# Plachtaa/FAcodec

Measured on AMD Instinct MI355X. Metric: 24kHz audio sec encoded+decoded per wall-sec, higher is better.
Workload: dtype f32; 1 GPU; configs[1]: batch=32/GPU x 2 s @ 24 kHz, forward encoder->FVQ(6 codebooks)->decoder, FAcodec configs/config.yml model (137.7 M params), weights formula-generated, weight-norm re-materialised every step; clips_per_gpu=32, samples_per_clip=48000, parallelism=dp1 (independent clips, no collective)

## Files before the change

facodec_amd/_lib.py:

```python
import ctypes as C
import os

_HERE = os.path.dirname(os.path.abspath(__file__))
LIB_PATH = os.environ.get("FAC_LIB_PATH", os.path.join(_HERE, "libfacodec_hip.so"))

PAD_ZERO, PAD_REFLECT = 0, 1
ACT_NONE, ACT_TANH, ACT_MISH, ACT_LOG_MEL = 0, 1, 2, 3
ACT_GATE, ACT_WN_RES_SKIP = 4, 5

_p = C.c_void_p
_i = C.c_int
_i64 = C.c_int64
_f = C.c_float


class ConvDesc(C.Structure):
    _fields_ = [
        ("x", _p), ("w", _p), ("bias", _p), ("alpha_in", _p), ("alpha_out", _p), ("res", _p), ("y", _p), ("y2", _p), ("alpha_y2", _p), ("w_k1", _p), ("bias_k1", _p),
        ("x_bs", _i64), ("x_cs", _i64), ("y_bs", _i64), ("y_cs", _i64),
        ("B", C.c_int32), ("C_in", C.c_int32), ("T_in", C.c_int32), ("C_out", C.c_int32),
        ("C_out_pad", C.c_int32), ("T_out", C.c_int32),
        ("K", C.c_int32), ("stride", C.c_int32), ("dilation", C.c_int32), ("pad_left", C.c_int32),
        ("pad_mode", C.c_int32), ("n_phase", C.c_int32), ("y_tstride", C.c_int32), ("phase_shift", C.c_int32),
        ("act", C.c_int32),
        ("w_batched", C.c_int32), ("w_bs", _i64), ("ws", _p), ("ws_bytes", _i64), ("w_split", _p),
        ("K1", C.c_int32), ("dilation2", C.c_int32), ("row_phases", C.c_int32),
        ("x_p8", _p), ("x_p8_plane_bytes", _i64), ("y2_p8", _p), ("y2_p8_plane_bytes", _i64),
        ("pw_split", C.c_int32), ("split_rows", C.c_int32),
        ("gate_cond", _p), ("gate_cond_bs", _i64),
    ]


class VqDesc(C.Structure):
    _fields_ = [
        ("residual", _p), ("z_in", _p), ("zq_acc", _p), ("zq_out", _p), ("w_in", _p), ("b_in", _p),
        ("codebook", _p), ("w_out", _p), ("w_out_scale", _p), ("b_out", _p), ("mask", _p), ("codes", _p), ("z_e", _p),
        ("loss_part", _p), ("codes_bs", _i64),
        ("B", C.c_int32), ("D", C.c_int32), ("T", C.c_int32), ("Kc", C.c_int32),
    ]



VQ_DECODE_MAX_Q = 16


class VqDecodeDesc(C.Structure):
    _fields_ = [
        ("codes", _p * 3), ("codes_bs", _i64 * 3), ("codes_qs", _i64 * 3), ("n_q", C.c_int32 * 3),
        ("codebook", _p * VQ_DECODE_MAX_Q), ("w_out", _p * VQ_DECODE_MAX_Q), ("w_out_scale", _p * VQ_DECODE_MAX_Q),
        ("b_out", _p * VQ_DECODE_MAX_Q), ("style", _p), ("outs", _p), ("z", _p * 3),
        ("B", C.c_int32), ("D", C.c_int32), ("T", C.c_int32), ("Kc", C.c_int32),
    ]


class ResampleDesc(C.Structure):
    _fields_ = [
        ("hist", _p), ("x", _p), ("lens", _p), ("y", _p), ("hist_out", _p), ("table", _p), ("offs", _p),
        ("hist_bs", _i64), ("x_bs", _i64), ("y_bs", _i64), ("q0", _i64), ("m_lo", _i64),
        ("B", C.c_int32), ("n_hist", C.c_int32), ("T", C.c_int32), ("n_out", C.c_int32),
        ("o", C.c_int32), ("n", C.c_int32), ("taps", C.c_int32),
    ]


SIGNATURES = {
    "fac_version": (_i, []),
    "fac_last_error": (C.c_char_p, []),
    "fac_wn_scale": (_i, [_p, _p, _p, _i, _i, _p]),
    "fac_pack_conv_w": (_i, [_p, _p, _p, _i, _i, _i, _i, _p]),
    "fac_pack_convtr_w_rows": (_i, [_p, _p, _p, _i, _i, _i, _p]),
    "fac_conv_w_split_bytes": (_i64, [_i, _i, _i]),
    "fac_conv_w_split2_bytes": (_i64, [_i, _i, _i, _i]),
    "fac_pack_conv_w_split2": (_i, [_p, _p, _p, _i, _i, _i, _i, _p]),
    "fac_gemm_w_split_bytes": (_i64, [_i, _i, _i, _i]),
    "fac_pack_gemm_w_split": (_i, [_p, _i64, _i64, _i64, _p, _p, _i, _i, _i, _i, _p]),
    "fac_pack_conv_w_split": (_i, [_p, _p, _p, _i, _i, _i, _p]),
    "fac_conv_w_split_rows_bytes": (_i64, [_i, _i, _i, _i]),
    "fac_pack_conv_w_split_rows": (_i, [_p, _p, _p, _i, _i, _i, _i, _p]),
    "fac_flip_transpose_w": (_i, [_p, _p, _p, _i, _i, _i, _p]),
    "fac_prep_begin": (_i, []),
    "fac_prep_set_phase": (_i, [_i]),
    "fac_prep_abort": (_i, []),
    "fac_prep_end": (_i, []),
    "fac_prep_replay": (_i, [_i, _p]),
    "fac_prep_info": (_i, [_i, _p, _p]),
    "fac_prep_free": (_i, [_i]),
    "fac_pack_conv_w_bwd": (_i, [_p, _p, _p, _i, _i, _i, _i, _p]),
    "fac_pad_fold_bwd": (_i, [_p, _p, _i, _i, _i, _i, _i, _i, _p]),
    "fac_conv1d_bwd_weight_ws_bytes": (_i64, [_i, _i, _i, _i, _i]),
    "fac_conv1d_bwd_weight": (_i, [_p, _p, _p, _p, _i64, _i, _i, _i, _i, _i, _i, _i, _i, _i, _i, _i, _i, _p]),
    "fac_conv1d_bwd_weight_split_ws_bytes": (_i64, [_i, _i, _i, _i, _i, _i, _i, _i, _i, _i]),
    "fac_conv1d_bwd_weight_split_form": (_i, [_i, _i, _i, _i, _i, _i, _i, _i, _i, _i, _i, C.POINTER(C.c_int)]),
    "fac_conv1d_bwd_weight_k1_ws_bytes": (_i64, [_i, _i, _i, _i]),
    "fac_conv1d_bwd_weight_k1_ws_bytes_for": (_i64, [_p, _p, _i, _i, _i, _i]),
    "fac_conv1d_bwd_weight_taps_tx": (_i64, [_i, _i, _i, _i, _i]),
    "fac_conv1d_bwd_weight_taps_ws_bytes": (_i64, [_i, _i, _i, _i, _i, _i, _i, _i]),
    "fac_conv1d_bwd_weight_taps_ws_bytes_for": (_i64, [_p, _i, _i, _i, _i, _i, _i, _i, _i]),
    "fac_conv1d_bwd_weight_taps": (_i, [_p, _p, _p, _p, _p, _i64, _i, _i, _i, _i, _i, _i, _i, _i, _i, _p]),
    "fac_conv1d_bwd_weight_k1": (_i, [_p, _p, _p, _p, _p, _i64, _i, _i, _i, _i, _p]),
    "fac_conv1d_bwd_weight_split": (_i, [_p, _p, _p, _p, _i64, _i, _i, _i, _i, _i, _i, _i, _i, _i, _i, _i, _i, _p]),
    "fac_conv1d_bwd_weight_split_db_ok": (_i, [_i, _i, _i, _i, _i, _i, _i, _i, _i, _i]),
    "fac_conv1d_bwd_weight_split_db": (_i, [_p, _p, _p, _p, _p, _i64, _i, _i, _i, _i, _i, _i, _i, _i, _i, _i, _i, _i, _p]),
    "fac_weight_norm_bwd": (_i, [_p, _p, _p, _p, _p, _i, _i, _p]),
    "fac_snake_bwd": (_i, [_p, _p, _p, _p, _p, _p, _i, _i, _i, _p]),
    "fac_pack_lstm_whh_t": (_i, [_p, _p, _i, _p]),
    "fac_lstm_layer_bwd": (_i, [_p, _p, _p, _p, _p, _p, _i, _i, _i, _p]),
    "fac_to_p8": (_i, [_p, _p, _p, _i, _i, _i, _p]),
    "fac_lstm_persist_ok": (_i, [_i, _i]),
    "fac_lstm_persist_stream_ok": (_i, [_p]),
    "fac_pack_lstm_whh16": (_i, [_p, _p, _i, _i, _p]),
    "fac_lstm_layer_fwd_persist": (_i, [_p, _p, _p, _p, _p, _p, _i, _i, _i, _i, _p]),
    "fac_lstm_layer_bwd_persist": (_i, [_p, _p, _p, _p, _p, _p, _i, _i, _i, _i, _p]),
    "fac_lstm_persist_split_ok": (_i, [_i, _i]),
    "fac_lstm_persist_timeouts": (_i, []),
    "fac_lstm_persist_arm": (_i, [_p]),
    "fac_lstm_abort_flag": (_i, [_p, _p]),
    "fac_mask_flags_if": (_i, [_p, _i, _p, _p]),
    "fac_pack_lstm_whh_split": (_i, [_p, _p, _i, _p]),
    "fac_lstm_layer_fwd_persist_split": (_i, [_p, _p, _p, _p, _i, _i, _i, _i, _p]),
    "fac_snake_bwd_fused": (_i, [_p, _p, _p, _p, _p, _p, _p, _p, _i, _i, _i, _p]),
    "fac_bias_grad": (_i, [_p, _p, _p, _i, _i, _i, _p]),
    "fac_snake_bwd_fused_rs": (_i, [_p, _p, _p, _i64, _p, _p, _p, _p, _p, _i, _i, _i, _p]),
    "fac_pad_fold_edges": (_i, [_p, _i, _i, _i, _i, _i, _p]),
    "fac_pack_convtr_w": (_i, [_p, _p, _p, _i, _i, _i, _i, _p]),
    "fac_conv1d_fwd": (_i, [C.POINTER(ConvDesc), _p]),
    "fac_conv1d_variant": (_i, [C.POINTER(ConvDesc), C.c_char_p, _i]),
    "fac_snake_fwd": (_i, [_p, _p, _p, _i, _i, _i, _p]),
    "fac_lstm_to_time_major": (_i, [_p, _p, _i, _i, _i, _p]),
    "fac_lstm_from_time_major": (_i, [_p, _p, _p, _p, _i, _i, _i, _p]),
    "fac_pack_lstm_whh": (_i, [_p, _p, _i, _p]),
    "fac_lstm_layer_fwd": (_i, [_p, _p, _p, _p, _i, _i, _i, _p]),
    "fac_lstm_layer_fwd_from": (_i, [_p, _p, _p, _p, _i, _i, _i, _i64, _p]),
    "fac_lstm_layer_fwd_train": (_i, [_p, _p, _p, _p, _p, _p, _i, _i, _i, _i64, _p]),
    "fac_lstm_gate_bwd": (_i, [_p, _p, _p, _p, _p, _p, _p, _i, _i, _i64, _i, _p]),
    "fac_tanh_bwd": (_i, [_p, _p, _p, _i64, _p]),
    "fac_pair_bwd": (_i, [_p, _p, _p, _i64, _i, C.c_float, C.c_float, _i, _p]),
    "fac_spec_power_bwd": (_i, [_p, _p, _p, _i, _i, _i, _i, _p]),
    "fac_stft_frames_bwd": (_i, [_p, _p, _i, _i, _i, _i, _i, _i, _i, _p]),
    "fac_vq_latent_bwd": (_i, [_p, _p, _p, _i64, _p, _p, _p, _p, _i, _i, _p]),
    "fac_vq_codebook_grad": (_i, [_p, _p, _p, _i64, _p, _p, _i, _i, _i, _i, _p]),
    "fac_layernorm_c_affine_bwd": (_i, [_p, _p, _p, _p, _p, _p, _i, _i, _i, _p]),
    "fac_rows_fma": (_i, [_p, _p, _p, _p, _i, _i64, _f, _p]),
    "fac_grad_norm_clip": (_i, [_p, _i64, _f, _p, _p, _p]),
    "fac_adamw_step": (_i, [_p, _p, _p, _p, _i64, _f, _f, _f, _f, _f, _i64, _p, _p]),
    "fac_logdiff_rms_bwd": (_i, [_p, _p, _p, _i, _i, _i, _f, _f, _i, _p]),
    "fac_gather_copy": (_i, [_p, _p, _p, _i, _p]),
    "fac_adamw_step_masked": (_i, [_p, _p, _p, _p, _i64, _p, _i, _p, _p, _p, _f, _f, _f, _f, _f, _p, _p]),
    "fac_gate_bwd": (_i, [_p, _p, _p, _i, _i, _i, _p]),
    "fac_mish_fwd": (_i, [_p, _p, _i64, _p]),
    "fac_mish_bwd": (_i, [_p, _p, _p, _i64, _p]),
    "fac_glu_bwd": (_i, [_p, _p, _p, _i, _i, _i, _p]),
    "fac_mul_scaled": (_i, [_p, _p, _p, _f, _i64, _p]),
    "fac_embed_sum_bwd": (_i, [_p, _p, _p, _i, _i, _i, _i, _i, _i, _i, _p]),
    "fac_gate_bwd_cond": (_i, [_p, _p, _i64, _p, _p, _p, _i64, _i, _i, _i, _p]),
    "fac_masked_mean_bwd": (_i, [_p, _p, _p, _i, _i, _i, _p]),
    "fac_attention_probs": (_i, [_p, _p, _p, _p, _i, _i, _i, _i, _p]),
    "fac_attention_pv": (_i, [_p, _p, _p, _i, _i, _i, _i, _p]),
    "fac_attention_bwd_pv": (_i, [_p, _p, _p, _p, _p, _i, _i, _i, _i, _p]),
    "fac_attention_bwd_qk": (_i, [_p, _p, _p, _p, _p, _p, _p, _i, _i, _i, _i, _p]),
    "fac_aa_snakebeta_bwd": (_i, [_p, _p, _p, _p, _p, _p, _p, _p, _p, _i, _i, _i, _p]),
    "fac_leaky_relu": (_i, [_p, _p, _p, _i64, _f, _i, _i, _i, _i, _i, _p]),
    "fac_spec_to_cat": (_i, [_p, _p, _i, _i, _i, _i, _i, _i, _i, _p]),
    "fac_period_fold": (_i, [_p, _p, _i, _i, _i, _i, _i, _i, _p]),
    "fac_zero_insert": (_i, [_p, _p, _i64, _i, _i, _p]),
    "fac_row_stack3": (_i, [_p, _p, _i64, _i, _i, _i, _i, _p]),
    "fac_spec_to_rows": (_i, [_p, _p, _i, _i, _i, _i, _i, _i, _p]),
    "fac_pad_reflect": (_i, [_p, _p, _i, _i, _i, _i, _p]),
    "fac_disc_preprocess": (_i, [_p, _p, _p, _p, _i, _i, _p]),
    "fac_cross_entropy": (_i, [_p, _p, _p, _p, _p, _i64, _i, _f, _p]),
    "fac_focal_scalar": (_i, [_p, _p, _f, _p]),
    "fac_crop_rows": (_i, [_p, _p, _p, _i, _i, _i64, _i, _i, _p]),
    "fac_stream_push": (_i, [_p, _p, _i64, _i64, _i, _i, _i, _p]),
    "fac_vq_fwd": (_i, [C.POINTER(VqDesc), _p]),
    "fac_vq_loss_tiles": (_i, [_i]),
    "fac_vq_decode": (_i, [C.POINTER(VqDecodeDesc), _p]),
    "fac_rccl_available": (_i, []),
    "fac_rccl_unique_id": (_i, [_p]),
    "fac_rccl_comm_init": (_i, [C.POINTER(_p), _p, _i, _i]),
    "fac_rccl_comm_destroy": (_i, [_p]),
    "fac_allreduce_arena": (_i, [_p, _p, _i64, _i, _p]),
    "fac_vq_search": (_i, [_p, _p, _p, _i64, _i, _p]),
    "fac_gate_tanh_sigmoid": (_i, [_p, _p, _i64, _p, _i, _i, _i, _p]),
    "fac_embed_sum": (_i, [_p, _p, _p, _i, _i, _i, _i, _i, _i, _i, _i, _p]),
    "fac_glu_residual": (_i, [_p, _p, _p, _i, _i, _i, _p]),
    "fac_add": (_i, [_p, _p, _p, _i64, _p]),
    "fac_sub2": (_i, [_p, _p, _p, _p, _i64, _p]),
    "fac_mul_mask": (_i, [_p, _p, _i, _i, _i, _p]),
    "fac_wn_res_skip": (_i, [_p, _p, _p, _i, _i, _i, _i, _p]),
    "fac_attention": (_i, [_p, _p, _p, _p, _p, _i, _i, _i, _i, _p]),
    "fac_attention_stream": (_i, [_p, _p, _p, _p, _p, _i, _i, _i, _i, _p]),
    "fac_attention_route": (_i, [_i, _i]),
    "fac_attention_stream_tile": (_i, [_i]),
    "fac_masked_mean": (_i, [_p, _p, _p, _i, _i, _i, _p]),
    "fac_layernorm_c_affine": (_i, [_p, _p, _p, _i, _i, _i, _p]),
    "fac_stft_frames": (_i, [_p, _p, _i, _i, _i, _i, _i, _i, _i, _p]),
    "fac_stft_frames_ragged": (_i, [_p, _p, _p, _i, _i, _i, _i, _i, _i, _i, _p]),
    "fac_mask_tail": (_i, [_p, _p, _i, _i, _i, _i, _p]),
    "fac_mask_tail_i64": (_i, [_p, _p, _i, _i, _i, _i, _p]),
    "fac_frame_mask": (_i, [_p, _p, _p, _i, _i, _i, _p]),
    "fac_resample": (_i, [C.POINTER(ResampleDesc), _p]),
    "fac_resample_form": (_i, [C.POINTER(ResampleDesc), _p]),
    "fac_spec_power": (_i, [_p, _p, _i, _i, _i, _i, _p]),
    "fac_reduce_pair": (_i, [_p, _p, _p, _p, _i64, _i, _f, _f, _i, _p]),
    "fac_aa_snakebeta_fwd": (_i, [_p, _p, _p, _p, _p, _i, _i, _i, _p]),
    "fac_logdiff_rms": (_i, [_p, _p, _p, _p, _i, _i, _i, _f, _f, _i, _p]),
    "fac_jdc_affine_lrelu_pool": (_i, [_p, _p, _p, _p, _i, _i, _i, _i, _i, _i, _i, _f, _p]),
    "fac_jdc_layout_in": (_i, [_p, _p, _i, _i, _i, _i, _p]),
    "fac_jdc_to_time_major": (_i, [_p, _p, _i, _i, _i, _i, _i, _i, _i, _p]),
    "fac_jdc_to_nchw": (_i, [_p, _p, _i, _i, _i, _i, _i, _i, _p]),
    "fac_jdc_head": (_i, [_p, _p, _p, _p, _p, _i, _i, _i, _i, _p]),
    "fac_f0_normalize": (_i, [_p, _p, _p, _i, _i, _p]),
    "fac_mel_log_norm": (_i, [_p, _p, _i, _i, _i, _p]),
}

_lib = None


class FacodecHipError(RuntimeError):
    pass


def load():
    global _lib
    if _lib is not None:
# ... 20 lines not shown
```

facodec_amd/build.py:

```python
import os
import subprocess
import sys
from concurrent.futures import ThreadPoolExecutor

HERE = os.path.dirname(os.path.abspath(__file__))
CSRC = os.path.join(HERE, "csrc")
TAG = os.environ.get("FAC_BUILD_TAG", "")
LIB = os.path.join(HERE, "libfacodec_hip%s.so" % ("_" + TAG if TAG else ""))
OBJDIR = "build" + ("_" + TAG if TAG else "")
SOURCES = ["conv1d_api.hip", "conv1d_tile_128x128.hip", "conv1d_tile_96x128.hip", "conv1d_tile_64x128.hip",
           "conv1d_tile_32x256.hip", "conv1d_tile_128x32.hip", "conv1d_tile_128x256.hip", "conv1d_fused_ru.hip", "conv1d_narrow.hip", "conv1d_pw.hip", "conv1d_pw_split.hip", "conv1d_skinny.hip", "conv1d_bsplit.hip", "conv1d_bsplit96.hip", "conv1d_gemm_split.hip", "conv1d_bsplit2.hip", "conv1d_bwd.hip", "conv1d_wgrad_split.hip", "conv1d_wgrad_k1.hip", "train_misc.hip", "optim.hip", "train_quant.hip", "train_pred.hip", "train_disc.hip", "train_redecoder.hip", "pack.hip", "prep_batch.hip", "lstm.hip", "lstm_persist.hip", "vq.hip", "vq_decode.hip", "misc.hip", "attention_stream.hip", "ragged.hip", "resample.hip", "jdc.hip", "rccl_arena.hip"]
FLAGS = ["--offload-arch=gfx950", "-O3", "-std=c++17", "-fPIC", "-ffp-contract=off",
         "-Wno-unused-result"] + os.environ.get("FAC_EXTRA_FLAGS", "").split()


def _hipcc():
    for cand in (os.environ.get("HIPCC"), "/opt/rocm/bin/hipcc", "hipcc"):
        if cand and (os.path.isabs(cand) and os.path.exists(cand) or not os.path.isabs(cand)):
            return cand
    return "hipcc"


def _stale(target, deps):
    if not os.path.exists(target):
        return True
    tt = os.path.getmtime(target)
    return any(os.path.getmtime(d) > tt for d in deps)


def build_lib(force=False, verbose=True):
    hipcc = _hipcc()
    headers = sorted(os.path.join(CSRC, f) for f in os.listdir(CSRC) if f.endswith(".h")) + [os.path.join(HERE, "..", "include", "facodec_hip.h")]
    objs, jobs = [], []
    os.makedirs(os.path.join(CSRC, OBJDIR), exist_ok=True)
    for src in SOURCES:
        s = os.path.join(CSRC, src)
        o = os.path.join(CSRC, OBJDIR, src.replace(".hip", ".o"))
        objs.append(o)
        if force or _stale(o, [s] + headers):
            jobs.append([hipcc, *FLAGS, "-c", s, "-o", o])

    def run(cmd):
        if verbose:
            print(" ".join(cmd), file=sys.stderr)
        subprocess.run(cmd, check=True)

    with ThreadPoolExecutor(max_workers=min(8, max(1, len(jobs)))) as ex:
        list(ex.map(run, jobs))
    if force or jobs or _stale(LIB, objs):
        run([hipcc, "--offload-arch=gfx950", "-shared", "-fPIC", *objs, "-ldl", "-o", LIB])
    return LIB


if __name__ == "__main__":
    build_lib(force="--force" in sys.argv)
    print(LIB)
```

facodec_amd/convplan.py:

```python
from collections import namedtuple

__all__ = ["ConvPlan", "ConvTrPlan", "plan_conv", "plan_convtr", "plan_gemm", "tile_rows", "gemm_split_ok", "gemm_split_strided_ok", "split2_ok",
           "pw_taps_ok", "pw_split_tail_ok", "convtr_split_ok", "convtr_rows_ok", "flat_strided_ok", "flat_convtr_ok", "W_FP32", "W_TAPS",
           "W_GEMM", "W_GEMM_STRIDED", "W_SPLIT2", "W_FP32_PW_TAPS", "PER_CLIP", "FLAT_STRIDED", "FLAT_STRIDE1", "TR_POLYPHASE", "TR_ROWS",
           "TR_ROWS_SPLIT", "TR_ROWS_PW_TAPS", "TR_FLAT"]

W_FP32, W_TAPS, W_GEMM, W_GEMM_STRIDED, W_SPLIT2, W_FP32_PW_TAPS = "fp32", "split_taps", "split_gemm", "split_gemm_strided", "split2", "fp32_pw_taps"
PER_CLIP, FLAT_STRIDED, FLAT_STRIDE1 = "per_clip", "flat_strided", "flat_stride1"
ConvPlan = namedtuple("ConvPlan", "layout form p8")
TR_POLYPHASE, TR_ROWS, TR_ROWS_SPLIT, TR_ROWS_PW_TAPS, TR_FLAT = "polyphase", "rows", "rows_split", "rows_pw_taps", "flat_rows_split"
ConvTrPlan = namedtuple("ConvTrPlan", "layout p8")


def _sw():
    from . import ops
    return ops


def gemm_split_ok(c_out, c_in, k, n_cols, t_out=None):
    sw = _sw()
    if not (sw.BF16_SPLIT and k in (1, 2)):
        return False
    if c_in < sw.GEMM_SPLIT_MIN_CIN or c_out < 64 or n_cols < 1024:
        return False
    return k == 1 or (t_out is not None and t_out >= 256)


def gemm_split_strided_ok(c_out, c_in, k, stride, batch, t_out):
    return (_sw().BF16_SPLIT and 1 < stride <= 16 and stride < k <= 2 * stride and c_in >= 32
            and c_out >= 64 and t_out >= 256 and batch * t_out >= 1024)


def split2_ok(c_out, k, k1, stride, n_cols):
    kv = k1 if 0 < k1 < k else k
    return (_sw().BF16_SPLIT and 8 <= c_out <= 32 and ((kv == 9 and stride in (1, 2)) or (kv == 3 and stride == 1))
            and n_cols >= 4096)


def pw_split_tail_ok(c_in, c_out, cols):
    sw = _sw()
    return sw.BF16_SPLIT and sw.PW_SPLIT and c_in == c_out and c_in in (256, 384) and cols >= 65536


def pw_taps_ok(c_in, c_out, k, stride, transposed, batch, t_out):
    sw = _sw()
    if not (sw.BF16_SPLIT and sw.PW_SPLIT and sw.PW_TAPS and stride == 2):
        return False
    taps, rows = (2, 2 * c_out) if transposed else (4, c_out)
    if k != 4 or (c_in * taps) % 64 or c_in * taps > 384 or rows % 64:
        return False
    return batch * ((t_out + 31) // 32) >= 2 * (256 // (rows // 64)) * 12


def convtr_rows_ok(t_in, stride, causal=True):
    sw = _sw()
    return sw.CONVTR_ROWS and causal and 2 <= stride <= 16 and t_in >= sw.CONVTR_ROWS_MIN_T


def convtr_split_ok(c_in, c_out, stride, batch, t_in, causal=True, alpha_in=None):
    return (_sw().BF16_SPLIT and causal and alpha_in is None and 2 <= stride <= 16 and c_in >= 64
            and t_in >= 256 and batch * t_in >= 1024 and c_out * stride >= 64)


def flat_strided_ok(c_out, c_in, k, s, batch, n_out):
    return (_sw().FLAT_TRAIN and k == 2 * s and s > 1 and n_out < 256 and not gemm_split_strided_ok(c_out, c_in, k, s, batch, n_out)
            and gemm_split_strided_ok(c_out, c_in, k, s, 1, batch * (n_out + 1) - 1))


def flat_convtr_ok(c_in, c_out, s, batch, t_cols):
    return (_sw().FLAT_TRAIN and t_cols < 256 and not convtr_split_ok(c_in, c_out, s, batch, t_cols)
            and convtr_split_ok(c_in, c_out, s, 1, batch * t_cols))


def tile_rows(c_out, c_in, k, grad=False):
    sw = _sw()
    return 96 if (sw.BF16_SPLIT and not grad and k == 7 and c_out in sw.BS_ROWS96 and c_in % 8 == 0) else 64


def plan_conv(c_out, c_in, k, stride, dilation, batch, t_in, t_out, *, k1=0, alpha_in=False, plain=True, res=False,
              causal_reflect=False, grad=True, c_out_mult16=True, split_k=(1, 3, 5, 7), floor_k=(3, 5), tail="pw_split",
              pw_taps=True, split2=False, flat_infer=False, flat_stride1=False, flat_train=None):
    sw = _sw()
    cols = batch * t_out
    p8 = 2.0 * c_out * k / (4.0 * stride)
    if split2 and split2_ok(c_out, k, k1, stride, cols):
        return ConvPlan(W_SPLIT2, PER_CLIP, None)
    if stride > 1:
        strided = not alpha_in and dilation == 1 and not k1
        flat_t = (flat_train is not None and strided and plain and t_in % stride == 0
                  and (flat_train == "zero" or (causal_reflect and t_in > stride))
                  and flat_strided_ok(c_out, c_in, k, stride, batch, t_out))
        if flat_t and flat_train == "reflect":
            return ConvPlan(W_GEMM_STRIDED, FLAT_STRIDED, p8)
        if pw_taps and stride == 2 and strided and plain and pw_taps_ok(c_in, c_out, k, 2, False, batch, t_out):
            return ConvPlan(W_FP32_PW_TAPS, PER_CLIP, None)
        if strided and gemm_split_strided_ok(c_out, c_in, k, stride, batch, t_out):
            return ConvPlan(W_GEMM_STRIDED, PER_CLIP, p8)
        if flat_t:
            return ConvPlan(W_GEMM_STRIDED, FLAT_STRIDED, p8)
        if (flat_infer and strided and not res and causal_reflect and k == 2 * stride and t_in % stride == 0 and t_in > stride
                and not grad and gemm_split_strided_ok(c_out, c_in, k, stride, 1, batch * (t_in // stride + 1) - 1)):
            return ConvPlan(W_GEMM_STRIDED, FLAT_STRIDED, p8)
    elif not alpha_in and not k1 and k in split_k:
        if k == 1 and gemm_split_ok(c_out, c_in, 1, cols):
            if not (pw_split_tail_ok(c_in, c_out, cols) if tail == "pw_split"
                    else tail is not None and c_in == c_out and c_in in (256, 384) and cols >= 65536):
                return ConvPlan(W_GEMM, PER_CLIP, None)
        if (sw.BF16_SPLIT and k in (3, 5, 7) and c_in % 16 == 0 and c_out > 2 and (c_out % 16 == 0 or not c_out_mult16)
                and cols > 640 and (k not in floor_k or (c_in >= 64 and c_out > 32))):
            if (flat_infer and flat_stride1 and k == 7 and not res and causal_reflect and not grad and batch >= 4
                    and (k - 1) * dilation < t_in <= 224 and c_in * c_out >= 1 << 20):
                return ConvPlan(W_TAPS, FLAT_STRIDE1, None)
            return ConvPlan(W_TAPS, PER_CLIP, None)
    return ConvPlan(W_FP32, PER_CLIP, None)


def plan_gemm(c_out, c_in, n_cols):
    ok = gemm_split_ok(c_out, c_in, 1, n_cols)
    return ConvPlan(W_GEMM if ok else W_FP32, PER_CLIP, 2.0 * c_out / 4.0 if ok else None)


def plan_convtr(c_in, c_out, stride, batch, t_in, *, causal=True, alpha_in=False, grad=True, flat_infer=False, flat_train_cols=None):
    a = True if alpha_in else None
    p8 = 2.0 * c_out * 2 * stride / 4.0
    if causal and flat_train_cols is not None and flat_convtr_ok(c_in, c_out, stride, batch, flat_train_cols):
        return ConvTrPlan(TR_FLAT, p8)
    if causal and not alpha_in and pw_taps_ok(c_in, c_out, 2 * stride, stride, True, batch, t_in):
        return ConvTrPlan(TR_ROWS_PW_TAPS, None)
    if convtr_split_ok(c_in, c_out, stride, batch, t_in, causal, a):
        return ConvTrPlan(TR_ROWS_SPLIT, p8)
    if flat_infer and not grad and t_in < 256 and convtr_split_ok(c_in, c_out, stride, 1, batch * (t_in + 1), causal, a):
        return ConvTrPlan(TR_FLAT, p8)
    return ConvTrPlan(TR_ROWS if convtr_rows_ok(t_in, stride, causal) else TR_POLYPHASE, None)
```

facodec_amd/csrc/common.h:

```cpp
#pragma once
#include <hip/hip_runtime.h>
#include <stdint.h>
#include <stdio.h>
#include <stdarg.h>
#include "../../include/facodec_hip.h"

namespace fac {

void set_error(const char* fmt, ...);

inline int check_launch(const char* what) {
  hipError_t e = hipGetLastError();
  if (e != hipSuccess) {
    set_error("%s: launch failed: %s", what, hipGetErrorString(e));
    return FAC_ERR_LAUNCH;
  }
  return FAC_OK;
}

#define FAC_REQUIRE(cond, ...)          \
  do {                                  \
    if (!(cond)) {                      \
      ::fac::set_error(__VA_ARGS__);    \
      return FAC_ERR_ARG;               \
    }                                   \
  } while (0)

__host__ __device__ constexpr int cin_pad_dev(int c) { return ((c + 47) / 48) * 48; }

__device__ __attribute__((noinline)) float sin_sq_slow(float y) {
  const float s = sinf(y);
  return __fmul_rn(s, s);
}

__device__ __forceinline__ float sin_sq(float y) {
  if (__builtin_expect(fabsf(y) > 4096.0f, 0)) return sin_sq_slow(y);
  const float k = rintf(y * 0.63661977236758134308f);
  float r = fmaf(k, -1.5703125f, y);
  r = fmaf(k, -4.837512969970703125e-4f, r);
  r = fmaf(k, -7.54978995489188216e-8f, r);
  const float z = r * r;
  float ps = fmaf(z, -1.9515295891e-4f, 8.3321608736e-3f);
  ps = fmaf(ps, z, -1.6666654611e-1f);
  const float sn = fmaf(ps * z, r, r);
  float pc = fmaf(z, 2.443315711809948e-5f, -1.388731625493765e-3f);
  pc = fmaf(pc, z, 4.166664568298827e-2f);
  const float cs = fmaf(pc * z, z, fmaf(z, -0.5f, 1.0f));
  const float v = (((int)k) & 1) ? cs : sn;
  return __fmul_rn(v, v);
}

__device__ __forceinline__ float snake_inv(float alpha) { return __fdiv_rn(1.0f, __fadd_rn(alpha, 1e-9f)); }
__device__ __forceinline__ float snake_apply(float x, float alpha, float inv) {
  return __fadd_rn(x, __fmul_rn(inv, sin_sq(__fmul_rn(alpha, x))));
}

__device__ __attribute__((noinline)) float apply_act_slow(float v, int act) {
  if (act == FAC_ACT_TANH) return tanhf(v);
  if (act == FAC_ACT_MISH) {
    const float sp = v > 20.f ? v : log1pf(expf(v));
    return v * tanhf(sp);
  }
  if (act == FAC_ACT_LOG_MEL) return (logf(1e-5f + v) + 4.0f) / 4.0f;
  return v;
}

__device__ __forceinline__ float sigmoid_f(float x) { return __fdiv_rn(1.0f, 1.0f + expf(-x)); }

__device__ __forceinline__ int reflect_index(int t, int T, int Text) {
  int j;
  if (t < 0) j = -t;
  else if (t < Text) j = t;
  else j = 2 * (Text - 1) - t;
  return (j >= 0 && j < T) ? j : -1;
}


typedef __bf16 bf16x8 __attribute__((ext_vector_type(8)));
typedef __bf16 bf16x4 __attribute__((ext_vector_type(4)));
typedef float f32x16 __attribute__((ext_vector_type(16)));
typedef float f32x4 __attribute__((ext_vector_type(4)));
typedef float f32x2 __attribute__((ext_vector_type(2)));
typedef unsigned u32x4 __attribute__((ext_vector_type(4)));

__device__ __forceinline__ void split3(float x, __bf16& h, __bf16& m, __bf16& l) {
  h = (__bf16)x;
  const float r1 = x - (float)h;
  m = (__bf16)r1;
  l = (__bf16)(r1 - (float)m);
}

__device__ __forceinline__ void wg_barrier() {
  asm volatile("" ::: "memory");
  __builtin_amdgcn_s_barrier();
  asm volatile("" ::: "memory");
}

template <class V>
__host__ __device__ constexpr int xcd_contiguous_id(V v, int n) {
  const int q8 = n >> 3, r8 = n & 7;
  const int xcd = v & 7, within = v >> 3;
  return (xcd < r8 ? xcd * (q8 + 1) : r8 * (q8 + 1) + (xcd - r8) * q8) + within;
}
constexpr bool xcd_contiguous_is_permutation(int n) {
  bool seen[64] = {};
  for (int v = 0; v < n; ++v) {
    const int id = xcd_contiguous_id(v, n);
    if (id < 0 || id >= n || seen[id]) return false;
    seen[id] = true;
  }
  return true;
}
static_assert(xcd_contiguous_is_permutation(1) && xcd_contiguous_is_permutation(7) && xcd_contiguous_is_permutation(8) &&
                  xcd_contiguous_is_permutation(9) && xcd_contiguous_is_permutation(13) && xcd_contiguous_is_permutation(64),
              "xcd_contiguous_id must map [0, n) onto [0, n)");

struct XcdGrid {
  int per_xcd;
  unsigned grid;
};
inline XcdGrid xcd_padded_grid(long long total) {
  const int per_xcd = (int)((total + 7) / 8);
  return {per_xcd, (unsigned)(8 * per_xcd)};
}


constexpr size_t FAC_LDS_MAX = 160 * 1024;

template <auto Kern>
inline void allow_dynamic_lds(size_t bytes = FAC_LDS_MAX) {
  static bool done = false;
  if (!done) {
    (void)hipFuncSetAttribute(reinterpret_cast<const void*>(Kern), hipFuncAttributeMaxDynamicSharedMemorySize, (int)bytes);
    done = true;
  }
}

constexpr int FAC_MAX_DEV = 16;
inline int device_cus() {
  static int cus[FAC_MAX_DEV] = {0};
  int dev = 0, v = 0;
  if (hipGetDevice(&dev) != hipSuccess || dev < 0 || dev >= FAC_MAX_DEV) return 0;
  if (cus[dev] == 0 && hipDeviceGetAttribute(&v, hipDeviceAttributeMultiprocessorCount, dev) == hipSuccess) cus[dev] = v;
  return cus[dev];
}

}

#define FAC_PRIO_STAGE 3
#define FAC_PRIO_MFMA 0
```

facodec_amd/csrc/conv1d_api.hip:

```cpp
#include "conv1d_mfma.h"
#include <stdlib.h>

namespace fac {

enum ConvKernel : int {
  CK_128x32 = 0,
  CK_32x256 = 1,
  CK_64x128 = 2,
  CK_96x128 = 3,
  CK_128x128 = 4,
  CK_128x256 = 5,
  CK_96x256 = 6,
  CK_FUSED_RU = 7,
  CK_128x160 = 8,
  CK_NARROW = 9,
  CK_SKINNY = 10,
  CK_BSPLIT = 11,
  CK_CIN1 = 12,
  CK_THIN = 13,
  CK_PW = 14,
  CK_GSPLIT = 15,
  CK_BSPLIT2 = 16,
  CK_PWS = 17,
  CK_PWT = 18,
  CK_BSPLIT96 = 19,
};

static ConvKernel select_variant(const fac_conv_desc* d) {
  const int co = d->C_out;
  if (d->row_phases > 1) return CK_128x256;
  if (d->T_out <= 32) return CK_128x32;
  if (co <= 32) return CK_32x256;
  if (co <= 64) return CK_64x128;
  const bool wide = d->K == 1 && d->n_phase == 1 && d->T_out >= 512;
  if (d->T_out > 128 && d->T_out <= 160 && co > 64) return CK_128x160;
  if (co % 128 != 0 && co % 96 == 0) return wide ? CK_96x256 : CK_96x128;
  return wide ? CK_128x256 : CK_128x128;
}

static bool narrow_ok(const fac_conv_desc* d) {
  return d->C_out <= 2 && d->stride == 1 && d->n_phase == 1 && d->phase_shift == 0 && d->y_tstride == 1 && !d->res && !d->y2 &&
         !d->w_batched && d->y && (long long)d->B <= 65535 && (long long)d->B * ((d->T_out + 1023) / 1024) >= 128;
}

static bool pw_enabled() {
  static const bool on = !(getenv("FAC_PW") && getenv("FAC_PW")[0] == '0');
  return on;
}

static int conv_plan(const fac_conv_desc* d, ConvArgs& a, ConvKernel& k) {
  FAC_REQUIRE(d && (d->x || d->x_p8) && (d->w || d->w_split) && (d->y || d->y2 || d->y2_p8), "conv1d: null pointer");
  FAC_REQUIRE(!d->y2 || d->alpha_y2 || d->act == FAC_ACT_WN_RES_SKIP, "conv1d: y2 needs alpha_y2");
  FAC_REQUIRE(d->B > 0 && d->C_in > 0 && d->C_out > 0 && d->T_in > 0 && d->T_out > 0,
              "conv1d: bad shape B=%d C_in=%d C_out=%d T_in=%d T_out=%d", d->B, d->C_in, d->C_out,
              d->T_in, d->T_out);
  FAC_REQUIRE(d->K >= 1 && d->stride >= 1 && d->dilation >= 1 && d->pad_left >= 0,
              "conv1d: bad K/stride/dilation/pad");
  FAC_REQUIRE(d->C_out_pad % 32 == 0 && (d->C_out_pad >= d->C_out || d->row_phases > 1), "conv1d: C_out_pad must be a multiple of 32");
  FAC_REQUIRE(d->n_phase >= 1 && d->y_tstride >= 1, "conv1d: bad phase config");
  FAC_REQUIRE((long long)d->B * d->n_phase <= 65535, "conv1d: B*n_phase too large for grid.z");
  a.x = d->x; a.w = d->w; a.bias = d->bias; a.alpha_in = d->alpha_in; a.alpha_out = d->alpha_out;
  a.res = d->res; a.y = d->y; a.y2 = d->y2; a.alpha2 = d->alpha_y2;
  a.w1 = d->w_k1; a.bias1 = d->bias_k1;
  a.x_p8 = reinterpret_cast<const unsigned char*>(d->x_p8); a.x_p8_ps = d->x_p8_plane_bytes;
  a.y2_p8 = reinterpret_cast<unsigned char*>(d->y2_p8); a.y2_p8_ps = d->y2_p8_plane_bytes;
  FAC_REQUIRE(!d->y2_p8 || d->alpha_y2, "conv1d: y2_p8 needs alpha_y2");
  if (d->w_k1) {
    FAC_REQUIRE(d->C_in == d->C_out && d->C_out_pad == d->C_out && d->n_phase == 1 && d->stride == 1 &&
                    d->alpha_out && d->act == FAC_ACT_NONE && !d->w_batched,
                "conv1d: fused ResidualUnit needs C_in == C_out (multiple of 32), stride 1, a Snake alpha_out");
  }
  a.x_bs = d->x_bs; a.x_cs = d->x_cs; a.y_bs = d->y_bs; a.y_cs = d->y_cs; a.w_bs = d->w_bs;
  a.B = d->B; a.C_in = d->C_in; a.T_in = d->T_in; a.C_out = d->C_out; a.C_out_pad = d->C_out_pad;
  a.T_out = d->T_out; a.K = d->K; a.stride = d->stride; a.dil = d->dilation;
  a.pad_left = d->pad_left; a.pad_mode = d->pad_mode; a.n_phase = d->n_phase;
  a.y_tstride = d->y_tstride; a.act = d->act; a.w_batched = d->w_batched;
  a.phase_shift = d->phase_shift;
  a.rp = d->row_phases > 1 ? d->row_phases : 1;
  FAC_REQUIRE(!d->gate_cond || (d->act == FAC_ACT_GATE && d->gate_cond_bs >= 0),
              "conv1d: gate_cond is the conditioning row of the FAC_ACT_GATE epilogue (act=%d gate_cond_bs=%lld)", d->act,
              (long long)d->gate_cond_bs);
  a.gate_cond = d->gate_cond; a.gate_cond_bs = d->gate_cond_bs;
  if (a.rp > 1) {
    FAC_REQUIRE(d->n_phase == 1 && d->y_tstride == 1 && d->phase_shift == 0 && d->stride == 1 && a.rp <= 128 && !d->w_k1 &&
                    !d->w_batched && d->C_out_pad == fac_convtr_rows(d->C_out, a.rp) && !(d->K1 > 0 && d->K1 < d->K),
                "conv1d: row_phases needs a plain stride-1 launch on weights from fac_pack_convtr_w_rows");
  }
  a.K1 = d->K1 > 0 ? d->K1 : d->K; a.dil2 = d->dilation2;
  FAC_REQUIRE(a.K1 <= d->K && d->K % a.K1 == 0 && (a.K1 == d->K || d->dilation2 > 0), "conv1d: bad two-level taps (K=%d K1=%d)", d->K, d->K1);
  FAC_REQUIRE(!conv_two_level(a) || (!d->w_k1 && d->n_phase == 1 && d->pad_mode == FAC_PAD_ZERO && !d->w_batched),
              "conv1d: two-level taps need a plain, zero-padded conv");
  conv_set_virtual(a);
  FAC_REQUIRE(d->phase_shift >= 0 && d->phase_shift < d->n_phase + (d->n_phase == 1), "conv1d: bad phase_shift");
  {
    long long last = (long long)(d->T_out - 1) * d->stride + (long long)conv_max_tap_offset(a) - d->pad_left;
    int pad_right = last >= d->T_in ? (int)(last - d->T_in + 1) : 0;
    int max_pad = d->pad_left > pad_right ? d->pad_left : pad_right;
    a.T_ext = d->T_in > max_pad ? d->T_in : max_pad + 1;
  }
  if (d->x_p8 || d->y2_p8) {
    const bool gs = d->w_split && (d->K <= 2 || (d->stride > 1 && d->K <= 2 * d->stride)) && conv_gsplit_ok(a) &&
                    !conv_skinny_ok(a, d->ws, d->ws_bytes) && d->C_in % 8 == 0 && d->x_p8_plane_bytes < (1ll << 32);
    const bool ok = !d->y2_p8 && (gs || (d->w_split && !conv_two_level(a) && (d->split_rows == 96 ? conv_bsplit96_p8_ok(a) : conv_bsplit_p8_ok(a)) &&
                                       !conv_cin1_ok(a)));
    FAC_REQUIRE(ok, "conv1d: P8 operands given but the launch does not run on a kernel that takes them (K=%d stride=%d C_in=%d columns=%lld)",
                d->K, d->stride, d->C_in, (long long)d->B * d->T_out);
  }
  if (d->act == FAC_ACT_GATE || d->act == FAC_ACT_WN_RES_SKIP) {
    FAC_REQUIRE(d->w && !d->w_k1 && !d->x_p8 && !conv_two_level(a) && conv_skinny_ok(a, d->ws, d->ws_bytes),
                "conv1d: FAC_ACT_GATE / FAC_ACT_WN_RES_SKIP exist only for few-column launches (B * T_out <= 640) with a workspace");
    k = CK_SKINNY;
    return FAC_OK;
  }
  if (d->w_k1) { k = CK_FUSED_RU; return FAC_OK; }
  a.gflat = 0;
  a.grt = 0;
  if (d->w_split && (a.KV == 9 || a.KV == 3) && d->C_out <= 32 && conv_bsplit2_ok(a)) {
    a.w = reinterpret_cast<const float*>(d->w_split);
    k = CK_BSPLIT2;
    return FAC_OK;
  }
  FAC_REQUIRE(!conv_two_level(a) || d->w, "conv1d: two-level taps outside the split kernel's shapes need fp32 weights");
  const bool pw_on = pw_enabled();
  if (pw_on && d->pw_split && d->w && conv_pwt_ok(a)) { k = CK_PWT; return FAC_OK; }
  if (d->w_split && (d->K <= 2 || (d->stride > 1 && d->K <= 2 * d->stride)) && conv_gsplit_ok(a) &&
      !conv_skinny_ok(a, d->ws, d->ws_bytes)) {
    a.w = reinterpret_cast<const float*>(d->w_split);
    k = CK_GSPLIT;
    return FAC_OK;
  }
  if (a.rp > 1) {
    FAC_REQUIRE(d->w != nullptr && d->w != (const float*)d->w_split, "conv1d: row_phases launch outside the split kernel's shapes needs fp32 weights");
    k = CK_128x256;
    return FAC_OK;
  }
  const bool two_level = conv_two_level(a);
  FAC_REQUIRE(d->split_rows == 0 || d->split_rows == 64 || d->split_rows == 96, "conv1d: split_rows must be 0, 64 or 96");
  if (d->split_rows == 96) {
    FAC_REQUIRE(d->w_split && !two_level && conv_bsplit96_ok(a) && !conv_cin1_ok(a),
                "conv1d: split_rows = 96 needs a stride-1 k = 7 launch with C_out %% 96 == 0, C_in %% 8 == 0 and more than 640 columns "
                "(K=%d stride=%d C_in=%d C_out=%d columns=%lld)", d->K, d->stride, d->C_in, d->C_out, (long long)d->B * d->T_out);
    a.w = reinterpret_cast<const float*>(d->w_split);
    k = CK_BSPLIT96;
    return FAC_OK;
  }
  if (d->w_split && !two_level && conv_bsplit_ok(a) && !conv_cin1_ok(a)) {
    a.w = reinterpret_cast<const float*>(d->w_split);
    k = CK_BSPLIT;
    return FAC_OK;
  }
  FAC_REQUIRE(d->w != nullptr && (const void*)d->w != d->w_split,
              "conv1d: shape does not qualify for a split-bf16 kernel (K=%d stride=%d C_in=%d C_out=%d columns=%lld) and no fp32 "
              "weights were given", d->K, d->stride, d->C_in, d->C_out, (long long)d->B * d->T_out);
  if (!two_level && conv_skinny_ok(a, d->ws, d->ws_bytes)) k = CK_SKINNY;
  else if (narrow_ok(d) && (!two_level || (a.KV - 1) * a.dil <= 64)) k = CK_NARROW;
  else if (conv_thin_ok(a, d->ws, d->ws_bytes)) k = CK_THIN;
  else if (conv_cin1_ok(a)) k = CK_CIN1;
  else if (pw_on && d->pw_split && conv_pw_ok(a) && conv_pws_ok(a)) k = CK_PWS;
  else if (pw_on && conv_pw_ok(a)) k = CK_PW;
  else k = select_variant(d);
  return FAC_OK;
}

}

extern "C" int fac_conv1d_fwd(const fac_conv_desc* d, fac_stream_t stream) {
  using namespace fac;
  ConvArgs a;
  ConvKernel k;
  if (const int rc = conv_plan(d, a, k)) return rc;
  hipStream_t s = (hipStream_t)stream;
  switch (k) {
    case CK_128x32: return conv_dispatch_128x32(a, s);
    case CK_32x256: return conv_dispatch_32x256(a, s);
    case CK_64x128: return conv_dispatch_64x128(a, s);
    case CK_96x128: return conv_dispatch_96x128(a, s);
    case CK_128x128: return conv_dispatch_128x128(a, s);
    case CK_128x256: return conv_dispatch_128x256(a, s);
    case CK_96x256: return conv_dispatch_96x256(a, s);
    case CK_FUSED_RU: return conv_dispatch_fused_ru(a, s);
    case CK_128x160: return conv_dispatch_128x160(a, s);
    case CK_NARROW: return conv_dispatch_narrow(a, s);
    case CK_SKINNY: return conv_dispatch_skinny(a, d->ws, d->ws_bytes, s);
    case CK_BSPLIT: return conv_dispatch_bsplit(a, s);
    case CK_CIN1: return conv_dispatch_cin1(a, s);
    case CK_THIN: return conv_dispatch_thin(a, d->ws, s);
    case CK_PW: return conv_dispatch_pw(a, s);
    case CK_GSPLIT: return conv_dispatch_gsplit(a, s);
    case CK_BSPLIT2: return conv_dispatch_bsplit2(a, s);
    case CK_PWS: return conv_dispatch_pws(a, s);
    case CK_PWT: return conv_dispatch_pwt(a, s);
    case CK_BSPLIT96: return conv_dispatch_bsplit96(a, s);
  }
  return FAC_ERR_ARG;
}

extern "C" int fac_conv1d_variant(const fac_conv_desc* d, char* name, int name_len) {
  using namespace fac;
  ConvArgs a;
  ConvKernel k;
  if (const int rc = conv_plan(d, a, k)) return rc;
  if (!name || name_len <= 0) return k;
  switch (k) {
    case CK_128x32: snprintf(name, name_len, "conv1d_mfma_kernel<1,1,4,1,K> 128x32"); break;
    case CK_32x256: snprintf(name, name_len, "conv1d_mfma_kernel<1,2,1,4,K> 32x256"); break;
    case CK_64x128: snprintf(name, name_len, "conv1d_mfma_kernel<2,1,1,4,K> 64x128"); break;
    case CK_96x128: snprintf(name, name_len, "conv1d_mfma_kernel<3,1,1,4,K> 96x128"); break;
    case CK_128x128: snprintf(name, name_len, "conv1d_mfma_kernel<2,2,2,2,K> 128x128"); break;
    case CK_128x256:
      snprintf(name, name_len, a.rp > 1 ? "conv1d_mfma_kernel<2,2,2,4,2> 128x256 (convtr, all phases per tile)" : "conv1d_mfma_kernel<2,2,2,4,K> 128x256");
      break;
    case CK_96x256: snprintf(name, name_len, "conv1d_mfma_kernel<3,1,1,8,K> 96x256"); break;
    case CK_FUSED_RU: snprintf(name, name_len, "conv1d_mfma_kernel<C/32,1,1,4,7,fused RU> Cx128"); break;
    case CK_128x160: snprintf(name, name_len, "conv1d_mfma_kernel<1,5,4,1,K> 128x160"); break;
    case CK_NARROW:
      snprintf(name, name_len, conv_two_level(a) ? "conv1d_narrow_kernel (VALU, C_out<=2, two-level taps)" : "conv1d_narrow_kernel (VALU, C_out<=2)");
      break;
    case CK_SKINNY:
      snprintf(name, name_len, conv_skinny_single_launch(a) ? "conv1d_gemv_kernel (single launch, <=4 columns)"
                                                            : "conv1d_skinny_kernel (split reduction, <=640 columns)");
      break;
    case CK_BSPLIT: snprintf(name, name_len, "conv1d_bsplit_kernel<%d> 64x256 (bf16x3 split, fp32-grade)", a.K); break;
    case CK_CIN1: snprintf(name, name_len, "conv1d_cin1_kernel (VALU, C_in=1, store stream)"); break;
    case CK_THIN: snprintf(name, name_len, "conv1d_thin_kernel (VALU, C_out<=8, split channels)"); break;
    case CK_PW: snprintf(name, name_len, "conv1d_pw_kernel (k=1 streaming, W in LDS)"); break;
    case CK_GSPLIT:
      snprintf(name, name_len, "conv1d_gemm_split_kernel<%d> 128x128 (bf16x3 split GEMM, fp32-grade)", a.stride > 1 ? 2 : a.K);
      break;
    case CK_BSPLIT2: snprintf(name, name_len, "conv1d_bsplit2_kernel<%d,%d> 32x512 (bf16x3 split, fp32-grade)", a.KV, a.stride); break;
    case CK_PWS: snprintf(name, name_len, "conv1d_pws_kernel (k=1 streaming, W planes in LDS, bf16x3 split, fp32-grade)"); break;
    case CK_PWT: snprintf(name, name_len, "conv1d_pwt_kernel<%d taps> (streaming, W planes in LDS, bf16x3 split, fp32-grade)", a.K); break;
    case CK_BSPLIT96: snprintf(name, name_len, "conv1d_bsplit_kernel<%d> 96x256 (bf16x3 split, fp32-grade)", a.K); break;
  }
  return k;
}
```

facodec_amd/csrc/conv1d_bsplit.hip:

```cpp
#include "conv1d_bsplit_kernel.h"

namespace fac {

__device__ __forceinline__ void pack_conv_split_body(const float* __restrict__ v, const float* __restrict__ scale,
                                                     bf16x8* __restrict__ out, int C_out, int C_in, int K, int G, int H, int n_st,
                                                     int CO, long long n, int vb, int vg) {
  for (long long idx = (long long)vb * 256 + threadIdx.x; idx < n; idx += (long long)vg * 256) {
    const int co = (int)(idx % CO);
    long long r = idx / CO;
    const int hs = (int)(r % H);
    r /= H;
    const int s = (int)(r % n_st);
    const int ct = (int)(r / n_st);
    const int g = hs % G, k = hs / G;
    const int cog = ct * CO + co;
    const float sc = (scale != nullptr && cog < C_out) ? scale[cog] : 1.0f;
    bf16x8 h, m, l;
#pragma unroll
    for (int i = 0; i < 8; ++i) {
      const int ci = (s * G + g) * 8 + i;
      float w = 0.f;
      if (cog < C_out && ci < C_in && k < K) {
        w = v[((long long)cog * C_in + ci) * K + k];
        if (scale != nullptr) w = __fmul_rn(w, sc);
      }
      __bf16 a, b2, c;
      split3(w, a, b2, c);
      h[i] = a; m[i] = b2; l[i] = c;
    }
    const long long base = ((long long)ct * n_st + s) * 3;
    out[((base + 0) * H + hs) * CO + co] = h;
    out[((base + 1) * H + hs) * CO + co] = m;
    out[((base + 2) * H + hs) * CO + co] = l;
  }
}

__global__ __launch_bounds__(256) void pack_conv_split_kernel(const float* __restrict__ v, const float* __restrict__ scale,
                                                              bf16x8* __restrict__ out, int C_out, int C_in, int K, int G, int H,
                                                              int n_st, int CO, long long n) {
  pack_conv_split_body(v, scale, out, C_out, C_in, K, G, H, n_st, CO, n, blockIdx.x, gridDim.x);
}

__global__ __launch_bounds__(256) void bsplit_batch_kernel(const PrepJob* __restrict__ jobs, const int* __restrict__ first, int njobs) {
  const int j = prep_find_job(first, njobs, blockIdx.x);
  const PrepJob& J = jobs[j];
  pack_conv_split_body(static_cast<const float*>(J.a), static_cast<const float*>(J.b), static_cast<bf16x8*>(J.out), J.i[0], J.i[1],
                       J.i[2], J.i[3], J.i[4], J.i[5], J.i[6], J.n, blockIdx.x - first[j], J.nblocks);
}

int prep_launch_bsplit(const PrepJob* jobs, const int* first, int njobs, int total, hipStream_t s) {
  hipLaunchKernelGGL(bsplit_batch_kernel, dim3(total), dim3(256), 0, s, jobs, first, njobs);
  return check_launch("bsplit_batch");
}

bool conv_bsplit_ok(const ConvArgs& a) {
  if (!((a.K == 7 || a.K == 5 || a.K == 3) && a.stride == 1 && a.n_phase == 1 && a.phase_shift == 0 && a.y_tstride == 1 && !a.alpha_in &&
        !a.w1 && !a.w_batched && (long long)a.B * a.T_out > 640))
    return false;
  const int G = bs_group(a.C_in), tt = G == 2 ? 256 : 512;
  const int kp = G == 2 ? a.K - 1 : ((a.K + 1) & ~1) - 1;
  return a.C_in % (8 * G) == 0 && G * ((tt + kp * a.dil + 63) / 64) <= BS_NSW * BS_XU &&
         a.x_cs * (long long)a.C_in < (1ll << 31);
}

bool conv_bsplit_p8_ok(const ConvArgs& a) {
  return conv_bsplit_ok(a) && bs_group(a.C_in) == 2 && (long long)a.T_in * 16 < (1ll << 32);
}

int conv_dispatch_bsplit(ConvArgs& a, hipStream_t s) {
  if (a.K == 5)
    return bs_group(a.C_in) == 2 ? bsplit_launch<5, 2, 4, BS_NSW_WIDE>(a, s) : bsplit_launch<5, 1, 8, BS_NSW>(a, s);
  if (a.K == 3)
    return bs_group(a.C_in) == 2 ? bsplit_launch<3, 2, 4, BS_NSW_WIDE>(a, s) : bsplit_launch<3, 1, 8, BS_NSW>(a, s);
  return bs_group(a.C_in) == 2 ? bsplit_launch<7, 2, 4, BS_NSW_WIDE>(a, s) : bsplit_launch<7, 1, 8, BS_NSW>(a, s);
}

}

extern "C" int fac_debug_bsplit_occupancy(int lds_bytes) {
  int n = -1;
  auto kern = fac::conv1d_bsplit_kernel<7, 2, 4, fac::BS_NSW_WIDE>;
  (void)hipFuncSetAttribute(reinterpret_cast<const void*>(kern), hipFuncAttributeMaxDynamicSharedMemorySize, (int)fac::FAC_LDS_MAX);
  if (hipOccupancyMaxActiveBlocksPerMultiprocessor(&n, kern, (4 + fac::BS_NSW) * 64, (size_t)lds_bytes) != hipSuccess) return -1;
  return n;
}

static bool split_rows_ok(int K, int rows) { return rows == fac::BS_CO || (rows == fac::BS96_CO && K == 7); }

extern "C" int64_t fac_conv_w_split_rows_bytes(int C_out, int C_in, int K, int rows) {
  using namespace fac;
  if (!split_rows_ok(K, rows)) return -1;
  const int G = rows == BS96_CO ? 1 : bs_group(C_in);
  const int64_t n_ct = (C_out + rows - 1) / rows, n_st = (C_in + 8 * G - 1) / (8 * G);
  return n_ct * n_st * 3 * bs_slots(K, G) * rows * 16;
}

extern "C" int64_t fac_conv_w_split_bytes(int C_out, int C_in, int K) { return fac_conv_w_split_rows_bytes(C_out, C_in, K, fac::BS_CO); }

extern "C" int fac_pack_conv_w_split_rows(const float* v, const float* scale, void* out, int C_out, int C_in, int K, int rows,
                                          fac_stream_t stream) {
  using namespace fac;
  FAC_REQUIRE(v && out && C_out > 0 && C_in > 0 && K > 0, "pack_conv_w_split: bad arguments");
  FAC_REQUIRE(split_rows_ok(K, rows), "pack_conv_w_split: no %d-row tile for K=%d", rows, K);
  const int G = rows == BS96_CO ? 1 : bs_group(C_in);
  const int n_ct = (C_out + rows - 1) / rows, n_st = (C_in + 8 * G - 1) / (8 * G), H = bs_slots(K, G);
  const long long n = (long long)n_ct * n_st * H * rows;
  const int blocks = (int)((n + 255) / 256 < 65535 ? (n + 255) / 256 : 65535);
  if (prep_recording()) {
    PrepJob j{}; j.a = v; j.b = scale; j.out = out; j.kind = PK_CONV_SPLIT; j.nblocks = blocks; j.n = n;
    j.i[0] = C_out; j.i[1] = C_in; j.i[2] = K; j.i[3] = G; j.i[4] = H; j.i[5] = n_st; j.i[6] = rows;
    return prep_record(PU_BSPLIT, j);
  }
  hipLaunchKernelGGL(pack_conv_split_kernel, dim3(blocks), dim3(256), 0, (hipStream_t)stream, v, scale,
                     reinterpret_cast<bf16x8*>(out), C_out, C_in, K, G, H, n_st, rows, n);
  return check_launch("pack_conv_w_split");
}

extern "C" int fac_pack_conv_w_split(const float* v, const float* scale, void* out, int C_out, int C_in, int K,
                                     fac_stream_t stream) {
  return fac_pack_conv_w_split_rows(v, scale, out, C_out, C_in, K, fac::BS_CO, stream);
}
```

facodec_amd/csrc/conv1d_bsplit_kernel.h:

```cpp
#pragma once
#include "conv1d_mfma.h"
#include <type_traits>
#include "inflight_regs.h"
#include "prep_batch.h"

namespace fac {

constexpr int BS_CO = 64;
constexpr int BS96_CO = 96;
constexpr int BS_NSW = 4;
constexpr int BS_NSW_WIDE = 4;
constexpr int BS_XU = 3;
constexpr int BS_WIDE_MIN = 64;
__host__ __device__ constexpr int bs_group(int C_in) { return C_in >= BS_WIDE_MIN ? 2 : 1; }

__host__ __device__ constexpr int bs_slots(int K, int G) { return (G * K + 1) & ~1; }

template <int KT, int G, int NMW, int NSW, int MB = 2>
__global__ __launch_bounds__((NMW + NSW) * 64, (NMW + NSW) / 4) void conv1d_bsplit_kernel(ConvArgs a) {
  constexpr int NB = 2;
  constexpr int CO = 32 * MB;
  constexpr bool WIDE = NMW == 4;
  constexpr int BS_TT = 64 * NMW;
  constexpr int H = bs_slots(KT, G);
  constexpr int W_STAGE = 3 * H * CO * 16;
  extern __shared__ __attribute__((aligned(16))) unsigned char sm[];
  const int tid = threadIdx.x;
  const int lane = tid & 63;
  const int wave = __builtin_amdgcn_readfirstlane(tid >> 6);
  const int XW = a.XW;
  const int X_STAGE = 48 * G * XW;
  const int STG = W_STAGE + X_STAGE;
  unsigned char* Wbuf = sm;
  unsigned char* Xbuf = sm + W_STAGE;
  const int n_chunks = (a.C_in + 8 * G - 1) / (8 * G);
  const int dil = a.dil;

  const int n_tiles = a.n_tiles;
  typedef const __attribute__((address_space(4))) ConvArgs* KArgP;
  const KArgP kargs = (KArgP)__builtin_amdgcn_kernarg_segment_ptr();
  auto fresh_args = [&]() {
    KArgP q = kargs;
    asm volatile("" : "+s"(q));
    return q;
  };
  auto decode = [&](KArgP ka, int v, int& t0_, int& co0_, int& b_) {
    const int id = xcd_contiguous_id(v, n_tiles);
    const int nt = ka->n_t_tiles;
    const int tt = id % nt;
    const int rest = id / nt;
    const int nb = ka->B;
    b_ = rest % nb;
    co0_ = (rest / nb) * CO;
    t0_ = tt * BS_TT;
  };
  const bool overlap = a.persist != 0;
  unsigned char* epi_base = sm + (overlap ? STG : 0);
  auto walk = [&](auto role) {
  constexpr int ROLE = decltype(role)::value;
  constexpr bool STAGING = ROLE != 0;
  bool first = true;
  unsigned cboff[BS_XU] = {}, nboff[BS_XU] = {};
  unsigned long long cmask[BS_XU] = {}, nmask[BS_XU] = {};
  const float *cxg = nullptr, *nxg = nullptr;
  const unsigned char *cws = nullptr, *nws = nullptr;
  for (int vb = blockIdx.x; vb < n_tiles; vb += gridDim.x) {
  int t0, co0, b;
  decode(fresh_args(), vb, t0, co0, b);
  const bool has_nt = overlap && vb + (int)gridDim.x < n_tiles;

  if constexpr (STAGING) {
    const int lw = wave - NMW;
    __builtin_amdgcn_s_setprio(FAC_PRIO_STAGE);
    const float* xg = a.x + (long long)b * a.x_bs;
    const int xcs = (int)a.x_cs;
    const unsigned char* wsrc = reinterpret_cast<const unsigned char*>(a.w) + (long long)(co0 / CO) * n_chunks * W_STAGE;
    const int n_blk = (XW + 63) >> 6;
    int u_g[BS_XU], u_c[BS_XU], u_idx[BS_XU];
#pragma unroll
    for (int j = 0; j < BS_XU; ++j) {
      const int u = lw + NSW * j;
      u_g[j] = u % G;
      const int c = (u / G) * 64 + lane;
      u_c[j] = (u < G * n_blk && c < XW) ? c : -1;
      const int tin = t0 - a.pad_left + c;
      int idx;
      if (a.pad_mode == FAC_PAD_REFLECT) idx = reflect_index(tin, a.T_in, a.T_ext);
      else idx = (tin >= 0 && tin < a.T_in) ? tin : -1;
      u_idx[j] = u_c[j] >= 0 ? idx : -1;
    }
    constexpr int NBLK = W_STAGE / 1024;
    constexpr int ND = (NBLK + NSW - 1) / NSW;
    constexpr int NX = BS_XU * 8;
    static_assert(W_STAGE % 1024 == 0 && ND + NX <= 63 && NX == 24, "vmcnt is a 6-bit counter; FAC_XREGS24_* list 24 registers per set");
    auto stage_w = [&](int chunk, int buf) {
      constexpr int N16 = W_STAGE / 16;
      const unsigned char* src = wsrc + (long long)chunk * W_STAGE;
      unsigned char* dst = Wbuf + buf * STG;
      for (int i = lw; i * 64 < N16; i += NSW) {
        const int q = i * 64 + lane;
        if (q < N16)
          __builtin_amdgcn_global_load_lds((glb_void_t*)(src + (long long)q * 16), (lds_void_t*)(dst + i * 1024), 16, 0, 0);
      }
    };
    auto write_x = [&](int buf, const float (&xr)[BS_XU][8]) {
      unsigned char* xd = Xbuf + buf * STG;
#pragma unroll
      for (int j = 0; j < BS_XU; ++j) {
        if (u_c[j] < 0) continue;
        bf16x8 h, m, l;
#pragma unroll
        for (int i = 0; i < 8; ++i) {
          __bf16 p0, p1, p2;
          split3(xr[j][i], p0, p1, p2);
          h[i] = p0; m[i] = p1; l[i] = p2;
        }
        *reinterpret_cast<bf16x8*>(xd + ((0 * G + u_g[j]) * XW + u_c[j]) * 16) = h;
        *reinterpret_cast<bf16x8*>(xd + ((1 * G + u_g[j]) * XW + u_c[j]) * 16) = m;
        *reinterpret_cast<bf16x8*>(xd + ((2 * G + u_g[j]) * XW + u_c[j]) * 16) = l;
      }
    };
    if constexpr (ROLE == 2) {
      typedef float wv4 __attribute__((ext_vector_type(4)));
      const unsigned char* xp = a.x_p8 + (long long)b * (a.C_in / 8) * a.T_in * 16;
      const long long grp_bytes = (long long)a.T_in * 16;
      unsigned u_poff[BS_XU];
      bool any_pad = false;
#pragma unroll
      for (int j = 0; j < BS_XU; ++j) {
        u_poff[j] = (unsigned)(u_idx[j] >= 0 ? u_idx[j] : 0) * 16u;
        any_pad = any_pad || __builtin_amdgcn_ballot_w64(u_c[j] >= 0 && u_idx[j] < 0) != 0;
      }
      for (int c = -1; c < n_chunks; ++c) {
        if (c + 1 < n_chunks) {
          const int buf = (c + 1) & 1;
          wv4 wv[ND], xv[BS_XU][3];
          const unsigned char* src = wsrc + (long long)(c + 1) * W_STAGE;
#pragma unroll
          for (int j = 0; j < ND; ++j) {
            const int bi = min(lw + NSW * j, NBLK - 1);
            wv[j] = *reinterpret_cast<const wv4*>(src + bi * 1024 + lane * 16);
          }
#pragma unroll
          for (int j = 0; j < BS_XU; ++j) {
            const unsigned char* grp = xp + (long long)((c + 1) * G + u_g[j]) * grp_bytes;
#pragma unroll
            for (int pl = 0; pl < 3; ++pl) xv[j][pl] = *reinterpret_cast<const wv4*>(grp + pl * a.x_p8_ps + u_poff[j]);
          }
          unsigned char* xd = Xbuf + buf * STG;
#pragma unroll
          for (int j = 0; j < BS_XU; ++j) {
            if (u_c[j] < 0) continue;
#pragma unroll
            for (int pl = 0; pl < 3; ++pl) {
              wv4 v = xv[j][pl];
              if (any_pad && u_idx[j] < 0) v = wv4{0.f, 0.f, 0.f, 0.f};
              *reinterpret_cast<wv4*>(xd + ((pl * G + u_g[j]) * XW + u_c[j]) * 16) = v;
            }
          }
          unsigned char* dst = Wbuf + buf * STG;
#pragma unroll
          for (int j = 0; j < ND; ++j) {
            const int bi = min(lw + NSW * j, NBLK - 1);
            *reinterpret_cast<wv4*>(dst + bi * 1024 + lane * 16) = wv[j];
          }
        }
        __syncthreads();
      }
    } else if constexpr (WIDE) {
#define BS_LD(n, R)                                                                                                          \
  asm volatile("global_load_dword v" #R ", %0, %1" : : "v"(u_boff[(n) / 8]), "s"(grp[(n) / 8] + (long long)((n) % 8) * xcs) : "memory", "v" #R);
#define BS_RD(n, R) asm volatile("v_cndmask_b32_e64 %0, 0, v" #R ", %1" : "=v"(xr[(n) / 8][(n) % 8]) : "s"(u_mask[(n) / 8]) : "memory");
      auto tile_params = [&](int t0_, int b_, int co0_, unsigned (&boff)[BS_XU], unsigned long long (&mask)[BS_XU], const float*& xgp,
                             const unsigned char*& wsp) {
        const KArgP ka = fresh_args();
        const int pad_left = ka->pad_left, pad_mode = ka->pad_mode, T_in = ka->T_in, T_ext = ka->T_ext;
#pragma unroll
        for (int j = 0; j < BS_XU; ++j) {
          const int tin = t0_ - pad_left + u_c[j];
          int idx;
          if (pad_mode == FAC_PAD_REFLECT) idx = reflect_index(tin, T_in, T_ext);
          else idx = (tin >= 0 && tin < T_in) ? tin : -1;
          if (u_c[j] < 0) idx = -1;
          boff[j] = (unsigned)(idx >= 0 ? idx : 0) * 4u;
          mask[j] = __builtin_amdgcn_ballot_w64(idx >= 0);
        }
        xgp = ka->x + (long long)b_ * ka->x_bs;
        wsp = reinterpret_cast<const unsigned char*>(ka->w) + (long long)(co0_ / CO) * n_chunks * W_STAGE;
      };
      if (first) tile_params(t0, b, co0, cboff, cmask, cxg, cws);
      if (has_nt) {
        int nt0, nco0, nb;
        decode(fresh_args(), vb + (int)gridDim.x, nt0, nco0, nb);
        tile_params(nt0, nb, nco0, nboff, nmask, nxg, nws);
      }
      auto load_a = [&](const float* xgp, const unsigned (&u_boff)[BS_XU], int chunk) {
        const float* grp[BS_XU];
#pragma unroll
        for (int j = 0; j < BS_XU; ++j) grp[j] = xgp + (long long)((chunk * G + u_g[j]) * 8) * xcs;
        FAC_XREGS24_A(BS_LD)
      };
      auto load_b = [&](const float* xgp, const unsigned (&u_boff)[BS_XU], int chunk) {
        const float* grp[BS_XU];
#pragma unroll
        for (int j = 0; j < BS_XU; ++j) grp[j] = xgp + (long long)((chunk * G + u_g[j]) * 8) * xcs;
        FAC_XREGS24_B(BS_LD)
      };
      auto take_a = [&](float (&xr)[BS_XU][8], const unsigned long long (&u_mask)[BS_XU]) { FAC_XREGS24_A(BS_RD) };
      auto take_b = [&](float (&xr)[BS_XU][8], const unsigned long long (&u_mask)[BS_XU]) { FAC_XREGS24_B(BS_RD) };
      typedef float wv4 __attribute__((ext_vector_type(4)));
// ... 25 lines not shown
            for (int j = 0; j < BS_XU; ++j) u_boff[j] = nx2 ? nboff[j] : cboff[j];
            const float* xgp = nx2 ? nxg : cxg;
            const int chunk = nx2 ? c + 2 - n_chunks : c + 2;
            if (i == 0) load_a(xgp, u_boff, chunk); else load_b(xgp, u_boff, chunk);
          }
          if (has_next) {
            write_x(1 - i, xr);
            if (has_next2) asm volatile("s_waitcnt vmcnt(%0)" : : "n"(NX) : "memory");
            else asm volatile("s_waitcnt vmcnt(0)" ::: "memory");
            unsigned char* dst = Wbuf + (1 - i) * STG + wblk0 * 1024 + lane16;
#pragma unroll
            for (int j = 0; j < ND; ++j) {
              asm volatile("" : "+v"(wv[j]) : : "memory");
              *reinterpret_cast<wv4*>(dst + j * 1024) = wv[j];
            }
          }
          if (c >= -1) {
            asm volatile("s_waitcnt lgkmcnt(0)" ::: "memory");
            __builtin_amdgcn_s_barrier();
            asm volatile("" ::: "memory");
          }
        }
      }
      if (has_nt) {
#pragma unroll
        for (int j = 0; j < BS_XU; ++j) {
          cboff[j] = nboff[j];
          cmask[j] = nmask[j];
        }
        cxg = nxg;
        cws = nws;
      }
#undef BS_LD
#undef BS_RD
    } else {
      int u_off[BS_XU];
#pragma unroll
      for (int j = 0; j < BS_XU; ++j) u_off[j] = u_idx[j] >= 0 ? u_idx[j] : 0;
      auto load_x = [&](int chunk, float (&xr)[BS_XU][8]) {
#pragma unroll
        for (int j = 0; j < BS_XU; ++j) {
          const float* grp = xg + (long long)((chunk * G + u_g[j]) * 8) * xcs;
#pragma unroll
          for (int i = 0; i < 8; ++i) {
            const float v = (grp + (long long)i * xcs)[u_off[j]];
            xr[j][i] = u_idx[j] >= 0 ? v : 0.f;
          }
        }
      };
      float xa[BS_XU][8], xb[BS_XU][8];
      load_x(0, xa);
      stage_w(0, 0);
      if (n_chunks > 1) load_x(1, xb);
      write_x(0, xa);
      __syncthreads();
      for (int chunk = 0; chunk < n_chunks; chunk += 2) {
        if (chunk + 1 < n_chunks) {
          stage_w(chunk + 1, 1);
          if (chunk + 2 < n_chunks) load_x(chunk + 2, xa);
          write_x(1, xb);
        }
        __syncthreads();
        if (chunk + 1 >= n_chunks) break;
        if (chunk + 2 < n_chunks) {
          stage_w(chunk + 2, 0);
          if (chunk + 3 < n_chunks) load_x(chunk + 3, xb);
          write_x(0, xa);
        }
        __syncthreads();
      }
    }
    __builtin_amdgcn_s_setprio(0);
  } else {
  __builtin_amdgcn_s_setprio(FAC_PRIO_MFMA);
  const int l31 = lane & 31;
  const int kq = lane >> 5;
  const int n0 = wave * 64;
  f32x16 acc[MB][NB];
#pragma unroll
  for (int m = 0; m < MB; ++m)
#pragma unroll
    for (int n = 0; n < NB; ++n)
#pragma unroll
      for (int r = 0; r < 16; ++r) acc[m][n][r] = 0.f;

  const int x_lane = (G == 2 ? kq * XW : kq * dil) * 16;
  const int x_step = (G == 2 ? dil : 2 * dil) * 16;

  if (first) __syncthreads();
  if constexpr (NMW == 4) {
    constexpr int S = H / 2;
    auto pipeline = [&](auto MBc) {
    constexpr int MBv = decltype(MBc)::value;
    bf16x8 A[2][MBv][3], Bf[2][NB][3];
    auto ld = [&](int buf, int st, bf16x8 (&Ad)[MBv][3], bf16x8 (&Bd)[NB][3]) {
      const unsigned char* Wb = Wbuf + buf * STG + (kq * CO + l31) * 16;
      const unsigned char* Xb = Xbuf + buf * STG + (n0 + l31) * 16 + x_lane + st * x_step;
      constexpr int PO[3] = {1, 0, 2};
#pragma unroll
      for (int pi = 0; pi < 3; ++pi) {
#pragma unroll
        for (int n = 0; n < NB; ++n) Bd[n][PO[pi]] = *reinterpret_cast<const bf16x8*>(Xb + (PO[pi] * G * XW + n * 32) * 16);
#pragma unroll
        for (int m = 0; m < MBv; ++m) Ad[m][PO[pi]] = *reinterpret_cast<const bf16x8*>(Wb + ((PO[pi] * H + 2 * st) * CO + m * 32) * 16);
      }
    };
    auto mma = [&](const bf16x8 (&Ac)[MBv][3], const bf16x8 (&Bc)[NB][3]) {
      constexpr int TA[6] = {1, 2, 0, 1, 0, 0}, TB[6] = {1, 0, 2, 0, 1, 0};
#pragma unroll
      for (int q = 0; q < 6; ++q)
#pragma unroll
        for (int m = 0; m < MBv; ++m)
#pragma unroll
          for (int n = 0; n < NB; ++n) acc[m][n] = __builtin_amdgcn_mfma_f32_32x32x16_bf16(Ac[m][TA[q]], Bc[n][TB[q]], acc[m][n], 0, 0, 0);
    };
    auto interleave = [&]() {
#pragma unroll
      for (int i = 0; i < 3 * (MBv + NB); ++i) {
        __builtin_amdgcn_sched_group_barrier(0x008, (6 * MBv * NB) / (3 * (MBv + NB)) > 0 ? (6 * MBv * NB) / (3 * (MBv + NB)) : 1, 0);
        __builtin_amdgcn_sched_group_barrier(0x100, 1, 0);
      }
    };
    ld(0, 0, A[0], Bf[0]);
    for (int base = 0; base < n_chunks; base += 2) {
#pragma unroll
      for (int cc = 0; cc < 2; ++cc) {
        const int chunk = base + cc;
        if (chunk >= n_chunks) break;
        const int buf = cc;
#pragma unroll
        for (int st = 0; st < S; ++st) {
          const int cur = (cc * S + st) & 1;
          if (st + 1 < S) {
            if (cur == 0) ld(buf, st + 1, A[1], Bf[1]); else ld(buf, st + 1, A[0], Bf[0]);
            if (cur == 0) mma(A[0], Bf[0]); else mma(A[1], Bf[1]);
            interleave();
            __builtin_amdgcn_sched_barrier(0);
          } else {
            asm volatile("s_waitcnt lgkmcnt(0)" ::: "memory");
            __builtin_amdgcn_s_barrier();
            asm volatile("" ::: "memory");
            __builtin_amdgcn_sched_barrier(0);
            if (chunk + 1 < n_chunks) {
              if (cur == 0) ld(buf ^ 1, 0, A[1], Bf[1]); else ld(buf ^ 1, 0, A[0], Bf[0]);
            }
            if (cur == 0) mma(A[0], Bf[0]); else mma(A[1], Bf[1]);
            if (chunk + 1 < n_chunks) interleave();
            __builtin_amdgcn_sched_barrier(0);
          }
        }
      }
    }
    };
    if (MB == 2 && co0 + 32 >= a.C_out) pipeline(std::integral_constant<int, 1>{});
    else pipeline(std::integral_constant<int, MB>{});
  } else {
  for (int chunk = 0; chunk < n_chunks; ++chunk) {
    const int buf = chunk & 1;
    const unsigned char* Wb = Wbuf + buf * STG + (kq * CO + l31) * 16;
    const unsigned char* Xb = Xbuf + buf * STG + (n0 + l31) * 16 + x_lane;
    bf16x8 A[2][MB][3], Bf[1][NB][3];
    auto ldA = [&](int st, bf16x8 (&Ad)[MB][3]) {
#pragma unroll
      for (int p = 0; p < 3; ++p)
#pragma unroll
        for (int m = 0; m < MB; ++m)
          Ad[m][p] = *reinterpret_cast<const bf16x8*>(Wb + ((p * H + 2 * st) * CO + m * 32) * 16);
    };
    auto ldB = [&](int st, bf16x8 (&Bd)[NB][3]) {
      const int xo = st * x_step;
      constexpr int PO[3] = {1, 0, 2};
#pragma unroll
      for (int pi = 0; pi < 3; ++pi)
#pragma unroll
        for (int n = 0; n < NB; ++n)
          Bd[n][PO[pi]] = *reinterpret_cast<const bf16x8*>(Xb + xo + (PO[pi] * G * XW + n * 32) * 16);
    };
#pragma unroll
    for (int st = 0; st < H / 2; ++st) {
      ldB(st, Bf[0]);
      ldA(st, A[0]);
      __builtin_amdgcn_sched_barrier(0);
      constexpr int TA[6] = {1, 2, 0, 1, 0, 0}, TB[6] = {1, 0, 2, 0, 1, 0};
#pragma unroll
      for (int q = 0; q < 6; ++q)
#pragma unroll
        for (int m = 0; m < MB; ++m)
#pragma unroll
          for (int n = 0; n < NB; ++n)
            acc[m][n] = __builtin_amdgcn_mfma_f32_32x32x16_bf16(A[0][m][TA[q]], Bf[0][n][TB[q]], acc[m][n], 0, 0, 0);
      __builtin_amdgcn_sched_barrier(0);
    }
    __syncthreads();
  }
  }
  __builtin_amdgcn_s_setprio(0);
  {
    float* tile = reinterpret_cast<float*>(epi_base);
    constexpr int EP = BS_TT + 4;
    if constexpr (MB == 3) {
      int lane_off = 4 * kq * EP + n0 + l31;
      asm volatile("" : "+v"(lane_off));
      tile += lane_off;
#pragma unroll
      for (int m = 0; m < MB; ++m)
#pragma unroll
        for (int n = 0; n < NB; ++n)
#pragma unroll
          for (int r = 0; r < 16; ++r) tile[(m * 32 + (r & 3) + 8 * (r >> 2)) * EP + n * 32] = acc[m][n][r];
    } else
#pragma unroll
    for (int m = 0; m < MB; ++m)
#pragma unroll
      for (int n = 0; n < NB; ++n)
#pragma unroll
        for (int r = 0; r < 16; ++r)
          tile[(m * 32 + (r & 3) + 8 * (r >> 2) + 4 * kq) * EP + n0 + n * 32 + l31] = acc[m][n][r];
  }
  }
  __syncthreads();

  {
    const KArgP e = fresh_args();
    const float* tile = reinterpret_cast<const float*>(epi_base);
    constexpr int EP = BS_TT + 4;
    constexpr int NTH = (NMW + NSW) * 64;
    constexpr int QPR = BS_TT / 4;
    float* yg = e->y ? e->y + (long long)b * e->y_bs : nullptr;
    float* y2g = e->y2 ? e->y2 + (long long)b * e->y_bs : nullptr;
    const float* rg = e->res ? e->res + (long long)b * e->y_bs : nullptr;
    const bool vec_ok = (e->y_cs & 3) == 0 && (e->y_bs & 3) == 0 && (!yg || (reinterpret_cast<unsigned long long>(e->y) & 15) == 0) &&
                        (!y2g || (reinterpret_cast<unsigned long long>(e->y2) & 15) == 0) &&
                        (!rg || (reinterpret_cast<unsigned long long>(e->res) & 15) == 0);
    for (int q = tid; q < CO * QPR; q += NTH) {
      const int row = q / QPR, tq = q - row * QPR;
      const int co = co0 + row, t = t0 + 4 * tq;
      if (co >= e->C_out || t >= e->T_out) continue;
      const float4 av = *reinterpret_cast<const float4*>(tile + row * EP + 4 * tq);
      float v[4] = {av.x, av.y, av.z, av.w};
      const float bs = e->bias ? e->bias[co] : 0.f;
      const float al = e->alpha_out ? e->alpha_out[co] : 0.f;
      const float inv = e->alpha_out ? snake_inv(al) : 0.f;
      const long long o = (long long)co * e->y_cs + t;
      const bool full = vec_ok && t + 3 < e->T_out;
      float rv[4] = {0.f, 0.f, 0.f, 0.f};
      if (rg) {
        if (full) {
          const float4 r4 = *reinterpret_cast<const float4*>(rg + o);
          rv[0] = r4.x; rv[1] = r4.y; rv[2] = r4.z; rv[3] = r4.w;
        } else {
#pragma unroll
          for (int i = 0; i < 4; ++i) rv[i] = t + i < e->T_out ? rg[o + i] : 0.f;
        }
      }
#pragma unroll
      for (int i = 0; i < 4; ++i) {
        float x = v[i] + bs;
        if (e->alpha_out) x = snake_apply(x, al, inv);
        if (e->act != FAC_ACT_NONE) x = apply_act_slow(x, e->act);
        v[i] = x + rv[i];
      }
      float w[4];
      if (y2g) {
        const float a2 = e->alpha2[co], i2 = snake_inv(a2);
#pragma unroll
        for (int i = 0; i < 4; ++i) w[i] = snake_apply(v[i], a2, i2);
      }
      if (full) {
        if (yg) *reinterpret_cast<float4*>(yg + o) = make_float4(v[0], v[1], v[2], v[3]);
        if (y2g) *reinterpret_cast<float4*>(y2g + o) = make_float4(w[0], w[1], w[2], w[3]);
      } else {
#pragma unroll
        for (int i = 0; i < 4; ++i) {
          if (t + i >= e->T_out) continue;
          if (yg) yg[o + i] = v[i];
          if (y2g) y2g[o + i] = w[i];
        }
      }
    }
  }
  first = !overlap;
  if (vb + (int)gridDim.x < n_tiles) __syncthreads();
  }
  };
  if (wave >= NMW) {
    if constexpr (WIDE) {
      if (a.x_p8 != nullptr) walk(std::integral_constant<int, 2>{});
      else walk(std::integral_constant<int, 1>{});
    } else {
      walk(std::integral_constant<int, 1>{});
    }
  } else {
    walk(std::integral_constant<int, 0>{});
  }
}

template <int KT, int G, int NMW, int NSW, int MB = 2>
static int bsplit_launch(ConvArgs& a, hipStream_t s) {
  constexpr int H = bs_slots(KT, G), TT = 64 * NMW, CO = 32 * MB;
  a.XW = TT + (H / G - 1) * a.dil;
  const size_t stg = (size_t)3 * H * CO * 16 + (size_t)48 * G * a.XW;
  const size_t epi = (size_t)CO * (TT + 4) * sizeof(float);
  a.n_t_tiles = (a.T_out + TT - 1) / TT;
  const long long n_wg = (long long)a.n_t_tiles * ((a.C_out + CO - 1) / CO) * a.B;
  if (n_wg > 0x7fffffffll) {
    set_error("conv1d: too many workgroups (%lld)", n_wg);
    return FAC_ERR_ARG;
  }
  const int n_chunks = (a.C_in + 8 * G - 1) / (8 * G);
  int cus = device_cus() & ~7;
  a.persist = (NMW == 4 && a.x_p8 == nullptr && n_chunks % 2 == 0 && cus >= 8 && n_wg > cus &&
               stg + (stg > epi ? stg : epi) <= FAC_LDS_MAX) ? 1 : 0;
  size_t lds = a.persist ? stg + (stg > epi ? stg : epi) : (2 * stg > epi ? 2 * stg : epi);
  if (lds > FAC_LDS_MAX) {
    set_error("conv1d(bf16 split): tile needs %zu B of LDS (dil=%d)", lds, a.dil);
    return FAC_ERR_ARG;
  }
  constexpr auto kern = conv1d_bsplit_kernel<KT, G, NMW, NSW, MB>;
  allow_dynamic_lds<kern>();
  a.n_tiles = (int)n_wg;
  hipLaunchKernelGGL(kern, dim3((unsigned)(a.persist ? cus : n_wg)), dim3((NMW + NSW) * 64), lds, s, a);
  return check_launch("conv1d_bsplit");
}

}
```

facodec_amd/csrc/conv1d_mfma.h:

```cpp
#pragma once
#include "common.h"

namespace fac {

typedef __attribute__((address_space(3))) void lds_void_t;
typedef __attribute__((address_space(1))) const void glb_void_t;

constexpr int CONV_XMAX = 6;

struct ConvArgs {
  const float* x;
  const float* w;
  const float* bias;
  const float* alpha_in;
  const float* alpha_out;
  const float* res;
  float* y;
  float* y2;
  const float* alpha2;
  const float* w1;
  const float* bias1;
  long long x_bs, x_cs, y_bs, y_cs, w_bs;
  int B, C_in, T_in, T_ext, C_out, C_out_pad, T_out;
  int K, stride, dil, pad_left, pad_mode;
  int n_phase, y_tstride, act, w_batched;
  int phase_shift;
  int K1, dil2;
  int K2v, KV, CV;
  int cic;
  int XW;
  int XB;
  int XQ, XR;
  int n_t_tiles;
  int n_tiles, persist;
  int x_off;
  int gflat;
  int grt;
  const unsigned char* x_p8;
  long long x_p8_ps;
  unsigned char* y2_p8;
  long long y2_p8_ps;
  int rp;
  const float* gate_cond;
  long long gate_cond_bs;
};

__host__ __device__ inline int conv_max_tap_offset(const ConvArgs& a) {
  const int K1 = (a.K1 > 0 && a.K1 < a.K) ? a.K1 : a.K;
  return (a.K / K1 - 1) * a.dil2 + (K1 - 1) * a.dil;
}
__host__ __device__ inline bool conv_two_level(const ConvArgs& a) { return a.K1 > 0 && a.K1 < a.K; }
inline void conv_set_virtual(ConvArgs& a) {
  a.KV = conv_two_level(a) ? a.K1 : a.K;
  a.K2v = a.K / a.KV;
  a.CV = a.C_in * a.K2v;
}

template <int KT>
struct ConvUnroll {
  static constexpr int UC = (KT == 1) ? 4 : ((KT == 2 || KT == 3) ? 2 : 1);
  static constexpr int CIC = KT == 1 ? 24 : (KT == 2 || KT == 3) ? 16 : (KT >= 4 && KT <= 7) ? 8 : (KT > 7 ? 4 : 0);
};

template <int KT, int T_TILE>
constexpr int conv_cic() {
  return ((KT == 2 || KT == 3) && T_TILE >= 256) ? 8 : ConvUnroll<KT>::CIC;
}

constexpr int CONV_WPE = 4;
template <int MB, int NB, int WM, int WN, int KT, bool FUSE = false>
__global__ __launch_bounds__((WM * WN + 4) * 64, (WM * WN == 4 ? CONV_WPE : 3)) void conv1d_mfma_kernel(ConvArgs a) {
  constexpr int NMW = WM * WN;
  constexpr int CO_TILE = 32 * MB * WM;
  constexpr int T_TILE = 32 * NB * WN;
  constexpr int CO4 = CO_TILE / 4;
  constexpr bool ALLW = (WM * WN == 8) && !FUSE;
  extern __shared__ __attribute__((aligned(16))) float smem[];

  const int tid = threadIdx.x;
  const int lane = tid & 63;
  const int wave = __builtin_amdgcn_readfirstlane(tid >> 6);

  int t0, co0, b, phase;
  {
    const int id = xcd_contiguous_id<unsigned>(blockIdx.x, gridDim.x);
    const int nt = a.n_t_tiles, nbp = a.B * a.n_phase;
    const int tt = id % nt;
    const int rest = id / nt;
    const int bp = rest % nbp;
    const int ct = rest / nbp;
    t0 = tt * T_TILE;
    co0 = ct * CO_TILE;
    b = bp / a.n_phase;
    phase = bp - b * a.n_phase;
  }
  int y_off = phase - a.phase_shift, tap_shift = 0;
  if (y_off < 0) {
    y_off += a.n_phase;
    tap_shift = 1;
  }

  const int K = KT > 0 ? KT : a.KV;
  const int cic = KT > 0 ? conv_cic<KT, T_TILE>() : a.cic;
  const int XW = a.XW, XB = a.XB;
  const int w_stage = cic * K * CO_TILE;
  const int x_stage = cic * XW;
  float* Wbuf = smem;
  float* Xbuf = smem + 2 * w_stage;
  const int n_chunks = (a.CV + cic - 1) / cic;

  if (wave >= NMW) {
    const int lw = wave - NMW;
    __builtin_amdgcn_s_setprio(3);
    const float* xg = a.x + (long long)b * a.x_bs;
    const int w_rows_total = cin_pad_dev(a.C_in) * a.K;
    const float* wg = a.w + (long long)phase * w_rows_total * a.C_out_pad +
                      (a.w_batched ? (long long)b * a.w_bs : 0ll);
    const int tin0 = t0 * a.stride - a.pad_left - a.x_off;
    const bool vec_ok = ((a.x_cs | a.x_bs) & 3) == 0 && ((reinterpret_cast<unsigned long long>(a.x) & 15) == 0);
    const int r_first = lw / XB, cb_first = lw - r_first * XB;
    const int K2v = a.K2v, dil2 = a.dil2;
    const bool x_dma = a.alpha_in == nullptr && vec_ok && tin0 >= 0 && tin0 + (K2v - 1) * dil2 + XW <= a.T_in &&
                       (K2v == 1 || (dil2 & 3) == 0);

    auto stage = [&](int chunk, int buf) {
      {
        const int n4 = cic * K * CO4;
        const int row_base = chunk * cic * K;
        float* dst0 = Wbuf + buf * w_stage;
        for (int i = lw; i * 64 < n4; i += 4) {
          const int q = i * 64 + lane;
          if (q < n4) {
            const int row = q / CO4;
            const int c4 = q - row * CO4;
            int grow = row_base + row;
            grow = grow < w_rows_total ? grow : w_rows_total - 1;
            int co = co0 + 4 * c4;
            co = co < a.C_out_pad ? co : a.C_out_pad - 4;
            const float* src = wg + (long long)grow * a.C_out_pad + co;
            __builtin_amdgcn_global_load_lds((glb_void_t*)src, (lds_void_t*)(dst0 + i * 256), 16, 0, 0);
          }
        }
      }
      const int ci0 = chunk * cic;
      const int XW4 = XW >> 2;
      if (x_dma) {
        float* dst = Xbuf + buf * x_stage;
        for (int it = lw; it < cic * XB; it += 4) {
          const int r = it / XB;
          const int c4 = (it - r * XB) * 64 + lane;
          if (c4 < XW4) {
            int v = ci0 + r;
            v = v < a.CV ? v : a.CV - 1;
            const int ci = v / K2v, k2 = v - ci * K2v;
            const float* src = xg + (long long)ci * a.x_cs + tin0 + k2 * dil2 + 4 * c4;
            __builtin_amdgcn_global_load_lds((glb_void_t*)src, (lds_void_t*)(dst + r * XW + (it - r * XB) * 256), 16, 0, 0);
          }
        }
        return;
      }
      float4 xr[CONV_XMAX];
      float xal[CONV_XMAX];
      {
        int r = r_first, cb = cb_first;
#pragma unroll
        for (int j = 0; j < CONV_XMAX; ++j) {
          float4 v = make_float4(0.f, 0.f, 0.f, 0.f);
          float al = 0.f;
          const int c4 = cb * 64 + lane;
          const int vch = ci0 + r;
          const int ci = vch / K2v, k2 = vch - ci * K2v;
          if (r < cic && c4 < XW4 && vch < a.CV) {
            const int tin = tin0 + 4 * c4 + k2 * dil2;
            const float* xrow = xg + (long long)ci * a.x_cs;
            if (vec_ok && (tin & 3) == 0 && tin >= 0 && tin + 3 < a.T_in) {
              v = *reinterpret_cast<const float4*>(xrow + tin);
            } else {
              float e[4];
#pragma unroll
              for (int u = 0; u < 4; ++u) {
                int idx;
                if (a.pad_mode == FAC_PAD_REFLECT) idx = reflect_index(tin + u, a.T_in, a.T_ext);
                else idx = (tin + u >= 0 && tin + u < a.T_in) ? tin + u : -1;
                e[u] = idx >= 0 ? xrow[idx] : 0.f;
              }
              v = make_float4(e[0], e[1], e[2], e[3]);
            }
            if (a.alpha_in != nullptr) al = a.alpha_in[ci];
          }
          xr[j] = v;
          xal[j] = al;
          r += a.XQ;
          cb += a.XR;
          if (cb >= XB) { cb -= XB; ++r; }
        }
      }
// ... 273 lines not shown
        if (y2g) {
          const float a2 = a.alpha2[co], i2 = snake_inv(a2);
#pragma unroll
          for (int i = 0; i < 4; ++i) w[i] = snake_apply(v[i], a2, i2);
        }
        if (full) {
          if (yg) *reinterpret_cast<float4*>(yg + o) = make_float4(v[0], v[1], v[2], v[3]);
          if (y2g) *reinterpret_cast<float4*>(y2g + o) = make_float4(w[0], w[1], w[2], w[3]);
        } else {
#pragma unroll
          for (int i = 0; i < 4; ++i) {
            if (u + i >= T_tot) continue;
            if (yg) yg[o + i] = v[i];
            if (y2g) y2g[o + i] = w[i];
          }
        }
      }
    } else
    for (int q = tid; q < CO_TILE * QPR; q += NTH) {
      const int row = q / QPR, tq = q - row * QPR;
      const int co = co0 + row, t = t0 + 4 * tq;
      if (co >= a.C_out || t >= a.T_out) continue;
      const float4 av = *reinterpret_cast<const float4*>(smem + row * EP + 4 * tq);
      float v[4] = {av.x, av.y, av.z, av.w};
      const float bs = a.bias ? a.bias[co] : 0.f;
      const float al = a.alpha_out ? a.alpha_out[co] : 0.f;
      const float inv = a.alpha_out ? snake_inv(al) : 0.f;
      const long long o = (long long)co * a.y_cs + (long long)t * a.y_tstride + y_off;
      const bool full = vec_ok && t + 3 < a.T_out;
      float rv[4] = {0.f, 0.f, 0.f, 0.f};
      if (rg) {
        if (full) {
          const float4 r4 = *reinterpret_cast<const float4*>(rg + o);
          rv[0] = r4.x; rv[1] = r4.y; rv[2] = r4.z; rv[3] = r4.w;
        } else {
#pragma unroll
          for (int i = 0; i < 4; ++i) rv[i] = t + i < a.T_out ? rg[o + (long long)i * a.y_tstride] : 0.f;
        }
      }
#pragma unroll
      for (int i = 0; i < 4; ++i) {
        float x = v[i] + bs;
        if (a.alpha_out) x = snake_apply(x, al, inv);
        if (a.act != FAC_ACT_NONE) x = apply_act_slow(x, a.act);
        v[i] = x + rv[i];
      }
      float w[4] = {0.f, 0.f, 0.f, 0.f};
      if (y2g) {
        const float a2 = a.alpha2[co], i2 = snake_inv(a2);
#pragma unroll
        for (int i = 0; i < 4; ++i) w[i] = snake_apply(v[i], a2, i2);
      }
      if (full) {
        if (yg) *reinterpret_cast<float4*>(yg + o) = make_float4(v[0], v[1], v[2], v[3]);
        if (y2g) *reinterpret_cast<float4*>(y2g + o) = make_float4(w[0], w[1], w[2], w[3]);
      } else {
#pragma unroll
        for (int i = 0; i < 4; ++i) {
          if (t + i >= a.T_out) continue;
          if (yg) yg[o + (long long)i * a.y_tstride] = v[i];
          if (y2g) y2g[o + (long long)i * a.y_tstride] = w[i];
        }
      }
    }
  }
}

template <int MB, int NB, int WM, int WN, int KT, bool FUSE = false>
int launch_cfg(ConvArgs& a, hipStream_t s) {
  constexpr int CO_TILE = 32 * MB * WM;
  constexpr int T_TILE = 32 * NB * WN;
  constexpr int UC = ConvUnroll<KT>::UC;
  constexpr int STEP = 2 * UC;
  a.x_off = ((-a.pad_left) % 4 + 4) % 4;
  a.XW = (((T_TILE - 1) * a.stride + (a.KV - 1) * a.dil + 1 + a.x_off + (a.phase_shift > 0 ? 1 : 0)) + 3) & ~3;
  a.XB = (a.XW / 4 + 63) / 64;
  a.XQ = 4 / a.XB;
  a.XR = 4 % a.XB;
  const int per_ci = a.KV * CO_TILE + a.XW;
  int cic;
  if constexpr (KT > 0) {
    cic = conv_cic<KT, T_TILE>();
    if (cic * a.XB > 4 * CONV_XMAX || (size_t)2 * cic * per_ci * sizeof(float) > (WM * WN == 4 ? 80 : 160) * 1024)
      return launch_cfg<MB, NB, WM, WN, 0, FUSE>(a, s);
  } else {
    int lim = 9216 / per_ci;
    const int lim_regs = (4 * CONV_XMAX) / a.XB;
    if (lim > lim_regs) lim = lim_regs;
    if (lim > 32) lim = 32;
    lim = (lim / STEP) * STEP;
    if (lim < STEP) lim = STEP;
    const int cin_r = ((a.CV + STEP - 1) / STEP) * STEP;
    cic = lim < cin_r ? lim : cin_r;
    for (int c = cic; c >= STEP && c * 2 > cic; c -= STEP)
      if (cin_r % c == 0) { cic = c; break; }
    if (cic * a.XB > 4 * CONV_XMAX) {
      set_error("conv1d: receptive field too wide to stage (K=%d stride=%d dil=%d)", a.K, a.stride, a.dil);
      return FAC_ERR_ARG;
    }
  }
  a.cic = cic;
  size_t lds = (size_t)2 * cic * per_ci * sizeof(float);
  if constexpr ((WM * WN == 8) && !FUSE) {
    const size_t epi = (size_t)CO_TILE * (T_TILE + 4) * sizeof(float);
    if (lds < epi) lds = epi;
  }
  if (lds > FAC_LDS_MAX) {
    set_error("conv1d: tile needs %zu B of LDS (K=%d stride=%d dil=%d)", lds, a.K, a.stride, a.dil);
    return FAC_ERR_ARG;
  }
  constexpr auto kern = conv1d_mfma_kernel<MB, NB, WM, WN, KT, FUSE>;
  allow_dynamic_lds<kern>();
  a.n_t_tiles = (a.T_out + T_TILE - 1) / T_TILE;
  if (a.rp > 1 && !((WM * WN == 8) && !FUSE && CO_TILE == 128)) {
    set_error("conv1d: row_phases needs the 128-row all-waves-epilogue tile");
    return FAC_ERR_ARG;
  }
  const int n_co_tiles = a.rp > 1 ? a.C_out_pad / CO_TILE : (a.C_out + CO_TILE - 1) / CO_TILE;
  const long long n_wg = (long long)a.n_t_tiles * n_co_tiles * a.B * a.n_phase;
  if (n_wg > 0x7fffffffll) {
    set_error("conv1d: too many workgroups (%lld)", n_wg);
    return FAC_ERR_ARG;
  }
  hipLaunchKernelGGL(kern, dim3((unsigned)n_wg), dim3((WM * WN + 4) * 64), lds, s, a);
  return check_launch("conv1d_mfma");
}

int conv_dispatch_128x128(ConvArgs& a, hipStream_t s);
int conv_dispatch_96x128(ConvArgs& a, hipStream_t s);
int conv_dispatch_64x128(ConvArgs& a, hipStream_t s);
int conv_dispatch_32x256(ConvArgs& a, hipStream_t s);
int conv_dispatch_128x32(ConvArgs& a, hipStream_t s);
int conv_dispatch_128x256(ConvArgs& a, hipStream_t s);
int conv_dispatch_96x256(ConvArgs& a, hipStream_t s);
int conv_dispatch_fused_ru(ConvArgs& a, hipStream_t s);
int conv_dispatch_128x160(ConvArgs& a, hipStream_t s);
int conv_dispatch_narrow(ConvArgs& a, hipStream_t s);
bool conv_cin1_ok(const ConvArgs& a);
bool conv_pw_ok(const ConvArgs& a);
int conv_dispatch_pw(ConvArgs& a, hipStream_t s);
bool conv_thin_ok(const ConvArgs& a, const void* ws, long long ws_bytes);
int conv_dispatch_thin(ConvArgs& a, void* ws, hipStream_t s);
int conv_dispatch_cin1(ConvArgs& a, hipStream_t s);
bool conv_bsplit2_ok(const ConvArgs& a);
int conv_dispatch_bsplit2(ConvArgs& a, hipStream_t s);
bool conv_gsplit_ok(const ConvArgs& a);
int conv_dispatch_gsplit(ConvArgs& a, hipStream_t s);
bool conv_bsplit_ok(const ConvArgs& a);
bool conv_bsplit_p8_ok(const ConvArgs& a);
int conv_dispatch_bsplit(ConvArgs& a, hipStream_t s);
bool conv_bsplit96_ok(const ConvArgs& a);
bool conv_bsplit96_p8_ok(const ConvArgs& a);
int conv_dispatch_bsplit96(ConvArgs& a, hipStream_t s);
bool conv_pws_ok(const ConvArgs& a);
int conv_dispatch_pws(ConvArgs& a, hipStream_t s);
bool conv_pwt_ok(const ConvArgs& a);
int conv_dispatch_pwt(ConvArgs& a, hipStream_t s);
bool conv_skinny_ok(const ConvArgs& a, const void* ws, long long ws_bytes);
bool conv_skinny_single_launch(const ConvArgs& a);
int conv_dispatch_skinny(ConvArgs& a, void* ws, long long ws_bytes, hipStream_t s);

}
```

facodec_amd/csrc/prep_batch.h:

```cpp
#pragma once
#include "common.h"

namespace fac {

struct PrepJob {
  const void* a;
  const void* b;
  void* out;
  long long n;
  long long l[3];
  int kind;
  int nblocks;
  int i[8];
};

enum PrepUnit { PU_PACK = 0, PU_BSPLIT, PU_GSPLIT, PU_BSPLIT2, PU_BWD, PU_COUNT };

enum PrepKind {
  PK_WN_SCALE = 0, PK_CONV, PK_CONVTR, PK_CONVTR_ROWS, PK_FLIP_T,
  PK_CONV_SPLIT,
  PK_GEMM_SPLIT,
  PK_CONV_SPLIT2,
  PK_CONV_BWD
};

bool prep_recording();
int prep_record(int unit, const PrepJob& j);

int prep_launch_pack(const PrepJob* jobs, const int* first, int njobs, int total, hipStream_t s);
int prep_launch_bsplit(const PrepJob* jobs, const int* first, int njobs, int total, hipStream_t s);
int prep_launch_gsplit(const PrepJob* jobs, const int* first, int njobs, int total, hipStream_t s);
int prep_launch_bsplit2(const PrepJob* jobs, const int* first, int njobs, int total, hipStream_t s);
int prep_launch_bwd(const PrepJob* jobs, const int* first, int njobs, int total, hipStream_t s);

inline int prep_blocks(long long n) { return (int)((n + 255) / 256 < 65535 ? (n + 255) / 256 : 65535); }

__device__ __forceinline__ int prep_find_job(const int* __restrict__ first, int njobs, int b) {
  int lo = 0, hi = njobs - 1;
  while (lo < hi) {
    const int mid = (lo + hi + 1) >> 1;
    if (first[mid] <= b) lo = mid; else hi = mid - 1;
  }
  return lo;
}

}
```

facodec_amd/dac_model.py:

```python
from torch import nn

from . import autograd as A
from . import ops
from .wprep import cached_forward
from .layers import SConv1d, SConvTranspose1d, SLSTM, Snake1d

FUSED_RU_CHANNELS = (64,)


class ResidualUnit(nn.Module):

    def __init__(self, dim=16, dilation=1, causal=False):
        super().__init__()
        self.block = nn.Sequential(
            Snake1d(dim),
            SConv1d(dim, dim, kernel_size=7, dilation=dilation, causal=causal, norm="weight_norm"),
            Snake1d(dim),
            SConv1d(dim, dim, kernel_size=1, causal=causal, norm="weight_norm"),
        )

    @property
    def alpha_in(self):
        return self.block[0].flat()

    def run(self, x, x_act, alpha_next=None, want_raw=True):
        b = self.block
        k7, k1 = b[1], b[3]
        streaming = ops.BF16_SPLIT and x.shape[0] * ((x.shape[-1] + 31) // 32) >= 8192
        if k7.w.c_out in FUSED_RU_CHANNELS and x_act.shape[-1] == x.shape[-1] and not streaming:
            return_pair = ops.conv1d(x_act, k7.w.packed(), k7.w.c_out, 7, bias=k7.w.bias, dilation=k7.dilation,
                                     alpha_out=b[2].flat(), res=x, w_k1=k1.w.packed(), bias_k1=k1.w.bias,
                                     alpha_y2=alpha_next, want_y=want_raw or alpha_next is None, causal=k7.causal)
            return return_pair if alpha_next is not None else (return_pair, None)
        h = b[1].run(x_act, alpha_out=b[2].flat())
        if h.shape[-1] != x.shape[-1]:
            pad = (x.shape[-1] - h.shape[-1]) // 2
            x = x[..., pad:-pad].contiguous()
        if alpha_next is None:
            return b[3].run(h, res=x), None
        return b[3].run(h, res=x, alpha_y2=alpha_next, want_y=want_raw)

    def forward(self, x):
        if self.training:
            b = self.block
            y = A.conv(b[3], A.snake(b[2], A.conv(b[1], A.snake(b[0], x))))
            return A.add(x, y)
        return self.run(x, ops.snake(x, self.alpha_in))[0]


def _run_units(units, x, x_act, alpha_after):
    for j, ru in enumerate(units):
        last = j == len(units) - 1
        nxt = alpha_after if last else units[j + 1].alpha_in
        x, x_act = ru.run(x, x_act, alpha_next=nxt, want_raw=not last)
    return x_act


class EncoderBlock(nn.Module):

    def __init__(self, dim=16, stride=1, causal=False):
        super().__init__()
        self.block = nn.Sequential(
            ResidualUnit(dim // 2, dilation=1, causal=causal),
            ResidualUnit(dim // 2, dilation=3, causal=causal),
            ResidualUnit(dim // 2, dilation=9, causal=causal),
            Snake1d(dim // 2),
            SConv1d(dim // 2, dim, kernel_size=2 * stride, stride=stride, causal=causal, norm="weight_norm"),
        )

    @property
    def alpha_in(self):
        return self.block[0].alpha_in

    def run(self, x, x_act, alpha_next=None):
        b = self.block
        z_act = _run_units([b[0], b[1], b[2]], x, x_act, b[3].flat())
        return b[4].run(z_act, alpha_y2=alpha_next) if alpha_next is not None else (b[4].run(z_act), None)

    def forward(self, x):
        return self.run(x, ops.snake(x, self.alpha_in))[0]


class Encoder(nn.Module):

    def __init__(self, d_model=64, strides=(2, 4, 8, 8), d_latent=64, causal=False, lstm=2):
        super().__init__()
        layers = [SConv1d(1, d_model, kernel_size=7, causal=causal, norm="weight_norm")]
        for s in strides:
            d_model *= 2
            layers.append(EncoderBlock(d_model, stride=s, causal=causal))
        self.use_lstm = lstm
        if lstm:
            layers.append(SLSTM(d_model, lstm))
        layers += [Snake1d(d_model), SConv1d(d_model, d_latent, kernel_size=3, causal=causal, norm="weight_norm")]
        self.block = nn.Sequential(*layers)
        self.enc_dim = d_model
        self.boundary_hook = None

    def _forward_train(self, x):
        mods = list(self.block)
        x = A.conv(mods[0], x)
        for m in mods[1:-2]:
            if self.boundary_hook is not None:
                self.boundary_hook(m, x)
            if isinstance(m, EncoderBlock):
                b = m.block
                x, xa = A.snake_dual(x, b[0].block[0].alpha)
                for j in range(3):
                    nxt = b[j + 1].block[0].alpha if j < 2 else b[3].alpha
                    x, xa = A.res_unit(b[j], x, xa, nxt)
                x = A.conv(b[4], xa)
            else:
                x = A.slstm(m, x)
        return A.conv(mods[-1], A.snake(mods[-2], x))

    @cached_forward
    def forward(self, x):
        if self.training:
            return self._forward_train(x)
        mods = list(self.block)
        blocks = [m for m in mods if isinstance(m, EncoderBlock)]
        final_alpha = mods[-2].flat()
        x, x_act = mods[0].run(x, alpha_y2=blocks[0].alpha_in)
        for i, blk in enumerate(blocks):
            if i + 1 < len(blocks):
                nxt = blocks[i + 1].alpha_in
            else:
                nxt = None if self.use_lstm else final_alpha
            x, x_act = blk.run(x, x_act, alpha_next=nxt)
        if self.use_lstm:
            x_act = mods[-3](x, alpha_out=final_alpha)
        return mods[-1].run(x_act)


class DecoderBlock(nn.Module):

    def __init__(self, input_dim=16, output_dim=8, stride=1, causal=False):
        super().__init__()
        self.block = nn.Sequential(
            Snake1d(input_dim),
            SConvTranspose1d(input_dim, output_dim, kernel_size=2 * stride, stride=stride, causal=causal,
                             norm="weight_norm"),
            ResidualUnit(output_dim, dilation=1, causal=causal),
            ResidualUnit(output_dim, dilation=3, causal=causal),
            ResidualUnit(output_dim, dilation=9, causal=causal),
        )

    @property
    def alpha_in(self):
        return self.block[0].flat()

    def run(self, x_act, alpha_after):
        b = self.block
        y, y_act = b[1].run(x_act, alpha_y2=b[2].alpha_in)
        return _run_units([b[2], b[3], b[4]], y, y_act, alpha_after)

    def forward(self, x):
        raise NotImplementedError("DecoderBlock is executed through Decoder.forward's fused plan")


class Decoder(nn.Module):

    def __init__(self, input_channel, channels, rates, d_out=1, causal=False, lstm=2):
        super().__init__()
        layers = [SConv1d(input_channel, channels, kernel_size=7, causal=causal, norm="weight_norm")]
        self.use_lstm = lstm
        if lstm:
            layers.append(SLSTM(channels, num_layers=lstm))
        out_dim = channels
        for i, s in enumerate(rates):
            in_dim, out_dim = channels // 2 ** i, channels // 2 ** (i + 1)
            layers.append(DecoderBlock(in_dim, out_dim, s, causal=causal))
        layers += [Snake1d(out_dim), SConv1d(out_dim, d_out, kernel_size=7, causal=causal, norm="weight_norm"),
                   nn.Tanh()]
        self.model = nn.Sequential(*layers)
        self.boundary_hook = None

    def _forward_train(self, x):
        mods = list(self.model)
        blocks = [m for m in mods if isinstance(m, DecoderBlock)]
        x = A.conv(mods[0], x)
# ... 36 lines not shown
```

facodec_amd/layers.py:

```python
import math

import torch
from torch import nn

from . import ops


def _uniform_(t, bound):
    with torch.no_grad():
        return t.uniform_(-bound, bound)


class ConvWeights(nn.Module):

    def __init__(self, c_in, c_out, k, weight_norm=True, transposed=False, stride=1, bias=True):
        super().__init__()
        self.c_in, self.c_out, self.k = c_in, c_out, k
        self.transposed, self.stride, self.weight_norm = transposed, stride, weight_norm
        shape = (c_in, c_out, k) if transposed else (c_out, c_in, k)
        fan_in = (c_out if transposed else c_in) * k
        w = _uniform_(torch.empty(shape), 1.0 / math.sqrt(fan_in))
        if weight_norm:
            self.weight_g = nn.Parameter(w.reshape(shape[0], -1).norm(dim=1).reshape(shape[0], 1, 1))
            self.weight_v = nn.Parameter(w)
        else:
            self.weight = nn.Parameter(w)
        self.bias = nn.Parameter(_uniform_(torch.empty(c_out), 1.0 / math.sqrt(fan_in))) if bias else None
        self._packed = None
        self._split = None
        self._rows = None
        self._rows_split = None
        self.freeze_packed = False

    def _vg(self):
        return (self.weight_v.detach(), self.weight_g.detach()) if self.weight_norm else (self.weight.detach(), None)

    def _cached(self, slot, pack, *a, **kw):
        cur = getattr(self, slot)
        if cur is None or not self.freeze_packed:
            cur = pack(*self._vg(), *a, out=cur[0] if isinstance(cur, tuple) else cur, **kw)
            setattr(self, slot, cur)
        return cur

    def packed(self):
        if self.transposed:
            return self._cached("_packed", ops.pack_convtr_weight, self.stride)
        return self._cached("_packed", ops.pack_conv_weight)

    def packed_rows(self):
        return self._cached("_rows", ops.pack_convtr_weight_rows, self.stride)

    def packed_rows_split(self):
        return self._cached("_rows_split", ops.pack_convtr_weight_rows_split, self.stride)

    def packed_split_strided(self, stride):
        return self._cached("_split", ops.pack_gemm_weight_split, in_stride=stride)

    def packed_split(self, rows=64):
        return self._cached("_split", ops.pack_conv_weight_split, rows=rows)

    def _apply(self, fn, *a, **kw):
        self._packed = None
        self._split = None
        self._rows = None
        self._rows_split = None
        return super()._apply(fn, *a, **kw)


class _Norm(nn.Module):

    def __init__(self, name, weights):
        super().__init__()
        setattr(self, name, weights)


FLAT_SHORT_CLIPS = True
FLAT_STRIDE1 = True


class SConv1d(nn.Module):

    def __init__(self, in_channels, out_channels, kernel_size, stride=1, dilation=1, causal=False,
                 norm="none", pad_mode="reflect", bias=True):
        super().__init__()
        self.conv = _Norm("conv", ConvWeights(in_channels, out_channels, kernel_size, norm == "weight_norm", bias=bias))
        self.kernel_size, self.stride, self.dilation = kernel_size, stride, dilation
        self.causal = causal
        self.pad_mode = ops.PAD_REFLECT if pad_mode == "reflect" else ops.PAD_ZERO

    @property
    def w(self):
        return self.conv.conv

    def plan(self, B, T, alpha_in=False, plain=True, res=False):
        return ops.plan_conv(self.w.c_out, self.w.c_in, self.kernel_size, self.stride, self.dilation, B, T, -(-T // self.stride),
                             alpha_in=alpha_in, plain=plain, res=res, causal_reflect=self.causal and self.pad_mode == ops.PAD_REFLECT,
                             grad=torch.is_grad_enabled(), c_out_mult16=False, tail="always", flat_infer=FLAT_SHORT_CLIPS,
                             flat_stride1=FLAT_STRIDE1)

    def run(self, x, alpha_in=None, alpha_out=None, res=None, act=ops.ACT_NONE, alpha_y2=None, want_y=True):
        w, k, s_ = self.w, self.kernel_size, self.stride
        B, _, T = x.shape
        plan = self.plan(B, T, alpha_in is not None, alpha_out is None and res is None and act == ops.ACT_NONE, res is not None)
        split = (w.packed_split_strided(s_) if plan.layout == ops.W_GEMM_STRIDED
                 else w.packed_split(ops.tile_rows(w.c_out, w.c_in, k)) if plan.layout == ops.W_TAPS
                 else w.packed_split() if plan.layout == ops.W_GEMM else None)
        if plan.form != ops.PER_CLIP:
            P = (k - 1) * self.dilation + 1 - s_
            return ops.conv1d_flat(torch.nn.functional.pad(x, (P, 0), mode="reflect"), split, w.c_out, k, s_, T // s_,
                                   dilation=self.dilation, bias=w.bias, p8=plan.p8, alpha_out=alpha_out, act=act, alpha_y2=alpha_y2,
                                   want_y=want_y)
        x = ops.p8_prepass(x, plan.p8)
        return ops.conv1d(x, w.packed() if split is None else None, w.c_out, k, bias=w.bias,
                          stride=s_, dilation=self.dilation, pad_mode=self.pad_mode, alpha_in=alpha_in,
                          alpha_out=alpha_out, res=res, act=act, causal=self.causal, alpha_y2=alpha_y2, want_y=want_y,
                          w_split=split)

    def forward(self, x):
        return self.run(x)


class SConvTranspose1d(nn.Module):

    def __init__(self, in_channels, out_channels, kernel_size, stride=1, causal=False, norm="none"):
        super().__init__()
        self.convtr = _Norm("convtr", ConvWeights(in_channels, out_channels, kernel_size, norm == "weight_norm",
                                                  transposed=True, stride=stride))
        self.stride = stride
        self.causal = causal

    @property
    def w(self):
        return self.convtr.convtr

    def plan(self, B, T, alpha_in=False):
        return ops.plan_convtr(self.w.c_in, self.w.c_out, self.stride, B, T, causal=self.causal, alpha_in=alpha_in,
                               grad=torch.is_grad_enabled(), flat_infer=FLAT_SHORT_CLIPS)

    def run(self, x, alpha_in=None, alpha_y2=None):
        w = self.w
        B, c_in, T = x.shape
        plan = self.plan(B, T, alpha_in is not None)
        if plan.layout == ops.TR_FLAT:
            xz = torch.cat([torch.zeros(B, c_in, 1, device=x.device, dtype=x.dtype), x], -1)
            return ops.conv_transpose1d_flat(xz, w.packed_rows_split(), w.c_out, self.stride, trim=self.stride, bias=w.bias,
                                             alpha_y2=alpha_y2, p8=plan.p8)
        wp = (w.packed_rows_split() if plan.layout == ops.TR_ROWS_SPLIT
              else w.packed() if plan.layout == ops.TR_POLYPHASE else w.packed_rows())
        return ops.conv_transpose1d(ops.p8_prepass(x, plan.p8), wp, w.c_out, self.stride, bias=w.bias, alpha_in=alpha_in,
                                    alpha_y2=alpha_y2, causal=self.causal)

    def forward(self, x):
        return self.run(x)


class Snake1d(nn.Module):

    def __init__(self, channels):
        super().__init__()
        self.alpha = nn.Parameter(torch.ones(1, channels, 1))

    def flat(self):
        return self.alpha.detach().reshape(-1)

    def forward(self, x):
        return ops.snake(x, self.flat())


class _LSTMParams(nn.Module):

    def __init__(self, hidden, num_layers):
        super().__init__()
        b = 1.0 / math.sqrt(hidden)
        for l in range(num_layers):
            for n, shp in (("weight_ih", (4 * hidden, hidden)), ("weight_hh", (4 * hidden, hidden)),
                           ("bias_ih", (4 * hidden,)), ("bias_hh", (4 * hidden,))):
                setattr(self, f"{n}_l{l}", nn.Parameter(_uniform_(torch.empty(shp), b)))


class SLSTM(nn.Module):

    def __init__(self, dimension, num_layers=2, skip=True):
        super().__init__()
        self.lstm = _LSTMParams(dimension, num_layers)
        self.dimension, self.num_layers, self.skip = dimension, num_layers, skip

    def forward(self, x, alpha_out=None):
        B, H, T = x.shape
        inp = ops.lstm_to_time_major(x)
        for l in range(self.num_layers):
            p = self.lstm
            w_raw = getattr(p, f"weight_ih_l{l}").detach()
            bias = ops.add(getattr(p, f"bias_ih_l{l}").detach(), getattr(p, f"bias_hh_l{l}").detach())
            w_hh = getattr(p, f"weight_hh_l{l}").detach()
            persist = ops.lstm_persist_ok(H, B)
            T_, BP = inp.shape[1], inp.shape[2]
            with ops.flop_scale(B / BP):
                pre = ops.lstm_input_proj(inp, w_raw, bias)
                if ops.lstm_persist_split_ok(H, B, T_):
                    inp = ops.lstm_layer_persist_split(pre, w_hh, H, B)
                elif persist:
                    inp = ops.lstm_layer_persist(pre, w_hh, H, B)
                else:
                    inp = ops.lstm_layer(pre, ops.pack_lstm_whh(w_hh), H)
        return ops.lstm_from_time_major(inp, x if self.skip else None, B, alpha_out)
```

facodec_amd/ops.py:

```python
import ctypes as C
import math
import os
from collections import namedtuple

import torch

from . import _lib
from .wprep import prepared
from .convplan import *
from ._lib import ConvDesc, VqDesc, VqDecodeDesc, ResampleDesc, PAD_REFLECT, PAD_ZERO, ACT_NONE, ACT_TANH, ACT_MISH, ACT_LOG_MEL, ACT_GATE, ACT_WN_RES_SKIP


def pad32(n):
    return (n + 31) & ~31


def cin_pad(c):
    return ((c + 47) // 48) * 48


_RAW_STREAM = getattr(torch._C, "_cuda_getCurrentRawStream", None)
_GET_DEVICE = getattr(torch._C, "_cuda_getDevice", None)


# ... 21 lines not shown

def _ptr(t):
    return C.c_void_p(t.data_ptr()) if t is not None else C.c_void_p(0)


def _dev(t, what="tensor"):
    if t is None:
        return None
    if not t.is_cuda:
        raise _lib.FacodecHipError(f"{what} must live on the GPU (got {t.device}); there is no CPU path")
    if t.dtype != torch.float32:
        raise _lib.FacodecHipError(f"{what} must be float32 (got {t.dtype})")
    return t if t.is_contiguous() else t.contiguous()


@prepared
def wn_scale(v, g, out=None):
    v = _dev(v, "weight_v")
    g = _dev(g, "weight_g")
    n = v.shape[0]
    scale = out if out is not None else torch.empty(n, device=v.device, dtype=torch.float32)
    _lib.check(_lib.load().fac_wn_scale(_ptr(v), _ptr(g), _ptr(scale), n, v.numel() // n, _stream()), "fac_wn_scale")
    return scale


@prepared
def pack_conv_weight(v, g=None, out=None, scale=None):
    v = _dev(v, "weight")
    if v.dim() == 2:
        v = v.unsqueeze(-1)
    c_out, c_in, k = v.shape
    cp = pad32(c_out)
    if scale is None and g is not None:
        scale = wn_scale(v, g)
    if out is None:
        out = torch.empty(cin_pad(c_in), k, cp, device=v.device, dtype=torch.float32)
    _lib.check(_lib.load().fac_pack_conv_w(_ptr(v), _ptr(scale), _ptr(out), c_out, c_in, k, cp, _stream()),
               "fac_pack_conv_w")
    return out


@prepared
def pack_convtr_weight(v, g, stride, out=None):
    v = _dev(v, "weight")
    c_in, c_out, k = v.shape
    if k != 2 * stride:
        raise _lib.FacodecHipError(f"polyphase ConvTranspose1d needs kernel_size == 2*stride (got {k}, {stride})")
    cp = pad32(c_out)
    scale = wn_scale(v, g) if g is not None else None
    if out is None:
        out = torch.empty(stride, cin_pad(c_in), 2, cp, device=v.device, dtype=torch.float32)
    _lib.check(_lib.load().fac_pack_convtr_w(_ptr(v), _ptr(scale), _ptr(out), c_in, c_out, stride, cp, _stream()),
               "fac_pack_convtr_w")
    return out


CONVTR_ROWS = False
CONVTR_ROWS_MIN_T = 512


def convtr_rows_pad(c_out, stride):
    cpt = 128 // stride
    return -(-c_out // cpt) * 128


@prepared
def pack_convtr_weight_rows(v, g, stride, out=None):
    v = _dev(v, "weight")
    c_in, c_out, k = v.shape
    if k != 2 * stride:
        raise _lib.FacodecHipError(f"ConvTranspose1d needs kernel_size == 2*stride (got {k}, {stride})")
    scale = wn_scale(v, g) if g is not None else None
    if out is None:
        out = torch.empty(cin_pad(c_in), 2, convtr_rows_pad(c_out, stride), device=v.device, dtype=torch.float32)
    _lib.check(_lib.load().fac_pack_convtr_w_rows(_ptr(v), _ptr(scale), _ptr(out), c_in, c_out, stride, _stream()),
               "fac_pack_convtr_w_rows")
    return out


class ConvLaunchProfile:

    def __init__(self):
        self.records = []

    def summary(self):
        out = {}
        for name, flops, e0, e1 in self.records:
            r = out.setdefault(name, dict(launches=0, flops=0.0, ms=0.0))
            r["launches"] += 1
            r["flops"] += flops
            r["ms"] += e0.elapsed_time(e1)
        return out


_PROFILE = None


class FlopCounter:

    def __init__(self):
        self.flops = dict(conv=0.0, wgrad=0.0, lstm=0.0, dft=0.0)
        self.launches = dict(conv=0, wgrad=0, lstm=0, dft=0)

    def add(self, key, f):
        self.flops[key] += f * _FLOP_SCALE
        self.launches[key] += 1

    @property
    def total(self):
        return sum(v for k, v in self.flops.items() if k != "dft")


_FLOPS = None
_FLOP_SCALE = 1.0


def set_flop_counter(c):
    global _FLOPS
    _FLOPS = c


_FLOP_KEY = "conv"


class flop_key:

    def __init__(self, key):
        self.key = key

    def __enter__(self):
        global _FLOP_KEY
        self.prev, _FLOP_KEY = _FLOP_KEY, self.key

    def __exit__(self, *a):
        global _FLOP_KEY
        _FLOP_KEY = self.prev


class flop_scale:

    def __init__(self, s):
        self.s = s

    def __enter__(self):
        global _FLOP_SCALE
        self.prev, _FLOP_SCALE = _FLOP_SCALE, self.s

    def __exit__(self, *a):
        global _FLOP_SCALE
        _FLOP_SCALE = self.prev

BF16_SPLIT = True
BS_ROWS96 = (96,)


def set_conv_profile(p):
    global _PROFILE
    _PROFILE = p


_CONV_WS = {}
CONV_WS_BYTES = 32 << 20


_STREAM_SLOTS = {}


def register_stream_slot(stream):
    key = stream.cuda_stream
    if key not in _STREAM_SLOTS:
        _STREAM_SLOTS[key] = len(_STREAM_SLOTS) + 1
    return _STREAM_SLOTS[key]


_SIDE_STREAMS = {}


def side_streams(device, n):
    key = (device, n)
    if key not in _SIDE_STREAMS:
        _SIDE_STREAMS[key] = [torch.cuda.Stream(device=device) for _ in range(n)]
        for st in _SIDE_STREAMS[key]:
            register_stream_slot(st)
    return _SIDE_STREAMS[key]


def join_side_streams(device):
    if device.type != "cuda":
        return
    cur = torch.cuda.current_stream(device)
    for (dev, _), streams in _SIDE_STREAMS.items():
        if dev.type == "cuda" and (dev.index is None or device.index is None or dev.index == device.index):
            for st in streams:
                if st != cur:
                    cur.wait_stream(st)


def run_chains(chains, device, n_streams, inputs=()):
    n = min(n_streams, len(chains))
    if n <= 1 or device.type != "cuda":
        return [c() for c in chains]
    main = torch.cuda.current_stream(device)
    streams = side_streams(device, n)
    for st in streams:
        st.wait_stream(main)
        _record_stream(inputs, st)
    outs = []
    for j, c in enumerate(chains):
        with torch.cuda.stream(streams[j % n]):
            outs.append(c())
    for st in streams:
        main.wait_stream(st)
    _record_stream(outs, main)
    return outs


def _record_stream(obj, stream):
    if torch.is_tensor(obj):
        if obj.is_cuda:
            obj.record_stream(stream)
    elif isinstance(obj, (list, tuple)):
        for o in obj:
            _record_stream(o, stream)
    elif isinstance(obj, dict):
        for o in obj.values():
            _record_stream(o, stream)


_CUDA_DEVICES = {}


def _cuda_device(index):
    d = _CUDA_DEVICES.get(index)
    if d is None:
        d = _CUDA_DEVICES[index] = torch.device("cuda", index)
    return d


def _conv_workspace(device):
    slot = _STREAM_SLOTS.get(_raw_stream(device.index), 0) if _STREAM_SLOTS else 0
    key = (device, slot)
    ws = _CONV_WS.get(key)
    if ws is None:
        ws = _CONV_WS[key] = torch.zeros(CONV_WS_BYTES // 4, device=device, dtype=torch.float32)
    return ws


def conv_variant(d):
    buf = C.create_string_buffer(96)
    return _lib.load().fac_conv1d_variant(C.byref(d), buf, 96), buf.value.decode()


def _launch_conv(d, what):
    lib = _lib.load()
    ws = _conv_workspace(_cuda_device(_GET_DEVICE() if _GET_DEVICE is not None else torch.cuda.current_device()))
    d.ws, d.ws_bytes = ws.data_ptr(), CONV_WS_BYTES
    if _FLOPS is not None or _PROFILE is not None:
        flops = 2.0 * d.B * d.n_phase * max(1, d.row_phases) * d.C_out * d.T_out * d.C_in * d.K
        if d.w_k1:
            flops += 2.0 * d.B * d.C_out * d.T_out * d.C_out
    if _FLOPS is not None:
        _FLOPS.add(_FLOP_KEY, flops)
    if _PROFILE is None:
        _lib.check(lib.fac_conv1d_fwd(C.byref(d), _stream()), what)
        return
    name = conv_variant(d)[1][:63]
    e0, e1 = torch.cuda.Event(enable_timing=True), torch.cuda.Event(enable_timing=True)
    e0.record()
    _lib.check(lib.fac_conv1d_fwd(C.byref(d), _stream()), what)
    e1.record()
    _PROFILE.records.append((name, flops, e0, e1))


GEMM_SPLIT_MIN_CIN = 256


@prepared
def pack_gemm_weight_split(v, g=None, out=None, in_stride=1, scale=None):
    v = _dev(v, "weight")
    if v.dim() == 2:
        v = v.unsqueeze(-1)
    c_out, c_in, k = v.shape
    lib = _lib.load()
    if scale is None and g is not None:
        scale = wn_scale(v, g)
    nbytes = lib.fac_gemm_w_split_bytes(c_out, c_in, k, in_stride)
    if out is None:
        out = torch.empty(nbytes, device=v.device, dtype=torch.uint8)
    _lib.check(lib.fac_pack_gemm_w_split(_ptr(v), c_in * k, k, 1, _ptr(scale), out.data_ptr(), c_out, c_in, k, in_stride, _stream()),
               "fac_pack_gemm_w_split")
    return out


def pack_gemm_weight_split_t(w, out=None):
    w = _dev(w, "weight")
    if w.dim() == 2:
        w = w.unsqueeze(-1)
    c_out, c_in, k = w.shape
    assert k == 1
    lib = _lib.load()
    nbytes = lib.fac_gemm_w_split_bytes(c_in, c_out, 1, 1)
    if out is None:
        out = torch.empty(nbytes, device=w.device, dtype=torch.uint8)
    _lib.check(lib.fac_pack_gemm_w_split(_ptr(w), 1, c_in, 1, None, out.data_ptr(), c_in, c_out, 1, 1, _stream()),
               "fac_pack_gemm_w_split(transposed)")
    return out


@prepared
def pack_conv_weight_split2(v, g=None, k1=0, out=None, scale=None):
    v = _dev(v, "weight")
    c_out, c_in, k = v.shape
    lib = _lib.load()
    if scale is None and g is not None:
        scale = wn_scale(v, g)
    nbytes = lib.fac_conv_w_split2_bytes(c_out, c_in, k, k1)
    if out is None:
        out = torch.empty(nbytes, device=v.device, dtype=torch.uint8)
    _lib.check(lib.fac_pack_conv_w_split2(_ptr(v), _ptr(scale), out.data_ptr(), c_out, c_in, k, k1, _stream()),
               "fac_pack_conv_w_split2")
    return out


@prepared
def pack_convtr_weight_rows_split(v, g, stride, out=None):
    rows = pack_convtr_weight_rows(v, g, stride)
    cip, _, R = rows.shape
    c_in = v.shape[0]
    lib = _lib.load()
    nbytes = lib.fac_gemm_w_split_bytes(R, c_in, 2, 1)
    if out is None:
        out = torch.empty(nbytes, device=v.device, dtype=torch.uint8)
    _lib.check(lib.fac_pack_gemm_w_split(_ptr(rows), 1, 2 * R, R, None, out.data_ptr(), R, c_in, 2, 1, _stream()),
               "fac_pack_gemm_w_split(convtr rows)")
    return out, R


@prepared
def pack_conv_weight_split(v, g=None, out=None, scale=None, rows=None):
    v = _dev(v, "weight")
    c_out, c_in, k = v.shape
    if k <= 2:
        return pack_gemm_weight_split(v, g, out=out, scale=scale)
    lib = _lib.load()
    if scale is None and g is not None:
        scale = wn_scale(v, g)
    if rows is None:
        rows = tile_rows(c_out, c_in, k)
    nbytes = lib.fac_conv_w_split_rows_bytes(c_out, c_in, k, rows)
    if nbytes < 0:
        raise _lib.FacodecHipError("pack_conv_weight_split: no %d-row tile for k = %d" % (rows, k))
    if out is None or out.numel() != nbytes:
        out = torch.empty(nbytes, device=v.device, dtype=torch.uint8)
    _lib.check(lib.fac_pack_conv_w_split_rows(_ptr(v), _ptr(scale), out.data_ptr(), c_out, c_in, k, rows, _stream()),
               "fac_pack_conv_w_split_rows")
    out.split_rows = rows
    return out


def conv_out_len(t_in, k, stride, dilation):
    k_eff = (k - 1) * dilation + 1
    padding_total = k_eff - stride
    n_frames = (t_in - k_eff + padding_total) / stride + 1
    ideal = (math.ceil(n_frames) - 1) * stride + (k_eff - padding_total)
    extra = ideal - t_in
    t_out = (t_in + padding_total + extra - k_eff) // stride + 1
    return t_out, padding_total, extra


class P8:

    def __init__(self, planes, shape):
        self.planes, self.shape = planes, tuple(shape)

    @staticmethod
    def empty(B, C, T, device):
        return P8(torch.empty(3, B * (C // 8) * T + 1, 8, device=device, dtype=torch.bfloat16), (B, C, T))

    @property
    def plane_bytes(self):
        return self.planes.stride(0) * 2

    def to_float(self):
        B, C, T = self.shape
        v = self.planes[:, :-1].float().sum(0).reshape(B, C // 8, T, 8)
        return v.permute(0, 1, 3, 2).reshape(B, C, T).contiguous()


def to_p8(x, alpha=None):
    x = _dev(x, "x")
    B, C, T = x.shape
    out = P8.empty(B, C, T, x.device)
    _lib.check(_lib.load().fac_to_p8(_ptr(x), _ptr(alpha), _ptr(out.planes), B, C, T, _stream()), "fac_to_p8")
    return out


P8_PREPASS_MIN_FLOP_PER_BYTE = 450.0


def p8_prepass(x, flop_per_in_byte):
    if (flop_per_in_byte is None or P8_PREPASS_MIN_FLOP_PER_BYTE <= 0 or flop_per_in_byte < P8_PREPASS_MIN_FLOP_PER_BYTE or not BF16_SPLIT or isinstance(x, P8)
            or torch.is_grad_enabled() or not x.is_cuda or x.shape[1] % 8 != 0 or x.shape[0] * (x.shape[1] // 8) * x.shape[2] * 16 >= (1 << 32)):
        return x
    return to_p8(x)


def conv_y_channels(c_out, act):
    return c_out // 2 if act in (ACT_GATE, ACT_WN_RES_SKIP) else c_out


def conv_desc(B, c_in, t_in, c_out, k, stride=1, dilation=1, pad_left=None, pad_mode=PAD_REFLECT, t_out=None, act=ACT_NONE, causal=True,
              k1=0, dilation2=0, c_out_pad=None, split_rows=0):
    if pad_left is None:
        t_o, padding_total, _ = conv_out_len(t_in, k, stride, dilation)
        pad_left = padding_total if causal else padding_total - padding_total // 2
        if t_out is None:
            t_out = t_o
    if t_out is None:
        raise ValueError("t_out required with explicit pad_left")
    d = ConvDesc()
    d.x_bs, d.x_cs = c_in * t_in, t_in
    d.y_bs, d.y_cs = conv_y_channels(c_out, act) * t_out, t_out
    d.B, d.C_in, d.T_in, d.C_out, d.C_out_pad, d.T_out = B, c_in, t_in, c_out, (pad32(c_out) if c_out_pad is None else c_out_pad), t_out
    d.K, d.stride, d.dilation, d.pad_left, d.pad_mode = k, stride, dilation, pad_left, pad_mode
    d.n_phase, d.y_tstride, d.act, d.w_batched, d.w_bs = 1, 1, act, 0, 0
    d.K1, d.dilation2, d.split_rows = k1, dilation2, split_rows
    d.pw_split = 1 if (BF16_SPLIT and PW_SPLIT and (k == 1 or (PW_TAPS and k == 4 and stride == 2))) else 0
    return d


def conv1d(x, w_packed, c_out, k, bias=None, stride=1, dilation=1, pad_left=None, pad_mode=PAD_REFLECT,
           t_out=None, alpha_in=None, alpha_out=None, res=None, act=ACT_NONE, out=None, causal=True,
           alpha_y2=None, want_y=True, w_k1=None, bias_k1=None, w_split=None, k1=0, dilation2=0, skip_acc=None, gate_cond=None):
    x_p8 = x if isinstance(x, P8) else None
    if x_p8 is not None:
        B, c_in, t_in = x_p8.shape
    else:
        if not (x.is_cuda and x.dtype == torch.float32 and x.dim() == 3 and x.stride(2) == 1):
            x = _dev(x, "x")
        B, c_in, t_in = x.shape
    dev_ = x_p8.planes.device if x_p8 is not None else x.device
    d = conv_desc(B, c_in, t_in, c_out, k, stride, dilation, pad_left, pad_mode, t_out, act, causal, k1, dilation2,
                  w_packed.shape[-1] if w_packed is not None else None,
                  getattr(w_split, "split_rows", 0))
    t_out, c_y = d.T_out, conv_y_channels(c_out, act)
    if out is None and want_y:
        out = torch.empty(B, c_y, t_out, device=dev_, dtype=torch.float32)
    y2 = torch.empty(B, c_out, t_out, device=dev_, dtype=torch.float32) if alpha_y2 is not None else None
    if act == ACT_WN_RES_SKIP:
        assert skip_acc is not None and skip_acc.is_contiguous() and skip_acc.shape == out.shape and alpha_y2 is None
        y2 = skip_acc
    res = _dev(res, "res")
    d.bias = bias.data_ptr() if bias is not None else None
    if x_p8 is not None:
        d.x, d.x_p8, d.x_p8_plane_bytes = None, x_p8.planes.data_ptr(), x_p8.plane_bytes
    else:
        d.x = x.data_ptr()
        d.x_bs, d.x_cs = x.stride(0), x.stride(1)
    d.w = w_packed.data_ptr() if w_packed is not None else w_split.data_ptr()
    d.alpha_in = alpha_in.data_ptr() if alpha_in is not None else None
    d.alpha_out = alpha_out.data_ptr() if alpha_out is not None else None
    d.res = res.data_ptr() if res is not None else None
    d.y = out.data_ptr() if out is not None else None
    d.y2 = y2.data_ptr() if y2 is not None else None
    d.alpha_y2 = alpha_y2.data_ptr() if alpha_y2 is not None else None
    d.w_k1 = w_k1.data_ptr() if w_k1 is not None else None
    d.bias_k1 = bias_k1.data_ptr() if bias_k1 is not None else None
    d.w_split = w_split.data_ptr() if w_split is not None else None
    if out is not None and (out.stride(0), out.stride(1)) != (d.y_bs, d.y_cs) and out.shape[0] * out.shape[1] > 1:
        assert out.stride(2) == 1 and y2 is None and res is None and out.shape == (B, c_y, t_out)
        d.y_bs, d.y_cs = out.stride(0), out.stride(1)
    if gate_cond is not None:
        if not (gate_cond.is_cuda and gate_cond.dtype == torch.float32 and gate_cond.dim() == 2 and gate_cond.shape == (B, c_out)
                and (gate_cond.stride(1) == 1 or c_out == 1)):
            raise ValueError(f"gate_cond must be a float32 GPU tensor (B={B}, c_out={c_out}) with contiguous rows, "
                             f"got {tuple(gate_cond.shape)} {gate_cond.dtype} {gate_cond.device}")
        d.gate_cond, d.gate_cond_bs = gate_cond.data_ptr(), gate_cond.stride(0)
    _launch_conv(d, "fac_conv1d_fwd")
    return (out, y2) if alpha_y2 is not None else out


STREAM_FOLD = True
SKINNY_MAX_COLS = 640


def convtr_desc(B, c_in, t_in, c_out, stride, c_out_pad, causal=True, has_history=False, rows=False, split=False):
    t_cols = t_in - 1 if has_history else t_in
    t_total = t_cols * stride
    d = ConvDesc()
    d.x_bs, d.x_cs = c_in * t_in, t_in
    d.y_bs, d.y_cs = c_out * t_total, t_total
    d.B, d.C_in, d.T_in, d.C_out, d.C_out_pad, d.T_out = B, c_in, t_in, c_out, c_out_pad, t_cols
    d.K, d.stride, d.dilation, d.pad_left, d.pad_mode = 2, 1, 1, (0 if has_history else 1), PAD_ZERO
    d.n_phase, d.y_tstride, d.act, d.w_batched, d.w_bs = stride, stride, ACT_NONE, 0, 0
    d.phase_shift = 0 if causal else stride - stride // 2
    if rows or split:
        if not causal or has_history:
            raise _lib.FacodecHipError("the all-phases ConvTranspose1d launch is causal and offline only")
        d.n_phase, d.y_tstride, d.phase_shift, d.row_phases = 1, 1, 0, stride
        d.pw_split = 1 if (BF16_SPLIT and PW_SPLIT and PW_TAPS and not split and stride == 2) else 0
    return d


def conv_transpose1d(x, w_packed, c_out, stride, bias=None, alpha_in=None, out=None, alpha_y2=None, causal=True,
                     has_history=False):
    x_p8 = x if isinstance(x, P8) else None
    if x_p8 is not None:
        assert not has_history
        B, c_in, t_in = x_p8.shape
    else:
        if not (has_history and x.is_cuda and x.dtype == torch.float32 and x.stride(2) == 1):
            x = _dev(x, "x")
        B, c_in, t_in = x.shape
    dev_ = x_p8.planes.device if x_p8 is not None else x.device
    if has_history:
        assert causal
    split_rows = isinstance(w_packed, tuple)
    d = convtr_desc(B, c_in, t_in, c_out, stride, w_packed[1] if split_rows else w_packed.shape[-1], causal, has_history,
                    not split_rows and w_packed.dim() == 3, split_rows)
    if out is None:
        out = torch.empty(B, c_out, d.T_out * stride, device=dev_, dtype=torch.float32)
    d.bias = bias.data_ptr() if bias is not None else None
    if x_p8 is not None:
        d.x, d.x_p8, d.x_p8_plane_bytes = None, x_p8.planes.data_ptr(), x_p8.plane_bytes
    else:
        d.x = x.data_ptr()
        d.x_bs, d.x_cs = x.stride(0), x.stride(1)
    if split_rows:
        d.w, d.w_split = None, w_packed[0].data_ptr()
    else:
        d.w = w_packed.data_ptr()
    d.alpha_in = alpha_in.data_ptr() if alpha_in is not None else None
    d.alpha_out, d.res, d.y = None, None, out.data_ptr()
    y2 = torch.empty_like(out) if alpha_y2 is not None else None
    d.y2 = y2.data_ptr() if y2 is not None else None
    d.alpha_y2 = alpha_y2.data_ptr() if alpha_y2 is not None else None
    _launch_conv(d, "fac_conv1d_fwd(convtr)")
    return (out, y2) if alpha_y2 is not None else out


FLAT_TRAIN = True
PW_SPLIT = os.environ.get("FAC_PW_SPLIT", "1") != "0"
PW_TAPS = True


def pack_conv_for(layout, v, g, stride=1, k1=0, scale=None):
    if layout in (W_FP32, W_FP32_PW_TAPS):
        return pack_conv_weight(v, g, scale=scale), None
    if layout == W_GEMM_STRIDED:
        return None, pack_gemm_weight_split(v, g, in_stride=stride, scale=scale)
    if layout == W_SPLIT2:
        return None, pack_conv_weight_split2(v, g, k1, scale=scale)
    return None, pack_conv_weight_split(v, g, scale=scale, rows=64)


def pack_convtr_for(layout, v, g, stride):
    if layout in (TR_ROWS_SPLIT, TR_FLAT):
        return pack_convtr_weight_rows_split(v, g, stride)
    return pack_convtr_weight(v, g, stride) if layout == TR_POLYPHASE else pack_convtr_weight_rows(v, g, stride)


def convtr_weight_for(v, g, stride, t_in, causal=True, batch=1, alpha_in=None):
    return pack_convtr_for(plan_convtr(v.shape[0], v.shape[1], stride, batch, t_in, causal=causal, alpha_in=alpha_in is not None).layout,
                           v, g, stride)


def flat_conv_cols(B, L, s, n):
    pitch = L // s
    return pitch, B * L, B * pitch - (pitch - n)


def flat_convtr_cols(B, T1):
    return B * T1


def conv1d_flat(xp, w_split, c_out, k, s, n, dilation=1, bias=None, p8=None, alpha_out=None, act=ACT_NONE, alpha_y2=None, want_y=True):
    B, c_in, L = xp.shape
    pitch, t_in, t_out = flat_conv_cols(B, L, s, n)
    xf = p8_prepass(xp.permute(1, 0, 2).reshape(1, c_in, t_in), p8)
    got = conv1d(xf, None, c_out, k, bias=bias, stride=s, dilation=dilation, pad_left=0, pad_mode=PAD_ZERO, t_out=t_out,
                 alpha_out=alpha_out, act=act, alpha_y2=alpha_y2, want_y=want_y, w_split=w_split)

    def back(y):
        if y is None:
            return None
        full = torch.empty(c_out, B * pitch, device=y.device, dtype=y.dtype)
        full[:, :t_out] = y[0]
        return full.reshape(c_out, B, pitch)[:, :, :n].permute(1, 0, 2).contiguous()

    return (back(got[0]), back(got[1])) if alpha_y2 is not None else back(got)


def conv_transpose1d_flat(xz, w_rows_split, c_out, s, trim=0, bias=None, alpha_y2=None, p8=None):
    B, c_in, T1 = xz.shape
    xf = p8_prepass(xz.permute(1, 0, 2).reshape(1, c_in, flat_convtr_cols(B, T1)), p8)
    got = conv_transpose1d(xf, w_rows_split, c_out, s, bias=bias, alpha_y2=alpha_y2, causal=True)
    back = lambda y: y.reshape(c_out, B, T1 * s)[:, :, trim:].permute(1, 0, 2).contiguous()
    return (back(got[0]), back(got[1])) if alpha_y2 is not None else back(got)


def snake(x, alpha, out=None):
    x = _dev(x, "x")
    B, c, t = x.shape
    if out is None:
        out = torch.empty_like(x)
    _lib.check(_lib.load().fac_snake_fwd(_ptr(x), _ptr(alpha), _ptr(out), B, c, t, _stream()), "fac_snake_fwd")
    return out


def lstm_to_time_major(x):
    x = _dev(x, "x")
    B, H, T = x.shape
    xT = torch.empty(H, T, pad32(B), device=x.device, dtype=torch.float32)
    _lib.check(_lib.load().fac_lstm_to_time_major(_ptr(x), _ptr(xT), B, H, T, _stream()), "fac_lstm_to_time_major")
    return xT


def lstm_from_time_major(yT, skip, B, alpha=None):
    H, T, BP = yT.shape
    out = torch.empty(B, H, T, device=yT.device, dtype=torch.float32)
    _lib.check(_lib.load().fac_lstm_from_time_major(_ptr(yT), _ptr(skip), _ptr(alpha), _ptr(out), B, H, T, _stream()),
# ... 944 lines not shown
```

include/facodec_hip.h:

```cpp
#ifndef FACODEC_HIP_H
#define FACODEC_HIP_H

#include <stdint.h>

#ifdef __cplusplus
extern "C" {
#endif

typedef void* fac_stream_t;

#define FAC_OK 0
#define FAC_ERR_ARG (-1)
#define FAC_ERR_LAUNCH (-2)

#define FAC_PAD_ZERO 0
#define FAC_PAD_REFLECT 1

#define FAC_ACT_NONE 0
#define FAC_ACT_TANH 1
#define FAC_ACT_MISH 2
#define FAC_ACT_LOG_MEL 3
#define FAC_ACT_GATE 4
#define FAC_ACT_WN_RES_SKIP 5

int fac_version(void);
const char* fac_last_error(void);


int fac_wn_scale(const float* v, const float* g, float* scale, int n_slices, int slice_len,
                 fac_stream_t stream);

int fac_pack_conv_w(const float* v, const float* scale, float* packed, int C_out, int C_in,
                    int K, int C_out_pad, fac_stream_t stream);

int fac_pack_convtr_w(const float* v, const float* scale, float* packed, int C_in, int C_out,
                      int stride, int C_out_pad, fac_stream_t stream);

static inline int fac_convtr_rows(int C_out, int stride) {
  const int cpt = 128 / stride;
  return ((C_out + cpt - 1) / cpt) * 128;
}
int fac_pack_convtr_w_rows(const float* v, const float* scale, float* packed, int C_in, int C_out, int stride,
                           fac_stream_t stream);

#define FAC_CONV_WS_BYTES (32ll << 20)

typedef struct fac_conv_desc {
  const float* x;
  const float* w;
  const float* bias;
  const float* alpha_in;
  const float* alpha_out;
  const float* res;
  float* y;
  float* y2;
  const float* alpha_y2;
  const float* w_k1;
  const float* bias_k1;
  int64_t x_bs, x_cs;
  int64_t y_bs, y_cs;
  int32_t B, C_in, T_in, C_out, C_out_pad;
  int32_t T_out;
  int32_t K, stride, dilation, pad_left, pad_mode;
  int32_t n_phase;
  int32_t y_tstride;
  int32_t phase_shift;
  int32_t act;
  int32_t w_batched;
  int64_t w_bs;
  void* ws;
  int64_t ws_bytes;
  const void* w_split;
  int32_t K1, dilation2;
  int32_t row_phases;
  const void* x_p8;
  int64_t x_p8_plane_bytes;
  void* y2_p8;
  int64_t y2_p8_plane_bytes;
  int32_t pw_split;
  int32_t split_rows;
  const float* gate_cond;
  int64_t gate_cond_bs;
} fac_conv_desc;

int fac_conv1d_fwd(const fac_conv_desc* d, fac_stream_t stream);
int fac_to_p8(const float* x, const float* alpha, void* out, int B, int C, int T, fac_stream_t stream);
int64_t fac_conv_w_split_bytes(int C_out, int C_in, int K);
int64_t fac_conv_w_split_rows_bytes(int C_out, int C_in, int K, int rows);
int fac_pack_conv_w_split_rows(const float* v, const float* scale, void* out, int C_out, int C_in, int K, int rows, fac_stream_t stream);
int fac_pack_conv_w_split(const float* v, const float* scale, void* out, int C_out, int C_in, int K,
                          fac_stream_t stream);
int64_t fac_conv_w_split2_bytes(int C_out, int C_in, int K, int K1);
int fac_pack_conv_w_split2(const float* v, const float* scale, void* out, int C_out, int C_in, int K, int K1, fac_stream_t stream);
int64_t fac_gemm_w_split_bytes(int R, int C_in, int K, int in_stride);
int fac_pack_gemm_w_split(const float* v, int64_t row_stride, int64_t ci_stride, int64_t k_stride, const float* row_scale, void* out,
                          int R, int C_in, int K, int in_stride, fac_stream_t stream);
int fac_conv1d_variant(const fac_conv_desc* d, char* name, int name_len);

int fac_snake_fwd(const float* x, const float* alpha, float* y, int B, int C, int T,
                  fac_stream_t stream);


int fac_lstm_to_time_major(const float* x, float* xT, int B, int H, int T, fac_stream_t stream);
int fac_lstm_from_time_major(const float* yT, const float* skip, const float* alpha, float* out, int B, int H, int T,
                             fac_stream_t stream);
int fac_pack_lstm_whh(const float* w_hh, float* packed, int H, fac_stream_t stream);
int fac_lstm_layer_fwd(const float* pre, const float* whh_packed, float* yT, float* c, int T,
                       int H, int BP, fac_stream_t stream);
int fac_lstm_layer_fwd_from(const float* pre, const float* whh_packed, float* yT, float* c, int T,
                            int H, int BP, int64_t step0, fac_stream_t stream);
int fac_lstm_layer_fwd_train(const float* pre, const float* whh_packed, float* yT, float* c, float* gates_save,
                             float* c_save, int T, int H, int BP, int64_t step0, fac_stream_t stream);
int fac_lstm_gate_bwd(const float* dy_t, const float* rec, const float* gates_t, const float* c_t, const float* c_prev,
                      float* dc, float* dgates_t, int H, int BP, int64_t rs, int first, fac_stream_t stream);
int fac_pack_lstm_whh_t(const float* w_hh, float* packed, int H, fac_stream_t stream);
int fac_lstm_layer_bwd(const float* dyT, const float* whh_t_packed, const float* gates, const float* cs, float* dgates, float* scratch,
                       int T, int H, int BP, fac_stream_t stream);

int fac_lstm_persist_ok(int H, int B);
int fac_lstm_persist_stream_ok(fac_stream_t stream);
int fac_pack_lstm_whh16(const float* w_hh, float* packed, int H, int transposed, fac_stream_t stream);
int fac_lstm_layer_fwd_persist(const float* pre, const float* whh16, float* hfrag, float* yT, float* gates_save, float* c_save,
                               int T, int H, int B, int BP, fac_stream_t stream);
int fac_lstm_layer_bwd_persist(const float* dyT, const float* whh16t, const float* gates, const float* cs, float* dgates,
                               float* scratch, int T, int H, int B, int BP, fac_stream_t stream);
int fac_lstm_persist_split_ok(int H, int B);
int fac_lstm_persist_timeouts(void);
int fac_lstm_persist_arm(fac_stream_t stream);
int fac_lstm_abort_flag(float* dst, fac_stream_t stream);
int fac_mask_flags_if(float* flags, int n, const float* poison, fac_stream_t stream);
int fac_pack_lstm_whh_split(const float* w_hh, void* packed, int H, fac_stream_t stream);
int fac_lstm_layer_fwd_persist_split(const float* pre, const void* wsplit, void* hsplit, float* yT, int T, int H, int B, int BP,
                                     fac_stream_t stream);
int fac_tanh_bwd(const float* y, const float* dy, float* dx, int64_t n, fac_stream_t stream);
int fac_pair_bwd(const float* a, const float* b, float* da, int64_t n, int mode, float eps, float scale, int accumulate,
                 fac_stream_t stream);
int fac_spec_power_bwd(const float* spec, const float* dout, float* dspec, int B, int F, int n_frames, int power,
                       fac_stream_t stream);
int fac_stft_frames_bwd(const float* dframes, float* dwave, int B, int T, int n_win, int n_frames, int hop, int pad,
                        int n_off, fac_stream_t stream);
int fac_vq_latent_bwd(const float* z_e, const float* codebook, const int64_t* codes, int64_t codes_bs, const float* d_zst,
                      const float* wc, float* d_ze, float* z_st, int B, int T, fac_stream_t stream);
int fac_vq_codebook_grad(const float* z_e, const float* codebook, const int64_t* codes, int64_t codes_bs, const float* wb,
                         float* dcb, int B, int T, int Kc, int accumulate, fac_stream_t stream);
int fac_layernorm_c_affine_bwd(const float* x, const float* style, const float* dout, float* dx, float* dstyle, float* stats,
                               int B, int C, int T, fac_stream_t stream);
int fac_rows_fma(const float* a, const float* w, const float* c, float* out, int B, int64_t per, float sign,
                 fac_stream_t stream);
int fac_grad_norm_clip(const float* g, int64_t n, float max_norm, float* scratch, float* norm_out, fac_stream_t stream);
int fac_adamw_step(float* p, const float* g, float* m, float* v, int64_t n, float lr, float beta1, float beta2, float eps,
                   float weight_decay, int64_t step, const float* clip, fac_stream_t stream);
int fac_adamw_step_masked(float* p, const float* g, float* m, float* v, int64_t n, const int64_t* offsets, int n_params,
                          const float* flags, int32_t* steps, float* bc, float lr, float beta1, float beta2, float eps,
                          float weight_decay, const float* clip, fac_stream_t stream);
int fac_gather_copy(const void* const* src, void* const* dst, const int64_t* n, int count, fac_stream_t stream);
int fac_gate_bwd(const float* a, const float* d, float* da, int B, int C, int T, fac_stream_t stream);
int fac_mish_fwd(const float* x, float* y, int64_t n, fac_stream_t stream);
int fac_mish_bwd(const float* x, const float* d, float* dx, int64_t n, fac_stream_t stream);
int fac_glu_bwd(const float* a, const float* d, float* da, int B, int C, int T, fac_stream_t stream);
int fac_mul_scaled(const float* a, const float* b, float* out, float scale, int64_t n, fac_stream_t stream);
int fac_embed_sum_bwd(const float* dx, const int64_t* codes, float* dtables, int B, int n_tab, int n_codes, int code_row0, int V,
                      int E, int T, fac_stream_t stream);
int fac_gate_bwd_cond(const float* a, const float* g, int64_t g_bs, const float* d, float* da, float* dcond, int64_t dcond_bs,
                      int B, int C, int T, fac_stream_t stream);
int fac_masked_mean_bwd(const float* dout, const float* mask, float* dx, int B, int C, int T, fac_stream_t stream);
int fac_attention_probs(const float* q, const float* k, const float* mask, float* P, int B, int H, int dk, int T,
                        fac_stream_t stream);
int fac_attention_pv(const float* P, const float* v, float* o, int B, int H, int dk, int T, fac_stream_t stream);
int fac_attention_bwd_pv(const float* P_used, const float* v, const float* dO, float* dv, float* dP, int B, int H, int dk,
                         int T, fac_stream_t stream);
int fac_attention_bwd_qk(const float* P, float* dP, const float* q, const float* k, const float* mask, float* dq, float* dk_,
                         int B, int H, int dk, int T, fac_stream_t stream);
int fac_aa_snakebeta_bwd(const float* x, const float* alpha_log, const float* beta_log, const float* filter12, const float* dy,
                         float* dx, float* dalpha, float* dbeta, float* scratch, int B, int C, int T, fac_stream_t stream);
int fac_leaky_relu(const float* x, const float* dy, float* out, int64_t n, float slope, int T, int pitch, int valid,
                   int rows_per_group, int valid_rows, fac_stream_t stream);
int fac_period_fold(const float* x, float* out, int B, int T, int period, int L, int pitch, int backward, fac_stream_t stream);
int fac_zero_insert(const float* dy, float* up, int64_t rows, int T, int stride, fac_stream_t stream);
int fac_row_stack3(const float* x, float* out, int64_t rows, int T, int C, int F, int backward, fac_stream_t stream);
int fac_spec_to_cat(const float* src, float* dst, int B, int Ft, int T, int f0, int Fb, int pitch, int backward, fac_stream_t stream);
int fac_spec_to_rows(const float* src, float* dst, int B, int Ft, int T, int f0, int Fb, int backward, fac_stream_t stream);
int fac_pad_reflect(const float* x, float* out, int B, int T, int pad_l, int pad_r, fac_stream_t stream);
int fac_disc_preprocess(const float* x, const float* dz, float* out, float* stats, int B, int T, fac_stream_t stream);
int fac_cross_entropy(const float* logits, const int64_t* labels, float* loss, float* dlogits, float* scratch, int64_t N,
                      int C, float grad_scale, fac_stream_t stream);
int fac_focal_scalar(const float* ce, float* out2, float gamma, fac_stream_t stream);
int fac_crop_rows(const float* src, float* dst, const int64_t* start, int B, int C, int64_t T_src, int T_dst, int scale,
                  fac_stream_t stream);
int fac_stream_push(float* buf, const float* src, int64_t rows, int64_t cap, int hist, int n_prev, int n_new,
                    fac_stream_t stream);

int fac_flip_transpose_w(const float* v, const float* scale, float* out, int C_out, int C_in, int K, fac_stream_t stream);

int fac_prep_begin(void);
int fac_prep_set_phase(int phase);
int fac_prep_abort(void);
int fac_prep_end(void);
int fac_prep_replay(int plan, fac_stream_t stream);
int fac_prep_info(int plan, int* n_jobs, int* n_launches);
int fac_prep_free(int plan);

int fac_pack_conv_w_bwd(const float* v, const float* scale, float* packed, int C_out, int C_in, int K, int C_in_pad,
                        fac_stream_t stream);
int fac_pad_fold_bwd(const float* dxpad, float* dx, int B, int C, int T, int Tp, int pad_left, int pad_mode,
                     fac_stream_t stream);
int fac_pad_fold_edges(float* dxpad, int B, int C, int T, int Tp, int pad_left, fac_stream_t stream);
int64_t fac_conv1d_bwd_weight_ws_bytes(int B, int C_in, int C_out, int T_out, int K);
int fac_conv1d_bwd_weight(const float* x, const float* dy, float* dw, void* ws, int64_t ws_bytes, int B, int C_in,
                          int T_in, int C_out, int T_out, int K, int stride, int dilation, int pad_left, int pad_mode,
                          int K1, int dilation2, fac_stream_t stream);
int64_t fac_conv1d_bwd_weight_k1_ws_bytes(int B, int C_in, int C_out, int T);
int64_t fac_conv1d_bwd_weight_k1_ws_bytes_for(const float* x, const float* dy, int B, int C_in, int C_out, int T);
int fac_conv1d_bwd_weight_k1(const float* x, const float* dy, float* dw, float* db, void* ws, int64_t ws_bytes, int B, int C_in, int C_out,
                             int T, fac_stream_t stream);
int64_t fac_conv1d_bwd_weight_taps_tx(int T_out, int K, int K1, int dilation, int dilation2);
int64_t fac_conv1d_bwd_weight_taps_ws_bytes(int B, int C_in, int C_out, int T_out, int K, int K1, int dilation, int dilation2);
int64_t fac_conv1d_bwd_weight_taps_ws_bytes_for(const float* dy, int B, int C_in, int C_out, int T_out, int K, int K1, int dilation,
                                                int dilation2);
int fac_conv1d_bwd_weight_taps(const float* xpad, const float* dy, float* dw, float* db, void* ws, int64_t ws_bytes, int B, int C_in, int Tx,
                               int C_out, int T_out, int K, int K1, int dilation, int dilation2, fac_stream_t stream);
int64_t fac_conv1d_bwd_weight_split_ws_bytes(int B, int C_in, int T_in, int C_out, int T_out, int K, int stride, int dilation,
                                             int K1, int dilation2);
int fac_conv1d_bwd_weight_split_form(int B, int C_in, int T_in, int C_out, int T_out, int K, int stride, int dilation, int K1,
                                     int dilation2, int want_db, int* form);
int fac_conv1d_bwd_weight_split(const float* x, const float* dy, float* dw, void* ws, int64_t ws_bytes, int B, int C_in, int T_in,
                                int C_out, int T_out, int K, int stride, int dilation, int pad_left, int pad_mode, int K1,
                                int dilation2, fac_stream_t stream);
int fac_conv1d_bwd_weight_split_db_ok(int B, int C_in, int T_in, int C_out, int T_out, int K, int stride, int dilation, int K1,
                                      int dilation2);
int fac_conv1d_bwd_weight_split_db(const float* x, const float* dy, float* dw, float* db, void* ws, int64_t ws_bytes, int B, int C_in,
                                   int T_in, int C_out, int T_out, int K, int stride, int dilation, int pad_left, int pad_mode, int K1,
                                   int dilation2, fac_stream_t stream);
int fac_weight_norm_bwd(const float* v, const float* g, const float* dw, float* dv, float* dg, int n_rows, int row_len,
                        fac_stream_t stream);
int fac_snake_bwd(const float* x, const float* alpha, const float* dy, float* dx, float* dalpha, float* scratch, int B, int C,
                  int T, fac_stream_t stream);
int fac_snake_bwd_fused(const float* x, const float* alpha, const float* dy, const float* add, float* dx, float* dalpha,
                        float* dbias, float* scratch, int B, int C, int T, fac_stream_t stream);
int fac_snake_bwd_fused_rs(const float* x, const float* alpha, const float* dy, long long dy_row_stride, const float* add, float* dx,
                           float* dalpha, float* dbias, float* scratch, int B, int C, int T, fac_stream_t stream);
int fac_bias_grad(const float* dy, float* db, float* scratch, int B, int C, int T, fac_stream_t stream);
// ... 134 lines not shown
```

Measured before the change: 1211 audio-s/s.

## Fuse ResidualUnit k1 tail into bf16x3 split k7 conv kernel for C=96

Adds a FUSED variant of the bf16-split k=7 conv kernel that applies bias and Snake in registers, then runs the 1x1 conv of the ResidualUnit as bf16x3 MFMAs with a new packed k1 weight layout and adds the residual in the epilogue. Previously the streaming path ran the k7 split conv and the k1 conv as separate kernels with an intermediate round trip through memory. This is enabled only for C=96 through BS_FUSED_RU. It adds register pressure and a slow fallback path for large Snake arguments.

```diff
diff --git a/facodec_amd/_lib.py b/facodec_amd/_lib.py
--- a/facodec_amd/_lib.py
+++ b/facodec_amd/_lib.py
@@ -28,6 +28,7 @@
         ("x_p8", _p), ("x_p8_plane_bytes", _i64), ("y2_p8", _p), ("y2_p8_plane_bytes", _i64),
         ("pw_split", C.c_int32), ("split_rows", C.c_int32),
         ("gate_cond", _p), ("gate_cond_bs", _i64),
+        ("w_k1_split", _p),
     ]
 
 
@@ -69,6 +70,9 @@
     "fac_pack_conv_w": (_i, [_p, _p, _p, _i, _i, _i, _i, _p]),
     "fac_pack_convtr_w_rows": (_i, [_p, _p, _p, _i, _i, _i, _p]),
     "fac_conv_w_split_bytes": (_i64, [_i, _i, _i]),
+    "fac_ru_w1_split_bytes": (_i64, [_i]),
+    "fac_ru_w1_split_index": (_i64, [_i, _i, _i]),
+    "fac_pack_ru_w1_split": (_i, [_p, _p, _p, _i, _p]),
     "fac_conv_w_split2_bytes": (_i64, [_i, _i, _i, _i]),
     "fac_pack_conv_w_split2": (_i, [_p, _p, _p, _i, _i, _i, _i, _p]),
     "fac_gemm_w_split_bytes": (_i64, [_i, _i, _i, _i]),
diff --git a/facodec_amd/build.py b/facodec_amd/build.py
--- a/facodec_amd/build.py
+++ b/facodec_amd/build.py
@@ -9,7 +9,7 @@
 LIB = os.path.join(HERE, "libfacodec_hip%s.so" % ("_" + TAG if TAG else ""))
 OBJDIR = "build" + ("_" + TAG if TAG else "")
 SOURCES = ["conv1d_api.hip", "conv1d_tile_128x128.hip", "conv1d_tile_96x128.hip", "conv1d_tile_64x128.hip",
-           "conv1d_tile_32x256.hip", "conv1d_tile_128x32.hip", "conv1d_tile_128x256.hip", "conv1d_fused_ru.hip", "conv1d_narrow.hip", "conv1d_pw.hip", "conv1d_pw_split.hip", "conv1d_skinny.hip", "conv1d_bsplit.hip", "conv1d_bsplit96.hip", "conv1d_gemm_split.hip", "conv1d_bsplit2.hip", "conv1d_bwd.hip", "conv1d_wgrad_split.hip", "conv1d_wgrad_k1.hip", "train_misc.hip", "optim.hip", "train_quant.hip", "train_pred.hip", "train_disc.hip", "train_redecoder.hip", "pack.hip", "prep_batch.hip", "lstm.hip", "lstm_persist.hip", "vq.hip", "vq_decode.hip", "misc.hip", "attention_stream.hip", "ragged.hip", "resample.hip", "jdc.hip", "rccl_arena.hip"]
+           "conv1d_tile_32x256.hip", "conv1d_tile_128x32.hip", "conv1d_tile_128x256.hip", "conv1d_fused_ru.hip", "conv1d_narrow.hip", "conv1d_pw.hip", "conv1d_pw_split.hip", "conv1d_skinny.hip", "conv1d_bsplit.hip", "conv1d_bsplit96.hip", "conv1d_bsplit_ru.hip", "conv1d_gemm_split.hip", "conv1d_bsplit2.hip", "conv1d_bwd.hip", "conv1d_wgrad_split.hip", "conv1d_wgrad_k1.hip", "train_misc.hip", "optim.hip", "train_quant.hip", "train_pred.hip", "train_disc.hip", "train_redecoder.hip", "pack.hip", "prep_batch.hip", "lstm.hip", "lstm_persist.hip", "vq.hip", "vq_decode.hip", "misc.hip", "attention_stream.hip", "ragged.hip", "resample.hip", "jdc.hip", "rccl_arena.hip"]
 FLAGS = ["--offload-arch=gfx950", "-O3", "-std=c++17", "-fPIC", "-ffp-contract=off",
          "-Wno-unused-result"] + os.environ.get("FAC_EXTRA_FLAGS", "").split()
 
diff --git a/facodec_amd/convplan.py b/facodec_amd/convplan.py
--- a/facodec_amd/convplan.py
+++ b/facodec_amd/convplan.py
@@ -1,6 +1,6 @@
 from collections import namedtuple
 
-__all__ = ["ConvPlan", "ConvTrPlan", "plan_conv", "plan_convtr", "plan_gemm", "tile_rows", "gemm_split_ok", "gemm_split_strided_ok", "split2_ok",
+__all__ = ["ConvPlan", "ConvTrPlan", "plan_conv", "plan_convtr", "plan_gemm", "tile_rows", "fused_tail", "gemm_split_ok", "gemm_split_strided_ok", "split2_ok",
            "pw_taps_ok", "pw_split_tail_ok", "convtr_split_ok", "convtr_rows_ok", "flat_strided_ok", "flat_convtr_ok", "W_FP32", "W_TAPS",
            "W_GEMM", "W_GEMM_STRIDED", "W_SPLIT2", "W_FP32_PW_TAPS", "PER_CLIP", "FLAT_STRIDED", "FLAT_STRIDE1", "TR_POLYPHASE", "TR_ROWS",
            "TR_ROWS_SPLIT", "TR_ROWS_PW_TAPS", "TR_FLAT"]
@@ -77,6 +77,13 @@
     return 96 if (sw.BF16_SPLIT and not grad and k == 7 and c_out in sw.BS_ROWS96 and c_in % 8 == 0) else 64
 
 
+def fused_tail(c, k, grad=False):
+    sw = _sw()
+    if not (sw.BF16_SPLIT and not grad and k == 7 and c in sw.BS_FUSED_RU and c in (64, 96)):
+        return False
+    return tile_rows(c, c, k) == (96 if c == 96 else 64)
+
+
 def plan_conv(c_out, c_in, k, stride, dilation, batch, t_in, t_out, *, k1=0, alpha_in=False, plain=True, res=False,
               causal_reflect=False, grad=True, c_out_mult16=True, split_k=(1, 3, 5, 7), floor_k=(3, 5), tail="pw_split",
               pw_taps=True, split2=False, flat_infer=False, flat_stride1=False, flat_train=None):
diff --git a/facodec_amd/csrc/common.h b/facodec_amd/csrc/common.h
--- a/facodec_amd/csrc/common.h
+++ b/facodec_amd/csrc/common.h
@@ -33,8 +33,7 @@
   return __fmul_rn(s, s);
 }
 
-__device__ __forceinline__ float sin_sq(float y) {
-  if (__builtin_expect(fabsf(y) > 4096.0f, 0)) return sin_sq_slow(y);
+__device__ __forceinline__ float sin_sq_poly(float y) {
   const float k = rintf(y * 0.63661977236758134308f);
   float r = fmaf(k, -1.5703125f, y);
   r = fmaf(k, -4.837512969970703125e-4f, r);
@@ -48,6 +47,11 @@
   const float cs = fmaf(pc * z, z, fmaf(z, -0.5f, 1.0f));
   const float v = (((int)k) & 1) ? cs : sn;
   return __fmul_rn(v, v);
+}
+
+__device__ __forceinline__ float sin_sq(float y) {
+  if (__builtin_expect(fabsf(y) > 4096.0f, 0)) return sin_sq_slow(y);
+  return sin_sq_poly(y);
 }
 
 __device__ __forceinline__ float snake_inv(float alpha) { return __fdiv_rn(1.0f, __fadd_rn(alpha, 1e-9f)); }
diff --git a/facodec_amd/csrc/conv1d_api.hip b/facodec_amd/csrc/conv1d_api.hip
--- a/facodec_amd/csrc/conv1d_api.hip
+++ b/facodec_amd/csrc/conv1d_api.hip
@@ -98,6 +98,19 @@
     int max_pad = d->pad_left > pad_right ? d->pad_left : pad_right;
     a.T_ext = d->T_in > max_pad ? d->T_in : max_pad + 1;
   }
+  if (d->w_k1_split) {
+    FAC_REQUIRE(!d->w_k1, "conv1d: w_k1 and w_k1_split are two forms of the same tail, give one");
+    FAC_REQUIRE(!d->x_p8 && !d->y2_p8, "conv1d: the fused split ResidualUnit takes fp32 input and writes fp32 outputs, no P8 operands");
+    FAC_REQUIRE(d->w_split && d->alpha_out && d->act == FAC_ACT_NONE && !d->alpha_in && !d->w_batched && a.rp == 1 && !conv_two_level(a) &&
+                    d->split_rows == (d->C_out == 96 ? 96 : d->split_rows == 64 ? 64 : 0) && conv_bsplit_ru_ok(a),
+                "conv1d: w_k1_split needs split k = 7 weights (split_rows = C for C = 96), C_in == C_out in {64, 96}, stride 1, a Snake "
+                "alpha_out, no activation and more than 640 columns (K=%d stride=%d C_in=%d C_out=%d split_rows=%d columns=%lld)",
+                d->K, d->stride, d->C_in, d->C_out, d->split_rows, (long long)d->B * d->T_out);
+    a.w = reinterpret_cast<const float*>(d->w_split);
+    a.w1 = reinterpret_cast<const float*>(d->w_k1_split);
+    k = CK_FUSED_RU;
+    return FAC_OK;
+  }
   if (d->x_p8 || d->y2_p8) {
     const bool gs = d->w_split && (d->K <= 2 || (d->stride > 1 && d->K <= 2 * d->stride)) && conv_gsplit_ok(a) &&
                     !conv_skinny_ok(a, d->ws, d->ws_bytes) && d->C_in % 8 == 0 && d->x_p8_plane_bytes < (1ll << 32);
@@ -178,7 +191,7 @@
     case CK_128x128: return conv_dispatch_128x128(a, s);
     case CK_128x256: return conv_dispatch_128x256(a, s);
     case CK_96x256: return conv_dispatch_96x256(a, s);
-    case CK_FUSED_RU: return conv_dispatch_fused_ru(a, s);
+    case CK_FUSED_RU: return d->w_k1_split ? conv_dispatch_bsplit_ru(a, s) : conv_dispatch_fused_ru(a, s);
     case CK_128x160: return conv_dispatch_128x160(a, s);
     case CK_NARROW: return conv_dispatch_narrow(a, s);
     case CK_SKINNY: return conv_dispatch_skinny(a, d->ws, d->ws_bytes, s);
@@ -211,7 +224,10 @@
       snprintf(name, name_len, a.rp > 1 ? "conv1d_mfma_kernel<2,2,2,4,2> 128x256 (convtr, all phases per tile)" : "conv1d_mfma_kernel<2,2,2,4,K> 128x256");
       break;
     case CK_96x256: snprintf(name, name_len, "conv1d_mfma_kernel<3,1,1,8,K> 96x256"); break;
-    case CK_FUSED_RU: snprintf(name, name_len, "conv1d_mfma_kernel<C/32,1,1,4,7,fused RU> Cx128"); break;
+    case CK_FUSED_RU:
+      if (d->w_k1_split) snprintf(name, name_len, "conv1d_bsplit_kernel<%d> %dx256 (bf16x3 split, fp32-grade, fused RU)", a.K, a.C_out);
+      else snprintf(name, name_len, "conv1d_mfma_kernel<C/32,1,1,4,7,fused RU> Cx128");
+      break;
     case CK_128x160: snprintf(name, name_len, "conv1d_mfma_kernel<1,5,4,1,K> 128x160"); break;
     case CK_NARROW:
       snprintf(name, name_len, conv_two_level(a) ? "conv1d_narrow_kernel (VALU, C_out<=2, two-level taps)" : "conv1d_narrow_kernel (VALU, C_out<=2)");
diff --git a/facodec_amd/csrc/conv1d_bsplit.hip b/facodec_amd/csrc/conv1d_bsplit.hip
--- a/facodec_amd/csrc/conv1d_bsplit.hip
+++ b/facodec_amd/csrc/conv1d_bsplit.hip
@@ -44,6 +44,11 @@
 __global__ __launch_bounds__(256) void bsplit_batch_kernel(const PrepJob* __restrict__ jobs, const int* __restrict__ first, int njobs) {
   const int j = prep_find_job(first, njobs, blockIdx.x);
   const PrepJob& J = jobs[j];
+  if (J.kind == PK_RU_W1_SPLIT) {
+    pack_ru_w1_split_body(static_cast<const float*>(J.a), static_cast<const float*>(J.b), static_cast<bf16x8*>(J.out), J.i[0], J.n,
+                          blockIdx.x - first[j], J.nblocks);
+    return;
+  }
   pack_conv_split_body(static_cast<const float*>(J.a), static_cast<const float*>(J.b), static_cast<bf16x8*>(J.out), J.i[0], J.i[1],
                        J.i[2], J.i[3], J.i[4], J.i[5], J.i[6], J.n, blockIdx.x - first[j], J.nblocks);
 }
diff --git a/facodec_amd/csrc/conv1d_bsplit_kernel.h b/facodec_amd/csrc/conv1d_bsplit_kernel.h
--- a/facodec_amd/csrc/conv1d_bsplit_kernel.h
+++ b/facodec_amd/csrc/conv1d_bsplit_kernel.h
@@ -16,7 +16,9 @@
 
 __host__ __device__ constexpr int bs_slots(int K, int G) { return (G * K + 1) & ~1; }
 
-template <int KT, int G, int NMW, int NSW, int MB = 2>
+constexpr int bs_ru_ksteps(int MB) { return 2 * MB; }
+__host__ __device__ constexpr int bs_ru_channel(int ks, int kq, int i) { return (ks >> 1) * 32 + 16 * (ks & 1) + (i & 3) + 8 * (i >> 2) + 4 * kq; }
+template <int KT, int G, int NMW, int NSW, int MB = 2, bool FUSED = false>
 __global__ __launch_bounds__((NMW + NSW) * 64, (NMW + NSW) / 4) void conv1d_bsplit_kernel(ConvArgs a) {
   constexpr int NB = 2;
   constexpr int CO = 32 * MB;
@@ -56,6 +58,17 @@
   };
   const bool overlap = a.persist != 0;
   unsigned char* epi_base = sm + (overlap ? STG : 0);
+  if constexpr (FUSED) {
+    static_assert(KT == 7 && NMW == 4 && (MB == 2 || MB == 3), "the fused ResidualUnit tail exists for the wide k = 7 forms");
+    const int epi_bytes = CO * (BS_TT + 4) * 4;
+    float* tab = reinterpret_cast<float*>(sm + (overlap ? STG + (STG > epi_bytes ? STG : epi_bytes) : (2 * STG > epi_bytes ? 2 * STG : epi_bytes)));
+    if (tid < CO) {
+      const float al = a.ru_alpha[tid];
+      tab[tid] = a.ru_bias ? a.ru_bias[tid] : 0.f;
+      tab[CO + tid] = al;
+      tab[2 * CO + tid] = snake_inv(al);
+    }
+  }
   auto walk = [&](auto role) {
   constexpr int ROLE = decltype(role)::value;
   constexpr bool STAGING = ROLE != 0;
@@ -387,7 +400,8 @@
       }
     }
     };
-    if (MB == 2 && co0 + 32 >= a.C_out) pipeline(std::integral_constant<int, 1>{});
+    if constexpr (FUSED) pipeline(std::integral_constant<int, MB>{});
+    else if (MB == 2 && co0 + 32 >= a.C_out) pipeline(std::integral_constant<int, 1>{});
     else pipeline(std::integral_constant<int, MB>{});
   } else {
   for (int chunk = 0; chunk < n_chunks; ++chunk) {
@@ -430,7 +444,117 @@
   }
   }
   __builtin_amdgcn_s_setprio(0);
-  {
+  if constexpr (FUSED) {
+    constexpr int EP = BS_TT + 4;
+    constexpr int KS = bs_ru_ksteps(MB), NU = KS * MB, D = 4;
+    int ln = lane;
+    asm volatile("" : "+v"(ln));
+    const int kq_t = ln >> 5;
+    float* tile = reinterpret_cast<float*>(epi_base) + (4 * kq_t * EP + n0 + (ln & 31));
+    const unsigned char* w1g = reinterpret_cast<const unsigned char*>(a.w1);
+    const unsigned w1l = (unsigned)ln * 16u;
+    const int epi_bytes = CO * EP * 4;
+    const float* tabl = reinterpret_cast<const float*>(sm + (overlap ? STG + (STG > epi_bytes ? STG : epi_bytes) : (2 * STG > epi_bytes ? 2 * STG : epi_bytes))) + 4 * kq_t;
+    bf16x8 W1f[D][3];
+    auto ldw = [&](int u, bf16x8 (&d)[3]) {
+      const int ks = u / MB, mo = u % MB;
+#pragma unroll
+      for (int p = 0; p < 3; ++p) {
+        unsigned off = w1l;
+        asm volatile("" : "+v"(off));
+        off += (unsigned)(((p * MB + mo) * KS + ks) * 1024);
+        asm volatile("" : "+v"(off));
+        d[p] = *reinterpret_cast<const bf16x8*>(w1g + off);
+      }
+    };
+#pragma unroll
+    for (int u = 0; u < D - 1; ++u) ldw(u % NU, W1f[u % D]);
+#pragma unroll
+    for (int n = 0; n < NB; ++n) {
+      bool big = false;
+#pragma unroll
+      for (int m = 0; m < MB; ++m)
+#pragma unroll
+        for (int g = 0; g < 4; ++g) {
+          const float4 bs = *reinterpret_cast<const float4*>(tabl + m * 32 + 8 * g);
+          const float4 al = *reinterpret_cast<const float4*>(tabl + CO + m * 32 + 8 * g);
+          const float b4[4] = {bs.x, bs.y, bs.z, bs.w}, a4[4] = {al.x, al.y, al.z, al.w};
+#pragma unroll
+          for (int i = 0; i < 4; ++i) {
+            const float x = acc[m][n][4 * g + i] + b4[i];
+            acc[m][n][4 * g + i] = x;
+            big = big | (fabsf(__fmul_rn(a4[i], x)) > 4096.0f);
+          }
+        }
+      if (__builtin_expect(__builtin_amdgcn_ballot_w64(big) != 0, 0)) {
+#pragma unroll
+        for (int m = 0; m < MB; ++m)
+#pragma unroll
+          for (int r = 0; r < 16; ++r) tile[(m * 32 + (r & 3) + 8 * (r >> 2)) * EP + n * 32] = acc[m][n][r];
+#pragma unroll 1
+        for (int j = 0; j < 16 * MB; ++j) {
+          const int rb = (j >> 4) * 32 + (j & 3) + 8 * ((j & 15) >> 2);
+          float* p = tile + rb * EP + n * 32;
+          const float x = *p, al = tabl[CO + rb], iv = tabl[2 * CO + rb], y = __fmul_rn(al, x);
+          float ss;
+          if (fabsf(y) > 4096.0f) {
+            const float sv = sinf(y);
+            ss = __fmul_rn(sv, sv);
+          } else {
+            ss = sin_sq_poly(y);
+          }
+          *p = __fadd_rn(x, __fmul_rn(iv, ss));
+        }
+#pragma unroll
+        for (int m = 0; m < MB; ++m)
+#pragma unroll
+          for (int r = 0; r < 16; ++r) acc[m][n][r] = tile[(m * 32 + (r & 3) + 8 * (r >> 2)) * EP + n * 32];
+      } else {
+#pragma unroll
+        for (int m = 0; m < MB; ++m)
+#pragma unroll
+          for (int g = 0; g < 4; ++g) {
+            const float4 al = *reinterpret_cast<const float4*>(tabl + CO + m * 32 + 8 * g);
+            const float4 iv = *reinterpret_cast<const float4*>(tabl + 2 * CO + m * 32 + 8 * g);
+            const float a4[4] = {al.x, al.y, al.z, al.w}, i4[4] = {iv.x, iv.y, iv.z, iv.w};
+#pragma unroll
+            for (int i = 0; i < 4; ++i) {
+              const float x = acc[m][n][4 * g + i];
+              acc[m][n][4 * g + i] = __fadd_rn(x, __fmul_rn(i4[i], sin_sq_poly(__fmul_rn(a4[i], x))));
+            }
+            __builtin_amdgcn_sched_barrier(0);
+          }
+      }
+      f32x16 o[MB];
+#pragma unroll
+      for (int mo = 0; mo < MB; ++mo)
+#pragma unroll
+        for (int r = 0; r < 16; ++r) o[mo][r] = 0.f;
+#pragma unroll
+      for (int ks = 0; ks < KS; ++ks) {
+        bf16x8 hB[3];
+#pragma unroll
+        for (int i = 0; i < 8; ++i) {
+          __bf16 p0, p1, p2;
+          split3(acc[ks >> 1][n][8 * (ks & 1) + i], p0, p1, p2);
+          hB[0][i] = p0; hB[1][i] = p1; hB[2][i] = p2;
+        }
+#pragma unroll
+        for (int mo = 0; mo < MB; ++mo) {
+          const int u = n * NU + ks * MB + mo;
+          if (u + D - 1 < NB * NU) ldw((u + D - 1) % NU, W1f[(u + D - 1) % D]);
+          constexpr int TA[6] = {1, 2, 0, 1, 0, 0}, TB[6] = {1, 0, 2, 0, 1, 0};
+#pragma unroll
+          for (int q = 0; q < 6; ++q) o[mo] = __builtin_amdgcn_mfma_f32_32x32x16_bf16(W1f[u % D][TA[q]], hB[TB[q]], o[mo], 0, 0, 0);
+          __builtin_amdgcn_sched_barrier(0);
+        }
+      }
+#pragma unroll
+      for (int mo = 0; mo < MB; ++mo)
+#pragma unroll
+        for (int r = 0; r < 16; ++r) tile[(mo * 32 + (r & 3) + 8 * (r >> 2)) * EP + n * 32] = o[mo][r];
+    }
+  } else {
     float* tile = reinterpret_cast<float*>(epi_base);
     constexpr int EP = BS_TT + 4;
     if constexpr (MB == 3) {
@@ -467,7 +591,44 @@
     const bool vec_ok = (e->y_cs & 3) == 0 && (e->y_bs & 3) == 0 && (!yg || (reinterpret_cast<unsigned long long>(e->y) & 15) == 0) &&
                         (!y2g || (reinterpret_cast<unsigned long long>(e->y2) & 15) == 0) &&
                         (!rg || (reinterpret_cast<unsigned long long>(e->res) & 15) == 0);
-    for (int q = tid; q < CO * QPR; q += NTH) {
+    int q_first = tid;
+    if constexpr (FUSED) {
+      constexpr int NIT = CO * QPR / NTH, PB = 4, NBAT = NIT / PB;
+      static_assert(CO * QPR % NTH == 0 && NIT % PB == 0, "every thread emits the same number of quads, in whole batches");
+      if (vec_ok && rg && t0 + BS_TT <= e->T_out) {
+        int tid_t = tid;
+        asm volatile("" : "+v"(tid_t));
+        float4 rr[2][PB];
+        auto request = [&](int bt, float4 (&d)[PB]) {
+#pragma unroll
+          for (int j = 0; j < PB; ++j) {
+            const int q = tid_t + (bt * PB + j) * NTH, row = q / QPR, tq = q - row * QPR;
+            d[j] = *reinterpret_cast<const float4*>(rg + ((long long)row * e->y_cs + t0 + 4 * tq));
+          }
+        };
+        request(0, rr[0]);
+#pragma unroll
+        for (int bt = 0; bt < NBAT; ++bt) {
+          if (bt + 1 < NBAT) request(bt + 1, rr[(bt + 1) & 1]);
+#pragma unroll
+          for (int j = 0; j < PB; ++j) {
+            const int q = tid_t + (bt * PB + j) * NTH, row = q / QPR, tq = q - row * QPR;
+            const float4 av = *reinterpret_cast<const float4*>(tile + row * EP + 4 * tq), r4 = rr[bt & 1][j];
+            const float bs = e->bias ? e->bias[row] : 0.f;
+            const long long o = (long long)row * e->y_cs + t0 + 4 * tq;
+            const float v[4] = {av.x + bs + r4.x, av.y + bs + r4.y, av.z + bs + r4.z, av.w + bs + r4.w};
+            if (yg) *reinterpret_cast<float4*>(yg + o) = make_float4(v[0], v[1], v[2], v[3]);
+            if (y2g) {
+              const float a2 = e->alpha2[row], i2 = snake_inv(a2);
+              *reinterpret_cast<float4*>(y2g + o) = make_float4(snake_apply(v[0], a2, i2), snake_apply(v[1], a2, i2),
+                                                                snake_apply(v[2], a2, i2), snake_apply(v[3], a2, i2));
+            }
+          }
+        }
+        q_first = CO * QPR;
+      }
+    }
+    for (int q = q_first; q < CO * QPR; q += NTH) {
       const int row = q / QPR, tq = q - row * QPR;
       const int co = co0 + row, t = t0 + 4 * tq;
       if (co >= e->C_out || t >= e->T_out) continue;
@@ -530,7 +691,29 @@
   }
 }
 
-template <int KT, int G, int NMW, int NSW, int MB = 2>
+__device__ __forceinline__ void pack_ru_w1_split_body(const float* __restrict__ v, const float* __restrict__ scale, bf16x8* __restrict__ out,
+                                                      int C, long long n, int vb, int vg) {
+  const int MB = C / 32, KS = bs_ru_ksteps(MB);
+  for (long long idx = (long long)vb * 256 + threadIdx.x; idx < n; idx += (long long)vg * 256) {
+    const int lane = (int)(idx & 63), ks = (int)((idx >> 6) % KS), mo = (int)((idx >> 6) / KS);
+    const int co = mo * 32 + (lane & 31), kq = lane >> 5;
+    const float sc = scale != nullptr ? scale[co] : 1.0f;
+    bf16x8 h, m, l;
+#pragma unroll
+    for (int i = 0; i < 8; ++i) {
+      float w = v[(long long)co * C + bs_ru_channel(ks, kq, i)];
+      if (scale != nullptr) w = __fmul_rn(w, sc);
+      __bf16 p0, p1, p2;
+      split3(w, p0, p1, p2);
+      h[i] = p0; m[i] = p1; l[i] = p2;
+    }
+    out[((0 * MB + mo) * KS + ks) * 64 + lane] = h;
+    out[((1 * MB + mo) * KS + ks) * 64 + lane] = m;
+    out[((2 * MB + mo) * KS + ks) * 64 + lane] = l;
+  }
+}
+
+template <int KT, int G, int NMW, int NSW, int MB = 2, bool FUSED = false>
 static int bsplit_launch(ConvArgs& a, hipStream_t s) {
   constexpr int H = bs_slots(KT, G), TT = 64 * NMW, CO = 32 * MB;
   a.XW = TT + (H / G - 1) * a.dil;
@@ -547,11 +730,12 @@
   a.persist = (NMW == 4 && a.x_p8 == nullptr && n_chunks % 2 == 0 && cus >= 8 && n_wg > cus &&
                stg + (stg > epi ? stg : epi) <= FAC_LDS_MAX) ? 1 : 0;
   size_t lds = a.persist ? stg + (stg > epi ? stg : epi) : (2 * stg > epi ? 2 * stg : epi);
+  if (FUSED) lds += (size_t)3 * CO * sizeof(float);
   if (lds > FAC_LDS_MAX) {
     set_error("conv1d(bf16 split): tile needs %zu B of LDS (dil=%d)", lds, a.dil);
     return FAC_ERR_ARG;
   }
-  constexpr auto kern = conv1d_bsplit_kernel<KT, G, NMW, NSW, MB>;
+  constexpr auto kern = conv1d_bsplit_kernel<KT, G, NMW, NSW, MB, FUSED>;
   allow_dynamic_lds<kern>();
   a.n_tiles = (int)n_wg;
   hipLaunchKernelGGL(kern, dim3((unsigned)(a.persist ? cus : n_wg)), dim3((NMW + NSW) * 64), lds, s, a);
diff --git a/facodec_amd/csrc/conv1d_bsplit_ru.hip b/facodec_amd/csrc/conv1d_bsplit_ru.hip
--- /dev/null
+++ b/facodec_amd/csrc/conv1d_bsplit_ru.hip
@@ -0,0 +1,53 @@
+#include "conv1d_bsplit_kernel.h"
+
+namespace fac {
+
+__global__ __launch_bounds__(256) void pack_ru_w1_split_kernel(const float* __restrict__ v, const float* __restrict__ scale,
+                                                               bf16x8* __restrict__ out, int C, long long n) {
+  pack_ru_w1_split_body(v, scale, out, C, n, blockIdx.x, gridDim.x);
+}
+
+bool conv_bsplit_ru_ok(const ConvArgs& a) {
+  if (!(a.K == 7 && a.C_in == a.C_out && a.alpha_out && a.act == FAC_ACT_NONE && !a.x_p8 && !a.y2_p8 && a.rp == 1)) return false;
+  if (a.C_out == BS96_CO) return conv_bsplit96_ok(a);
+  return a.C_out == BS_CO && conv_bsplit_ok(a);
+}
+
+int conv_dispatch_bsplit_ru(ConvArgs& a, hipStream_t s) {
+  a.ru_bias = a.bias;
+  a.ru_alpha = a.alpha_out;
+  a.bias = a.bias1;
+  a.alpha_out = nullptr;
+  if (a.C_out == BS96_CO) return bsplit_launch<7, 1, 4, BS_NSW_WIDE, 3, true>(a, s);
+  return bsplit_launch<7, 2, 4, BS_NSW_WIDE, 2, true>(a, s);
+}
+
+}
+
+extern "C" int64_t fac_ru_w1_split_bytes(int C) {
+  return (C == fac::BS_CO || C == fac::BS96_CO) ? (int64_t)3 * C * C * 2 : -1;
+}
+
+extern "C" int64_t fac_ru_w1_split_index(int C, int co, int ci) {
+  using namespace fac;
+  if (!(C == BS_CO || C == BS96_CO) || co < 0 || co >= C || ci < 0 || ci >= C) return -1;
+  const int MB = C / 32, KS = bs_ru_ksteps(MB);
+  const int ks = 2 * (ci / 32) + (ci % 32) / 16, r16 = ci % 16, kq = (r16 >> 2) & 1, i = (r16 & 3) + 4 * (r16 >> 3);
+  if (bs_ru_channel(ks, kq, i) != ci) return -1;
+  return ((int64_t)((co / 32) * KS + ks) * 64 + 32 * kq + co % 32) * 8 + i;
+}
+
+extern "C" int fac_pack_ru_w1_split(const float* v, const float* scale, void* out, int C, fac_stream_t stream) {
+  using namespace fac;
+  FAC_REQUIRE(v && out, "pack_ru_w1_split: null pointer");
+  FAC_REQUIRE(C == BS_CO || C == BS96_CO, "pack_ru_w1_split: the fused split ResidualUnit exists for C = 64 and C = 96 (C=%d)", C);
+  const long long n = (long long)(C / 32) * bs_ru_ksteps(C / 32) * 64;
+  const int blocks = prep_blocks(n);
+  if (prep_recording()) {
+    PrepJob j{}; j.a = v; j.b = scale; j.out = out; j.kind = PK_RU_W1_SPLIT; j.nblocks = blocks; j.n = n;
+    j.i[0] = C;
+    return prep_record(PU_BSPLIT, j);
+  }
+  hipLaunchKernelGGL(pack_ru_w1_split_kernel, dim3(blocks), dim3(256), 0, (hipStream_t)stream, v, scale, reinterpret_cast<bf16x8*>(out), C, n);
+  return check_launch("pack_ru_w1_split");
+}
diff --git a/facodec_amd/csrc/conv1d_mfma.h b/facodec_amd/csrc/conv1d_mfma.h
--- a/facodec_amd/csrc/conv1d_mfma.h
+++ b/facodec_amd/csrc/conv1d_mfma.h
@@ -12,7 +12,7 @@
   const float* x;
   const float* w;
   const float* bias;
-  const float* alpha_in;
+  union { const float* alpha_in; const float* ru_bias; };
   const float* alpha_out;
   const float* res;
   float* y;
@@ -41,7 +41,7 @@
   unsigned char* y2_p8;
   long long y2_p8_ps;
   int rp;
-  const float* gate_cond;
+  union { const float* gate_cond; const float* ru_alpha; };
   long long gate_cond_bs;
 };
 
@@ -621,6 +621,8 @@
 bool conv_bsplit96_ok(const ConvArgs& a);
 bool conv_bsplit96_p8_ok(const ConvArgs& a);
 int conv_dispatch_bsplit96(ConvArgs& a, hipStream_t s);
+bool conv_bsplit_ru_ok(const ConvArgs& a);
+int conv_dispatch_bsplit_ru(ConvArgs& a, hipStream_t s);
 bool conv_pws_ok(const ConvArgs& a);
 int conv_dispatch_pws(ConvArgs& a, hipStream_t s);
 bool conv_pwt_ok(const ConvArgs& a);
diff --git a/facodec_amd/csrc/prep_batch.h b/facodec_amd/csrc/prep_batch.h
--- a/facodec_amd/csrc/prep_batch.h
+++ b/facodec_amd/csrc/prep_batch.h
@@ -21,7 +21,8 @@
   PK_CONV_SPLIT,
   PK_GEMM_SPLIT,
   PK_CONV_SPLIT2,
-  PK_CONV_BWD
+  PK_CONV_BWD,
+  PK_RU_W1_SPLIT
 };
 
 bool prep_recording();
diff --git a/facodec_amd/dac_model.py b/facodec_amd/dac_model.py
--- a/facodec_amd/dac_model.py
+++ b/facodec_amd/dac_model.py
@@ -27,6 +27,14 @@
         b = self.block
         k7, k1 = b[1], b[3]
         streaming = ops.BF16_SPLIT and x.shape[0] * ((x.shape[-1] + 31) // 32) >= 8192
+        if streaming and ops.fused_tail(k7.w.c_out, 7) and x_act.shape[-1] == x.shape[-1]:
+            plan = k7.plan(x.shape[0], x.shape[-1], False, False, False)
+            if plan.layout == ops.W_TAPS and plan.form == ops.PER_CLIP:
+                c = k7.w.c_out
+                pair = ops.conv1d(x_act, None, c, 7, bias=k7.w.bias, dilation=k7.dilation, pad_mode=k7.pad_mode, alpha_out=b[2].flat(),
+                                  res=x, w_split=k7.w.packed_split(ops.tile_rows(c, c, 7)), w_k1_split=k1.w.packed_ru_tail(),
+                                  bias_k1=k1.w.bias, alpha_y2=alpha_next, want_y=want_raw or alpha_next is None, causal=k7.causal)
+                return pair if alpha_next is not None else (pair, None)
         if k7.w.c_out in FUSED_RU_CHANNELS and x_act.shape[-1] == x.shape[-1] and not streaming:
             return_pair = ops.conv1d(x_act, k7.w.packed(), k7.w.c_out, 7, bias=k7.w.bias, dilation=k7.dilation,
                                      alpha_out=b[2].flat(), res=x, w_k1=k1.w.packed(), bias_k1=k1.w.bias,
diff --git a/facodec_amd/layers.py b/facodec_amd/layers.py
--- a/facodec_amd/layers.py
+++ b/facodec_amd/layers.py
@@ -30,6 +30,7 @@
         self._split = None
         self._rows = None
         self._rows_split = None
+        self._ru_tail = None
         self.freeze_packed = False
 
     def _vg(self):
@@ -59,8 +60,12 @@
     def packed_split(self, rows=64):
         return self._cached("_split", ops.pack_conv_weight_split, rows=rows)
 
+    def packed_ru_tail(self):
+        return self._cached("_ru_tail", ops.pack_ru_tail_split)
+
     def _apply(self, fn, *a, **kw):
         self._packed = None
+        self._ru_tail = None
         self._split = None
         self._rows = None
         self._rows_split = None
diff --git a/facodec_amd/ops.py b/facodec_amd/ops.py
--- a/facodec_amd/ops.py
+++ b/facodec_amd/ops.py
@@ -197,6 +197,7 @@
 
 BF16_SPLIT = True
 BS_ROWS96 = (96,)
+BS_FUSED_RU = (96,)
 
 
 def set_conv_profile(p):
@@ -302,7 +303,7 @@
     d.ws, d.ws_bytes = ws.data_ptr(), CONV_WS_BYTES
     if _FLOPS is not None or _PROFILE is not None:
         flops = 2.0 * d.B * d.n_phase * max(1, d.row_phases) * d.C_out * d.T_out * d.C_in * d.K
-        if d.w_k1:
+        if d.w_k1 or d.w_k1_split:
             flops += 2.0 * d.B * d.C_out * d.T_out * d.C_out
     if _FLOPS is not None:
         _FLOPS.add(_FLOP_KEY, flops)
@@ -403,6 +404,22 @@
     return out
 
 
+@prepared
+def pack_ru_tail_split(v, g=None, out=None, scale=None):
+    v = _dev(v, "weight")
+    c_out, c_in, k = v.shape
+    lib = _lib.load()
+    nbytes = lib.fac_ru_w1_split_bytes(c_out) if (k == 1 and c_in == c_out) else -1
+    if nbytes < 0:
+        raise _lib.FacodecHipError("pack_ru_tail_split: no fused split ResidualUnit for weights %s" % (tuple(v.shape),))
+    if scale is None and g is not None:
+        scale = wn_scale(v, g)
+    if out is None:
+        out = torch.empty(nbytes, device=v.device, dtype=torch.uint8)
+    _lib.check(lib.fac_pack_ru_w1_split(_ptr(v), _ptr(scale), out.data_ptr(), c_out, _stream()), "fac_pack_ru_w1_split")
+    return out
+
+
 def conv_out_len(t_in, k, stride, dilation):
     k_eff = (k - 1) * dilation + 1
     padding_total = k_eff - stride
@@ -476,7 +493,8 @@
 
 def conv1d(x, w_packed, c_out, k, bias=None, stride=1, dilation=1, pad_left=None, pad_mode=PAD_REFLECT,
            t_out=None, alpha_in=None, alpha_out=None, res=None, act=ACT_NONE, out=None, causal=True,
-           alpha_y2=None, want_y=True, w_k1=None, bias_k1=None, w_split=None, k1=0, dilation2=0, skip_acc=None, gate_cond=None):
+           alpha_y2=None, want_y=True, w_k1=None, bias_k1=None, w_split=None, k1=0, dilation2=0, skip_acc=None, gate_cond=None,
+           w_k1_split=None):
     x_p8 = x if isinstance(x, P8) else None
     if x_p8 is not None:
         B, c_in, t_in = x_p8.shape
@@ -512,6 +530,7 @@
     d.w_k1 = w_k1.data_ptr() if w_k1 is not None else None
     d.bias_k1 = bias_k1.data_ptr() if bias_k1 is not None else None
     d.w_split = w_split.data_ptr() if w_split is not None else None
+    d.w_k1_split = w_k1_split.data_ptr() if w_k1_split is not None else None
     if out is not None and (out.stride(0), out.stride(1)) != (d.y_bs, d.y_cs) and out.shape[0] * out.shape[1] > 1:
         assert out.stride(2) == 1 and y2 is None and res is None and out.shape == (B, c_y, t_out)
         d.y_bs, d.y_cs = out.stride(0), out.stride(1)
diff --git a/include/facodec_hip.h b/include/facodec_hip.h
--- a/include/facodec_hip.h
+++ b/include/facodec_hip.h
@@ -81,12 +81,16 @@
   int32_t split_rows;
   const float* gate_cond;
   int64_t gate_cond_bs;
+  const void* w_k1_split;
 } fac_conv_desc;
 
 int fac_conv1d_fwd(const fac_conv_desc* d, fac_stream_t stream);
 int fac_to_p8(const float* x, const float* alpha, void* out, int B, int C, int T, fac_stream_t stream);
 int64_t fac_conv_w_split_bytes(int C_out, int C_in, int K);
 int64_t fac_conv_w_split_rows_bytes(int C_out, int C_in, int K, int rows);
+int64_t fac_ru_w1_split_bytes(int C);
+int64_t fac_ru_w1_split_index(int C, int co, int ci);
+int fac_pack_ru_w1_split(const float* v, const float* scale, void* out, int C, fac_stream_t stream);
 int fac_pack_conv_w_split_rows(const float* v, const float* scale, void* out, int C_out, int C_in, int K, int rows, fac_stream_t stream);
 int fac_pack_conv_w_split(const float* v, const float* scale, void* out, int C_out, int C_in, int K,
                           fac_stream_t stream);
```

Result: no change. 1221 audio-s/s, median of 6 (+0.8%).
